# LUMII-Syslab/DiffusionSAT

Hardware: NVIDIA B200
Metric: diffusion samples/sec, 3-SAT n=100 (higher is better)
Workload: dtype f32

## Files before the change

diffusionsat_b200/csrc/dsat_api.cu:

```cuda
#include <cuda_runtime.h>
#include <math.h>
#include <stdint.h>
#include <stdio.h>
#include <stdlib.h>
#include <string.h>

#include <algorithm>
#include <string>
#include <type_traits>
#include <vector>

#include "../../include/dsat.h"
#include "../../include/dsat_debug.h"
#include "dsat_common.cuh"
#include "dsat_gemm_simt.cuh"
#include "dsat_message.cuh"
#include "dsat_spmm.cuh"
#include "dsat_graph_host.cuh"
#include "dsat_norm_head.cuh"
#include "dsat_hist.cuh"
#ifdef DSAT_WITH_TCGEN05
#include "dsat_gemm_tc.cuh"
#include "dsat_mlp_fused.cuh"
#include "dsat_mlp_x3.cuh"
#endif

using namespace dsat;

static cudaError_t dsat_memcpy_sync(void* dst, const void* src, size_t bytes, cudaMemcpyKind kind) {
    cudaError_t e = cudaMemcpy(dst, src, bytes, kind);
    if (e == cudaSuccess && kind == cudaMemcpyHostToDevice) e = cudaDeviceSynchronize();
    return e;
}

namespace {

template <typename T>
struct DevBuf {
    T* p = nullptr;
    size_t count = 0;
    size_t cap = 0;
    cudaError_t alloc(size_t n) {
        if (p && n <= cap) { count = n; return cudaSuccess; }
        release();
        if (n == 0) return cudaSuccess;
        cudaError_t e = cudaMalloc(reinterpret_cast<void**>(&p), n * sizeof(T));
        if (e == cudaSuccess) { count = n; cap = n; }
        else p = nullptr;
        return e;
    }
    void drop() { count = 0; }
    void release() {
        if (p) cudaFree(p);
        p = nullptr; count = 0; cap = 0;
    }
    cudaError_t upload(const T* host, size_t n, cudaStream_t s) {
        return cudaMemcpyAsync(p, host, n * sizeof(T), cudaMemcpyHostToDevice, s);
    }
};

struct PackedLayer {
    DevBuf<float> w, b;
#ifdef DSAT_WITH_TCGEN05
    DevBuf<__nv_bfloat16> w_bf16;
#endif
    int K = 0, N = 0;
};

enum OpId { OP_V1 = 0, OP_Q2, OP_L2, OP_L3, OP_C1, OP_C2, OP_U1, OP_U2, OP_U3, OP_O1, OP_O2, OP_COUNT };

}

constexpr int SPMM_DW_CLAUSE = 2;
struct dsat_ctx {
    int device = 0;
    int sm_count = 148;
    cudaStream_t own_stream = nullptr, stream = nullptr;
    cudaEvent_t ev0 = nullptr, ev1 = nullptr;
    std::string err;
    long long launches = 0;
#ifdef DSAT_WITH_TCGEN05
    int precision = DSAT_F32_TC;
#else
    int precision = DSAT_F32;
#endif
    struct ProfMark { cudaEvent_t ev; int cls; };
    std::vector<ProfMark> prof;
    size_t prof_used = 0;
    bool profiling = false;

    bool has_model = false;
    int F = 0, Q = 0, HQ = 0, HL = 0, HC = 0, HU = 0, HO = 0;
    PackedLayer ops[OP_COUNT];

    bool has_graph = false;
    int n = 0, m = 0, nnz = 0, n_graphs = 0, chains = 0, group_graphs = 0, n_groups = 0, total_graphs = 0;
    int words = 0;
    int max_graph_vars = 0, max_graph_clauses = 0;
    long long Nt = 0, Mt = 0;
    DevBuf<int> cl_rowptr, cl_lit, lit_rowptr, lit_clause, var_seg, clause_seg;
    DevBuf<float> deg_w, vdeg_w, rev_w;
    DevBuf<int> var_order;
    DevBuf<unsigned short> cl_idx16, lit_idx16;
    int cl_idx16_vecs = 0, lit_idx16_vecs = 0, cl_col_off = 0, lit_col_off = 0, lit_ord_off = 0;
    DevBuf<int> cl_desc, lit_desc, lit_desc4;
    bool use_spmm_order = true;
    std::vector<int32_t> h_cl_rowptr, h_cl_lit, h_lit_rowptr, h_lit_clause;
    std::vector<float> h_deg_w, h_rev_w;
    bool spmm_desc_ready = false;
    int spmm_minb = 0, spmm_pf = -1;
    int spmm_half = -1;
    int spmm_lit_dw = 0;
    bool use_idx16 = true;

    bool has_buffers = false;
    DevBuf<float> VROW, CROW, H1, H2, QS, LIT, CH, COUT, U1, U2, UOUT, SPRE, O1, LOGITS, OUT;
    DevBuf<float2> X;
    DevBuf<int> labels, done, steps_taken, rounds_run, graph_sat, graph_map, latch_step, sat_now;
    DevBuf<float> loss_sum, graph_loss;
    DevBuf<unsigned char> BITS, LAST, LATCH, FINAL, is_sat, sat_any;
    DevBuf<unsigned long long> packed;
    DevBuf<int> hist_idx, hist_run, hist_totals;
    DevBuf<unsigned long long> hist_keys, hist_counts;
    DevBuf<float> inj_normals, inj_uniforms, inj_noisy;
    DevBuf<int> inj_labels;
#ifdef DSAT_WITH_TCGEN05
    DevBuf<__nv_bfloat16> VROWb, CROWb, H1b, H2b, QSb, LITb, CHb, COUTb, U1b, U2b, UOUTb, SPREb, O1b;
    CUtensorMap map_a[OP_COUNT];
    CUtensorMap map_b[OP_COUNT];
    int a_box_rows[OP_COUNT] = {0}, b_box_rows[OP_COUNT] = {0};
    bool has_tc_buffers = false;
    fm::FusedMlp fused[5];
    bool fused_ready = false;
    bool use_fused = true;
    bool use_smem_gather = true;
    DevBuf<__nv_bfloat16> VROWp, CROWp, SPREp, H1p, H2p;
    DevBuf<__nv_bfloat16> CHp, U1p, U2p;
    x3::X3Mlp x3s[5];
    bool split_clause = false, split_update = false;
    DevBuf<__nv_bfloat16> wx[12];
    int wx_k64[12] = {0}, wx_n[12] = {0};
    x3::X3Mlp x3[7];
    bool has_x3_buffers = false;
    bool x3_ready = false;
#endif
    bool has_simt_buffers = false;
    float last_noise_scale = 0.f;
    int sampling = DSAT_SAMPLE_INVERSE_CDF;
    DevBuf<StepParams> step_tab;
    DevBuf<int> step_cur;
    std::vector<StepParams> step_tab_host;
    cudaGraphExec_t step_graph = nullptr;
    long long generation = 0, step_graph_generation = -1;
    int step_graph_rounds = -1, step_graph_precision = -1, step_launches = 0;
    bool use_graph = true;

    int ldv() const { return F + DSAT_AUX_PAD + 3 * Q; }
    int ldc() const { return F + 2 * Q; }
    int ldh1() const { return HQ + HL; }
};

#ifdef DSAT_ASSERT
static int* g_assert_host = nullptr;
static std::string assert_note() {
    return g_assert_host && g_assert_host[0] ? " [DSAT_ASSERT failed at line " + std::to_string(g_assert_host[0]) + " of a kernel header]" : "";
}
#else
static std::string assert_note() { return ""; }
#endif

#define CK_CUDA(ctx, expr)                                                              \
    do {                                                                                \
        cudaError_t e__ = (expr);                                                       \
        if (e__ != cudaSuccess) {                                                       \
            (ctx)->err = std::string(#expr) + ": " + cudaGetErrorString(e__) + assert_note(); \
            return DSAT_ERR_CUDA;                                                       \
        }                                                                               \
    } while (0)

#define CK_ARG(ctx, cond, msg)                                                          \
    do {                                                                                \
        if (!(cond)) { (ctx)->err = (msg); return DSAT_ERR_ARG; }                       \
    } while (0)

#define LAUNCHED(ctx)                                                                   \
    do {                                                                                \
        (ctx)->launches++;                                                              \
        CK_CUDA(ctx, cudaGetLastError());                                               \
    } while (0)

namespace {

cudaError_t configure_kernels_for_device() {
    static PerDeviceOnce configured;
    if (configured.done()) return cudaSuccess;
    cudaError_t e = cudaSuccess;
    auto opt_in = [&](auto kernel) {
        if (e == cudaSuccess) e = cudaFuncSetAttribute(kernel, cudaFuncAttributeMaxDynamicSharedMemorySize, 227 * 1024);
    };
#ifdef DSAT_WITH_TCGEN05
    opt_in(clause_gather_smem_kernel<128, true>); opt_in(clause_gather_smem_kernel<128, false>);
    opt_in(clause_gather_smem_kernel<64, true>); opt_in(clause_gather_smem_kernel<64, false>);
    opt_in(clause_gather_smem_kernel<32, true>); opt_in(clause_gather_smem_kernel<32, false>);
    opt_in(literal_gather_smem_kernel<128, true>); opt_in(literal_gather_smem_kernel<128, false>);
    opt_in(literal_gather_smem_kernel<64, true>); opt_in(literal_gather_smem_kernel<64, false>);
    opt_in(literal_gather_smem_kernel<32, true>); opt_in(literal_gather_smem_kernel<32, false>);
    opt_in(clause_gather_smem_f32_kernel<128, true>); opt_in(clause_gather_smem_f32_kernel<128, false>);
    opt_in(clause_gather_smem_f32_kernel<64, true>); opt_in(clause_gather_smem_f32_kernel<64, false>);
    opt_in(clause_gather_smem_f32_kernel<32, true>); opt_in(clause_gather_smem_f32_kernel<32, false>);
    opt_in(clause_gather_smem_f32x2_kernel<128, true>); opt_in(clause_gather_smem_f32x2_kernel<128, false>);
    opt_in(clause_gather_smem_f32x2_kernel<64, true>); opt_in(clause_gather_smem_f32x2_kernel<64, false>);
    opt_in(clause_gather_smem_f32x2_kernel<32, true>); opt_in(clause_gather_smem_f32x2_kernel<32, false>);
    opt_in(literal_gather_smem_f32_kernel<128, true>); opt_in(literal_gather_smem_f32_kernel<128, false>);
    opt_in(literal_gather_smem_f32_kernel<64, true>); opt_in(literal_gather_smem_f32_kernel<64, false>);
    opt_in(literal_gather_smem_f32_kernel<32, true>); opt_in(literal_gather_smem_f32_kernel<32, false>);
    opt_in(pairnorm_smem_kernel<2>); opt_in(pairnorm_smem_kernel<4>); opt_in(pairnorm_smem_kernel<8>);
    if (e == cudaSuccess) e = fm::configure_fused_device();
    if (e == cudaSuccess) e = x3::configure_x3_device(0);
    if (e == cudaSuccess) e = tc::configure_tc_device();
#endif
    if (e == cudaSuccess) configured.mark();
    return e;
}

UnitGraphDev graph_view(const dsat_ctx* c) {
    UnitGraphDev g;
    g.n = c->n; g.m = c->m; g.nnz = c->nnz; g.n_graphs = c->n_graphs;
    g.cl_rowptr = c->cl_rowptr.p; g.cl_lit = c->cl_lit.p;
    g.lit_rowptr = c->lit_rowptr.p; g.lit_clause = c->lit_clause.p;
    g.var_seg = c->var_seg.p; g.clause_seg = c->clause_seg.p;
    g.deg_w = c->deg_w.p; g.vdeg_w = c->vdeg_w.p; g.rev_w = c->rev_w.p;
    g.var_order = c->var_order.p;
    g.cl_idx16 = c->cl_idx16_vecs ? c->cl_idx16.p : nullptr;
    g.lit_idx16 = c->lit_idx16_vecs ? c->lit_idx16.p : nullptr;
    g.cl_idx16_vecs = c->cl_idx16_vecs; g.lit_idx16_vecs = c->lit_idx16_vecs;
    g.cl_col_off = c->cl_col_off; g.lit_col_off = c->lit_col_off; g.lit_ord_off = c->lit_ord_off;
    return g;
}

SkipInfo skip_info(const dsat_ctx* c) {
    static const bool off = getenv("DSAT_SKIP_DONE") && atoi(getenv("DSAT_SKIP_DONE")) == 0;
    if (off || c->n_graphs <= 0 || c->group_graphs % c->n_graphs != 0) return SkipInfo{nullptr, 1};
    return SkipInfo{c->done.p, c->group_graphs / c->n_graphs};
}

int ensure_common_buffers(dsat_ctx* c) {
    if (c->has_buffers) return DSAT_OK;
    if (!c->has_model || !c->has_graph) { c->err = "set the model and the graph first"; return DSAT_ERR_STATE; }
    const size_t Nt = (size_t)c->Nt, Mt = (size_t)c->Mt;
    CK_CUDA(c, c->QS.alloc(Nt * 3 * c->Q));
    CK_CUDA(c, c->LIT.alloc(Nt * 2 * c->Q));
    CK_CUDA(c, c->COUT.alloc(Mt * (c->Q + c->F)));
    CK_CUDA(c, c->UOUT.alloc(Nt * c->F));
    CK_CUDA(c, c->LOGITS.alloc(Nt * DSAT_LOGIT_PAD));
    CK_CUDA(c, c->OUT.alloc(Nt));
    CK_CUDA(c, c->X.alloc(Nt + 1));
    CK_CUDA(c, c->labels.alloc(Nt));
    CK_CUDA(c, c->BITS.alloc(Nt));
    CK_CUDA(c, c->LAST.alloc(Nt));
    CK_CUDA(c, c->LATCH.alloc(Nt));
    CK_CUDA(c, c->FINAL.alloc(Nt));
    const size_t G = (size_t)c->total_graphs, NG = (size_t)c->n_groups;
    CK_CUDA(c, c->done.alloc(NG));
    CK_CUDA(c, c->steps_taken.alloc(NG));
    CK_CUDA(c, c->rounds_run.alloc(NG));
    CK_CUDA(c, c->loss_sum.alloc(NG));
    CK_CUDA(c, c->graph_sat.alloc(G));
    CK_CUDA(c, c->graph_map.alloc(G));
    CK_CUDA(c, c->graph_loss.alloc(G));
    CK_CUDA(c, c->latch_step.alloc(G));
    CK_CUDA(c, c->sat_now.alloc(G));
    CK_CUDA(c, c->is_sat.alloc(G));
    CK_CUDA(c, c->sat_any.alloc(G));
    CK_CUDA(c, c->packed.alloc(G * c->words));
    CK_CUDA(c, cudaMemsetAsync(c->OUT.p, 0, c->OUT.count * sizeof(float), c->stream));
    c->has_buffers = true;
    return DSAT_OK;
}

int ensure_buffers(dsat_ctx* c) {
    int rc = ensure_common_buffers(c);
    if (rc) return rc;
    if (c->has_simt_buffers) return DSAT_OK;
    const size_t Nt = (size_t)c->Nt, Mt = (size_t)c->Mt;
    CK_CUDA(c, c->VROW.alloc(Nt * c->ldv()));
    CK_CUDA(c, c->CROW.alloc(Mt * c->ldc()));
    CK_CUDA(c, c->H1.alloc(Nt * c->ldh1()));
    CK_CUDA(c, c->H2.alloc(Nt * c->HL));
    CK_CUDA(c, c->CH.alloc(Mt * c->HC));
    CK_CUDA(c, c->U1.alloc(Nt * c->HU));
    CK_CUDA(c, c->U2.alloc(Nt * c->HU));
    CK_CUDA(c, c->SPRE.alloc(Nt * c->F));
    CK_CUDA(c, c->O1.alloc(Nt * c->HO));
    CK_CUDA(c, cudaMemsetAsync(c->VROW.p, 0, c->VROW.count * sizeof(float), c->stream));
    CK_CUDA(c, cudaMemsetAsync(c->CROW.p, 0, c->CROW.count * sizeof(float), c->stream));
    c->has_simt_buffers = true;
    return DSAT_OK;
}

#ifdef DSAT_WITH_TCGEN05
static int pick_slice_width(size_t table_rows, int Q, size_t* bytes_out, int budget_kb, int elt_bytes = 2);

__global__ void mirror_cols_kernel(const float* __restrict__ src, int ld_src, __nv_bfloat16* __restrict__ dst, int ld_dst,
                                   long long rows, int cols) {
    const long long i = (long long)blockIdx.x * blockDim.x + threadIdx.x;
    if (i >= rows * cols) return;
    const long long r = i / cols; const int cc = (int)(i % cols);
    dst[(size_t)r * ld_dst + cc] = __float2bfloat16_rn(src[(size_t)r * ld_src + cc]);
}

int ensure_tc_buffers(dsat_ctx* c) {
    if (c->has_tc_buffers) return DSAT_OK;
    int rc = ensure_buffers(c);
    if (rc) return rc;
    const size_t Nt = (size_t)c->Nt, Mt = (size_t)c->Mt;
    const int F = c->F, Q = c->Q;
    CK_CUDA(c, c->VROWb.alloc(Nt * c->ldv()));
    CK_CUDA(c, c->CROWb.alloc(Mt * c->ldc()));
    CK_CUDA(c, c->H1b.alloc(Nt * c->ldh1()));
    CK_CUDA(c, c->H2b.alloc(Nt * c->HL));
    CK_CUDA(c, c->QSb.alloc(Nt * 3 * Q));
    CK_CUDA(c, c->LITb.alloc(Nt * 2 * Q));
    CK_CUDA(c, c->CHb.alloc(Mt * c->HC));
    CK_CUDA(c, c->COUTb.alloc(Mt * (Q + F)));
    CK_CUDA(c, c->UOUTb.alloc(Nt * F));
    CK_CUDA(c, c->U1b.alloc(Nt * c->HU));
    CK_CUDA(c, c->U2b.alloc(Nt * c->HU));
    CK_CUDA(c, c->SPREb.alloc(Nt * F));
    CK_CUDA(c, c->O1b.alloc(Nt * c->HO));
    CK_CUDA(c, cudaMemsetAsync(c->VROWb.p, 0, c->VROWb.count * 2, c->stream));
    CK_CUDA(c, cudaMemsetAsync(c->CROWb.p, 0, c->CROWb.count * 2, c->stream));
    struct Src { const void* p; long long rows; int k; int ld; };
    const Src srcs[OP_COUNT] = {
        {c->VROWb.p, c->Nt, F + DSAT_AUX_PAD, c->ldv()},
        {c->H1b.p, c->Nt, c->HQ, c->ldh1()},
        {c->H1b.p + c->HQ, c->Nt, c->HL, c->ldh1()},
        {c->H2b.p, c->Nt, c->HL, c->HL},
        {c->CROWb.p, c->Mt, F + 2 * Q, c->ldc()},
        {c->CHb.p, c->Mt, c->HC, c->HC},
        {c->VROWb.p, c->Nt, F + DSAT_AUX_PAD + 3 * Q, c->ldv()},
        {c->U1b.p, c->Nt, c->HU, c->HU},
        {c->U2b.p, c->Nt, c->HU, c->HU},
        {c->SPREb.p, c->Nt, F, F},
        {c->O1b.p, c->Nt, c->HO, c->HO},
    };
    for (int op = 0; op < OP_COUNT; ++op) {
        if (srcs[op].k != c->ops[op].K) { c->err = "internal: A operand width mismatch"; return DSAT_ERR_STATE; }
        c->a_box_rows[op] = (int)(srcs[op].rows < tc::BLOCK_M ? srcs[op].rows : tc::BLOCK_M);
        if (!tc::make_bf16_map(&c->map_a[op], srcs[op].p, srcs[op].rows, srcs[op].k, srcs[op].ld, c->a_box_rows[op])) {
            c->err = "cuTensorMapEncodeTiled failed for an activation operand";
            return DSAT_ERR_CUDA;
        }
    }
    {
        enum { FQ = 0, FL, FC, FU, FO };
        const int k64_v1 = (c->ops[OP_V1].K + 63) / 64 * 64;
        struct L { int op; int n; const __nv_bfloat16* w; const float* b; int epi; };
        auto build = [&](int which, int a_op, std::initializer_list<L> layers, tc::TcOut out) -> bool {
            fm::FusedMlp& f = c->fused[which];
            f.map_a = c->map_a[a_op];
            f.p.n_layers = (int)layers.size();
            f.p.rows = (int)(a_op == OP_C1 ? c->Mt : c->Nt);
            f.p.a_box_rows = c->a_box_rows[a_op];
            f.p.qmaps = Q;
            f.p.prof = nullptr;
            f.p.dbg = getenv("DSAT_FM_DEBUG") ? atoi(getenv("DSAT_FM_DEBUG")) : 0;
            f.p.out = out;
            int i = 0;
            for (const L& l : layers) {
                const int K = c->ops[l.op].K, K64 = (K + 63) / 64 * 64;
                f.p.layer[i].K = K; f.p.layer[i].N = l.n; f.p.layer[i].epi = l.epi; f.p.layer[i].bias = l.b;
                f.p.layer[i].box_rows = l.n < 256 ? l.n : 256;
                if (!tc::make_bf16_map(&f.map_w[i], l.w, l.n, K64, K64, f.p.layer[i].box_rows)) return false;
                if (!tc::make_bf16_map(&f.map_wp[i], l.w, l.n, K64, K64, f.p.layer[i].box_rows / 2)) return false;
                ++i;
            }
            {
                static const int mask = getenv("DSAT_A_RING") ? atoi(getenv("DSAT_A_RING")) : 0x1d;
                f.stream_input = ((mask >> which) & 1) != 0;
                static const int pair_mask = getenv("DSAT_PAIR_MODE") ? atoi(getenv("DSAT_PAIR_MODE")) : 0xe;
                f.pair_mode = ((pair_mask >> which) & 1) != 0;
                static const bool pp_env = getenv("DSAT_PING_PONG") != nullptr;
                static const int pp_mask = pp_env ? atoi(getenv("DSAT_PING_PONG")) : 0x1b;
                f.ping_pong = ((pp_mask >> which) & 1) != 0 || (!pp_env && which == FC && f.pair_mode);
                static const int split_on = getenv("DSAT_SPLIT_MODE") ? atoi(getenv("DSAT_SPLIT_MODE")) : 1;
                f.split_step_bias = (split_on & 2) == 0;
                f.split_mode = split_on != 0;
            }
            if (!fm::plan_fused(f)) return false;
            if (getenv("DSAT_PLAN_LOG"))
                fprintf(stderr, "[dsat] fused mlp %d: smem %d B (pad %d), hidden blocks %d x%d, input ring %d, weight ring %d x %d B, "
                        "epilogue warps %d, ping-pong %d, staging in hidden %d, cta pair %d, split %d (%d steps)\n", which, f.smem_bytes, f.p.smem_pad, f.p.ah_blocks,
                        f.p.pp ? 2 : 1, f.p.a_slots, f.p.slots, f.p.slot_bytes, f.p.epi_warps, f.p.pp, f.p.stage_in_h, f.p.pair, f.p.split, f.p.n_steps);
            return true;
        };
        auto W = [&](int op) { return (const __nv_bfloat16*)c->ops[op].w_bf16.p; };
        auto B = [&](int op) { return (const float*)c->ops[op].b.p; };
        tc::TcOut o;
        bool ok = true;
        o = {c->QSb.p, 3 * Q, 1, nullptr, 0, 0, 0};
        ok = ok && build(FQ, OP_V1, {{OP_V1, c->HQ, W(OP_V1), B(OP_V1), tc::TC_LRELU},
                                     {OP_Q2, Q, W(OP_Q2), B(OP_Q2), tc::TC_QUERY}}, o);
        o = {c->LITb.p, 2 * Q, 1, nullptr, 0, 0, 0};
        ok = ok && build(FL, OP_V1, {{OP_V1, c->HL, W(OP_V1) + (size_t)c->HQ * k64_v1, B(OP_V1) + c->HQ, tc::TC_LRELU},
                                     {OP_L2, c->HL, W(OP_L2), B(OP_L2), tc::TC_LRELU},
                                     {OP_L3, 2 * Q, W(OP_L3), B(OP_L3), tc::TC_LINEAR}}, o);
        o = {c->COUTb.p, Q + F, 1, nullptr, 0, 0, 0};
        ok = ok && build(FC, OP_C1, {{OP_C1, c->HC, W(OP_C1), B(OP_C1), tc::TC_LRELU},
                                     {OP_C2, Q + F, W(OP_C2), B(OP_C2), tc::TC_LINEAR}}, o);
        o = {c->UOUTb.p, F, 1, nullptr, 0, 0, 0};
        ok = ok && build(FU, OP_U1, {{OP_U1, c->HU, W(OP_U1), B(OP_U1), tc::TC_LRELU},
                                     {OP_U2, c->HU, W(OP_U2), B(OP_U2), tc::TC_LRELU},
                                     {OP_U3, F, W(OP_U3), B(OP_U3), tc::TC_LINEAR}}, o);
        o = {c->LOGITS.p, DSAT_LOGIT_PAD, 0, nullptr, 0, 0, 0};
        ok = ok && build(FO, OP_O1, {{OP_O1, c->HO, W(OP_O1), B(OP_O1), tc::TC_LRELU},
                                     {OP_O2, DSAT_LOGIT_PAD, W(OP_O2), B(OP_O2), tc::TC_LINEAR}}, o);
        c->fused_ready = ok;
    }
    c->has_tc_buffers = true;
    return DSAT_OK;
}

int tc_pack_weights(dsat_ctx* c) {
    for (int op = 0; op < OP_COUNT; ++op) {
        const int K = c->ops[op].K, N = c->ops[op].N;
        const int K64 = (K + 63) / 64 * 64;
        std::vector<float> w((size_t)K * N);
        CK_CUDA(c, dsat_memcpy_sync(w.data(), c->ops[op].w.p, w.size() * sizeof(float), cudaMemcpyDeviceToHost));
        std::vector<__nv_bfloat16> wt((size_t)N * K64, __float2bfloat16(0.f));
        for (int k = 0; k < K; ++k)
            for (int n = 0; n < N; ++n) wt[(size_t)n * K64 + k] = __float2bfloat16(w[(size_t)k * N + n]);
        CK_CUDA(c, c->ops[op].w_bf16.alloc(wt.size()));
        CK_CUDA(c, dsat_memcpy_sync(c->ops[op].w_bf16.p, wt.data(), wt.size() * 2, cudaMemcpyHostToDevice));
        c->b_box_rows[op] = N < tc::BLOCK_N ? N : tc::BLOCK_N;
        if (!tc::make_bf16_map(&c->map_b[op], c->ops[op].w_bf16.p, N, K64, K64, c->b_box_rows[op])) {
            c->err = "cuTensorMapEncodeTiled failed for a weight operand (no CUDA driver?)";
            return DSAT_ERR_CUDA;
        }
    }
    return DSAT_OK;
}
#endif

void release_buffers(dsat_ctx* c) {
    c->generation++;
    c->VROW.drop(); c->CROW.drop(); c->H1.drop(); c->H2.drop(); c->QS.drop(); c->LIT.drop();
    c->CH.drop(); c->COUT.drop(); c->U1.drop(); c->U2.drop(); c->UOUT.drop(); c->SPRE.drop();
    c->O1.drop(); c->LOGITS.drop(); c->OUT.drop(); c->X.drop(); c->labels.drop();
    c->BITS.drop(); c->LAST.drop(); c->LATCH.drop(); c->FINAL.drop();
    c->done.drop(); c->steps_taken.drop(); c->rounds_run.drop(); c->loss_sum.drop();
    c->graph_sat.drop(); c->graph_map.drop(); c->graph_loss.drop(); c->latch_step.drop();
    c->sat_now.drop(); c->is_sat.drop(); c->sat_any.drop(); c->packed.drop();
    c->inj_normals.drop(); c->inj_uniforms.drop(); c->inj_noisy.drop(); c->inj_labels.drop();
    c->hist_idx.drop(); c->hist_run.drop(); c->hist_totals.drop(); c->hist_keys.drop(); c->hist_counts.drop();
#ifdef DSAT_WITH_TCGEN05
    c->VROWb.drop(); c->CROWb.drop(); c->H1b.drop(); c->H2b.drop(); c->QSb.drop(); c->LITb.drop();
    c->CHb.drop(); c->COUTb.drop(); c->UOUTb.drop(); c->U1b.drop(); c->U2b.drop(); c->SPREb.drop();
    c->O1b.drop();
    c->has_tc_buffers = false;
    c->VROWp.drop(); c->CROWp.drop(); c->SPREp.drop(); c->H1p.drop(); c->H2p.drop();
    c->CHp.drop(); c->U1p.drop(); c->U2p.drop();
    c->has_x3_buffers = false;
#endif
    c->has_buffers = false;
    c->has_simt_buffers = false;
}

void free_buffers(dsat_ctx* c) {
    c->VROW.release(); c->CROW.release(); c->H1.release(); c->H2.release(); c->QS.release(); c->LIT.release();
    c->CH.release(); c->COUT.release(); c->U1.release(); c->U2.release(); c->UOUT.release(); c->SPRE.release();
    c->O1.release(); c->LOGITS.release(); c->OUT.release(); c->X.release(); c->labels.release();
    c->BITS.release(); c->LAST.release(); c->LATCH.release(); c->FINAL.release();
    c->done.release(); c->steps_taken.release(); c->rounds_run.release(); c->loss_sum.release();
    c->graph_sat.release(); c->graph_map.release(); c->graph_loss.release(); c->latch_step.release();
    c->sat_now.release(); c->is_sat.release(); c->sat_any.release(); c->packed.release();
    c->inj_normals.release(); c->inj_uniforms.release(); c->inj_noisy.release(); c->inj_labels.release();
    c->hist_idx.release(); c->hist_run.release(); c->hist_totals.release(); c->hist_keys.release(); c->hist_counts.release();
#ifdef DSAT_WITH_TCGEN05
    c->VROWb.release(); c->CROWb.release(); c->H1b.release(); c->H2b.release(); c->QSb.release(); c->LITb.release();
    c->CHb.release(); c->COUTb.release(); c->UOUTb.release(); c->U1b.release(); c->U2b.release(); c->SPREb.release();
    c->O1b.release();
    c->has_tc_buffers = false;
    c->VROWp.release(); c->CROWp.release(); c->SPREp.release(); c->H1p.release(); c->H2p.release();
    c->CHp.release(); c->U1p.release(); c->U2p.release();
    c->has_x3_buffers = false;
#endif
    c->has_buffers = false;
    c->has_simt_buffers = false;
}

enum ProfClass { PROF_CLAUSE_GATHER = OP_COUNT, PROF_LITERAL_GATHER, PROF_NORM_CLAUSE, PROF_NORM_VAR, PROF_HEAD,
                 PROF_NOISE, PROF_END, PROF_CLASSES = PROF_END };

void prof_mark(dsat_ctx* c, int cls) {
    if (!c->profiling) return;
    if (c->prof_used == c->prof.size()) {
        cudaEvent_t e;
        cudaEventCreate(&e);
        c->prof.push_back({e, cls});
    }
    c->prof[c->prof_used].cls = cls;
    cudaEventRecord(c->prof[c->prof_used].ev, c->stream);
    c->prof_used++;
}

#ifdef DSAT_WITH_TCGEN05
int x3_pack_weights(dsat_ctx* c) {
    struct Cut { int op, col0, n; };
    const Cut cuts[12] = {
        {OP_V1, 0, c->HQ}, {OP_Q2, 0, c->Q}, {OP_V1, c->HQ, c->HL}, {OP_L2, 0, c->HL}, {OP_L3, 0, 2 * c->Q},
        {OP_C1, 0, c->HC}, {OP_C2, 0, c->Q + c->F}, {OP_U1, 0, c->HU}, {OP_U2, 0, c->HU}, {OP_U3, 0, c->F},
        {OP_O1, 0, c->HO}, {OP_O2, 0, DSAT_LOGIT_PAD}};
    for (int i = 0; i < 12; ++i) {
        const int op = cuts[i].op, K = c->ops[op].K, Nop = c->ops[op].N, n = cuts[i].n;
        const int K64 = (K + 63) / 64 * 64;
        std::vector<float> w((size_t)K * Nop);
        CK_CUDA(c, dsat_memcpy_sync(w.data(), c->ops[op].w.p, w.size() * sizeof(float), cudaMemcpyDeviceToHost));
        std::vector<__nv_bfloat16> wt((size_t)2 * n * K64, __float2bfloat16(0.f));
        for (int k = 0; k < K; ++k)
            for (int j = 0; j < n; ++j) {
                const float v = w[(size_t)k * Nop + cuts[i].col0 + j];
                const __nv_bfloat16 hi = __float2bfloat16(v);
                wt[(size_t)j * K64 + k] = hi;
                wt[(size_t)(n + j) * K64 + k] = __float2bfloat16(v - __bfloat162float(hi));
            }
        CK_CUDA(c, c->wx[i].alloc(wt.size()));
        CK_CUDA(c, dsat_memcpy_sync(c->wx[i].p, wt.data(), wt.size() * 2, cudaMemcpyHostToDevice));
        c->wx_k64[i] = K64; c->wx_n[i] = n;
    }
    return DSAT_OK;
}

int ensure_x3_buffers(dsat_ctx* c) {
    if (c->has_x3_buffers) return DSAT_OK;
    int rc = ensure_common_buffers(c);
    if (rc) return rc;
    const size_t Nt = (size_t)c->Nt, Mt = (size_t)c->Mt;
    const int F = c->F, Q = c->Q;
    CK_CUDA(c, c->VROWp.alloc(2 * Nt * c->ldv()));
    CK_CUDA(c, c->CROWp.alloc(2 * Mt * c->ldc()));
    CK_CUDA(c, c->SPREp.alloc(2 * Nt * F));
    CK_CUDA(c, c->H1p.alloc(2 * Nt * c->HL));
    CK_CUDA(c, c->H2p.alloc(2 * Nt * c->HL));
    CK_CUDA(c, cudaMemsetAsync(c->VROWp.p, 0, c->VROWp.count * 2, c->stream));
    CK_CUDA(c, cudaMemsetAsync(c->CROWp.p, 0, c->CROWp.count * 2, c->stream));
    enum { XQ = 0, XL1, XL2, XL3, XC, XU, XO };
    struct L { int wi; int op; int bias_off; int epi; };
    static const int pair_mask = getenv("DSAT_X3_PAIR") ? atoi(getenv("DSAT_X3_PAIR")) : 0x3e;
    auto build = [&](int which, const __nv_bfloat16* a_hi, size_t a_plane, long long rows, int k, int lda,
                     std::initializer_list<L> layers, int n_groups, int out_mode, void* out0, void* out1, int ld_out) -> bool {
        x3::X3Mlp& f = c->x3[which];
        f.ready = false;
        x3::X3Params& p = f.p;
        p.n_layers = (int)layers.size();
        p.rows = (int)rows;
        p.n_groups = n_groups;
        p.a_box_rows = (int)(rows < x3::BLOCK_M ? rows : x3::BLOCK_M);
        p.qmaps = Q;
        p.prof = nullptr;
        p.out_mode = out_mode; p.out0 = out0; p.out1 = out1; p.ld_out = ld_out;
        {
            const SkipInfo sk = skip_info(c);
            p.done = sk.done; p.chains_per_group = sk.chains_per_group;
            p.rows_per_chain = rows == c->Mt ? c->m : c->n;
        }
        f.pair_mode = ((pair_mask >> which) & 1) != 0;
        static const int epi4_mask = getenv("DSAT_X3_EPI4") ? atoi(getenv("DSAT_X3_EPI4")) : 0;
        f.four_epilogue_warps = ((epi4_mask >> which) & 1) != 0;
        if (!tc::make_bf16_map(&f.map_a_hi, a_hi, rows, k, lda, p.a_box_rows)) return false;
        if (!tc::make_bf16_map(&f.map_a_lo, a_hi + a_plane, rows, k, lda, p.a_box_rows)) return false;
        int i = 0;
        for (const L& l : layers) {
            x3::X3Layer& ly = p.layer[i];
            const int n_total = c->wx_n[l.wi];
            ly.K = c->ops[l.op].K; ly.N = n_groups > 1 ? 256 : n_total; ly.n_total = n_total;
            ly.epi = l.epi; ly.w_lo_row = n_total; ly.bias = c->ops[l.op].b.p + l.bias_off;
            if (n_groups > 1 && n_total != 256 * n_groups) return false;
            ++i;
        }
        if (!x3::plan_x3(f)) return false;
        i = 0;
        for (const L& l : layers) {
            const int box = f.p.pair ? p.layer[i].N / 2 : p.layer[i].N;
            if (!tc::make_bf16_map(&f.map_w[i], c->wx[l.wi].p, 2 * c->wx_n[l.wi], c->wx_k64[l.wi], c->wx_k64[l.wi], box)) return false;
            ++i;
        }
        for (; i < x3::MAX_LAYERS; ++i) f.map_w[i] = f.map_w[0];
        if (getenv("DSAT_PLAN_LOG"))
            fprintf(stderr, "[dsat] x3 mlp %d: smem %d B, hidden blocks 2 x %d, input ring %d, weight ring %d x %d B, epilogue warps %d, "
                    "staging in hidden %d, cta pair %d, groups %d\n", which, f.smem_bytes, p.h_blocks, p.a_slots, p.w_slots, p.w_slot_bytes,
                    p.epi_warps, p.stage_in_h, p.pair, p.n_groups);
        return true;
    };
    const size_t vplane = Nt * c->ldv(), cplane = Mt * c->ldc(), splane = Nt * F, hplane = Nt * c->HL;
    bool ok = true;
    ok = ok && build(XQ, c->VROWp.p, vplane, c->Nt, F + DSAT_AUX_PAD, c->ldv(),
                     {{0, OP_V1, 0, tc::TC_LRELU}, {1, OP_Q2, 0, tc::TC_QUERY}}, 1, x3::OUT_F32, c->QS.p, nullptr, 3 * Q);
    const int lgroups = c->HL > 256 ? c->HL / 256 : 1;
    ok = ok && (c->HL <= 256 || c->HL % 256 == 0);
    ok = ok && build(XL1, c->VROWp.p, vplane, c->Nt, F + DSAT_AUX_PAD, c->ldv(),
                     {{2, OP_V1, c->HQ, tc::TC_LRELU}}, lgroups, x3::OUT_SPLIT, c->H1p.p, c->H1p.p + hplane, c->HL);
    ok = ok && build(XL2, c->H1p.p, hplane, c->Nt, c->HL, c->HL,
                     {{3, OP_L2, 0, tc::TC_LRELU}}, lgroups, x3::OUT_SPLIT, c->H2p.p, c->H2p.p + hplane, c->HL);
    const int l3groups = 2 * Q > 256 ? 2 * Q / 256 : 1;
    ok = ok && build(XL3, c->H2p.p, hplane, c->Nt, c->HL, c->HL,
                     {{4, OP_L3, 0, tc::TC_LINEAR}}, l3groups, x3::OUT_F32, c->LIT.p, nullptr, 2 * Q);
    if (Q + F <= 256 && c->HC <= 256)
        ok = ok && build(XC, c->CROWp.p, cplane, c->Mt, F + 2 * Q, c->ldc(),
                         {{5, OP_C1, 0, tc::TC_LRELU}, {6, OP_C2, 0, tc::TC_LINEAR}}, 1, x3::OUT_F32, c->COUT.p, nullptr, Q + F);
    else ok = false;
    if (c->HU <= 256)
        ok = ok && build(XU, c->VROWp.p, vplane, c->Nt, F + DSAT_AUX_PAD + 3 * Q, c->ldv(),
                         {{7, OP_U1, 0, tc::TC_LRELU}, {8, OP_U2, 0, tc::TC_LRELU}, {9, OP_U3, 0, tc::TC_LINEAR}}, 1, x3::OUT_F32,
                         c->UOUT.p, nullptr, F);
    else ok = false;
    ok = ok && build(XO, c->SPREp.p, splane, c->Nt, F, F,
                     {{10, OP_O1, 0, tc::TC_LRELU}, {11, OP_O2, 0, tc::TC_LINEAR}}, 1, x3::OUT_F32, c->LOGITS.p, nullptr, DSAT_LOGIT_PAD);
    {
        static const int split_mask = getenv("DSAT_X3_SPLIT") ? atoi(getenv("DSAT_X3_SPLIT")) : 1;
        c->split_clause = c->split_update = false;
        if (ok && (split_mask & 1)) {
            const size_t chplane = Mt * c->HC;
            CK_CUDA(c, c->CHp.alloc(2 * chplane));
            x3::X3Mlp keep_c = c->x3[XC];
            bool k = build(XC, c->CROWp.p, cplane, c->Mt, F + 2 * Q, c->ldc(), {{5, OP_C1, 0, tc::TC_LRELU}}, 1, x3::OUT_SPLIT,
                           c->CHp.p, c->CHp.p + chplane, c->HC);
            c->x3s[0] = c->x3[XC];
            k = k && build(XC, c->CHp.p, chplane, c->Mt, c->HC, c->HC, {{6, OP_C2, 0, tc::TC_LINEAR}}, 1, x3::OUT_F32,
                           c->COUT.p, nullptr, Q + F);
            c->x3s[1] = c->x3[XC];
            c->x3[XC] = keep_c;
            c->split_clause = k;
        }
        if (ok && (split_mask & 2)) {
            const size_t uplane = Nt * c->HU;
            CK_CUDA(c, c->U1p.alloc(2 * uplane));
            CK_CUDA(c, c->U2p.alloc(2 * uplane));
            x3::X3Mlp keep_u = c->x3[XU];
            bool k = build(XU, c->VROWp.p, vplane, c->Nt, F + DSAT_AUX_PAD + 3 * Q, c->ldv(), {{7, OP_U1, 0, tc::TC_LRELU}}, 1,
                           x3::OUT_SPLIT, c->U1p.p, c->U1p.p + uplane, c->HU);
            c->x3s[2] = c->x3[XU];
            k = k && build(XU, c->U1p.p, uplane, c->Nt, c->HU, c->HU, {{8, OP_U2, 0, tc::TC_LRELU}}, 1, x3::OUT_SPLIT,
                           c->U2p.p, c->U2p.p + uplane, c->HU);
            c->x3s[3] = c->x3[XU];
            k = k && build(XU, c->U2p.p, uplane, c->Nt, c->HU, c->HU, {{9, OP_U3, 0, tc::TC_LINEAR}}, 1, x3::OUT_F32,
                           c->UOUT.p, nullptr, F);
            c->x3s[4] = c->x3[XU];
            c->x3[XU] = keep_u;
            c->split_update = k;
        }
    }
    c->x3_ready = ok;
    if (!ok) { c->err = "the fp32-accurate tensor-core path supports feature_maps = query_maps <= 128 (hidden widths <= 256 or 512)"; return DSAT_ERR_UNSUPPORTED; }
    c->has_x3_buffers = true;
    return DSAT_OK;
}

int run_x3(dsat_ctx* c, int which, int prof_class) {
    prof_mark(c, prof_class);
    CK_CUDA(c, x3::launch_x3(c->x3[which], c->device, c->sm_count, c->stream));
    c->launches++;
    return DSAT_OK;
}
#endif

int run_linear(dsat_ctx* c, int op, const float* A, int lda, float* Y, int ldy, long long rows, int epi) {
    prof_mark(c, op);
    LinearOp l;
    l.A = A; l.lda = lda; l.W = c->ops[op].w.p; l.ldw = c->ops[op].N; l.bias = c->ops[op].b.p;
    l.Y = Y; l.ldy = ldy; l.rows = (int)rows; l.K = c->ops[op].K; l.N = c->ops[op].N; l.epi = epi; l.qmaps = c->Q;
    CK_CUDA(c, launch_sgemm(l, c->stream));
    c->launches++;
    return DSAT_OK;
}

template <typename KernelLauncher>
int dispatch_width(dsat_ctx* c, int width, KernelLauncher&& fn) {
    switch (width) {
        case 64: fn(std::integral_constant<int, 2>()); break;
        case 128: fn(std::integral_constant<int, 4>()); break;
        case 256: fn(std::integral_constant<int, 8>()); break;
        default: c->err = "feature width must be 64, 128 or 256"; return DSAT_ERR_UNSUPPORTED;
    }
    return DSAT_OK;
}

struct LossScalars { float t, ts, norm_plus; };


float kl_host(float pa, float pb) {
    float qa = 1.0f - pa;
    float t1 = pa == 0.f ? 0.f : pa * (logf(pa) - logf(pb));
    float t2 = qa == 0.f ? 0.f : qa * (log1pf(-pa) - log1pf(-pb));
    return t1 + t2;
}
LossScalars loss_scalars(float noise_scale) {
    LossScalars s;
    s.t = powf(noise_scale, 0.5f);
    s.ts = fminf(s.t + 0.01f, 1.0f);
    float pa = 0.0f * (1.0f - s.ts) + s.ts / 2.0f;
    float pb = 0.0f * (1.0f - 1.0f) + 1.0f / 2.0f;
    s.norm_plus = kl_host(pa, pb) + 1e-4f;
    return s;
}

#ifdef DSAT_WITH_TCGEN05
static inline bool use_tc(const dsat_ctx* c) { return c->precision == DSAT_BF16 || c->precision == DSAT_BF16_UNFUSED; }
static inline bool use_x3(const dsat_ctx* c) { return c->precision == DSAT_F32_TC; }
static inline __nv_bfloat16* vrow_b(dsat_ctx* c) { return use_tc(c) ? c->VROWb.p : use_x3(c) ? c->VROWp.p : nullptr; }
static inline __nv_bfloat16* crow_b(dsat_ctx* c) { return use_tc(c) ? c->CROWb.p : use_x3(c) ? c->CROWp.p : nullptr; }
#else
static inline bool use_tc(const dsat_ctx*) { return false; }
static inline bool use_x3(const dsat_ctx*) { return false; }
static inline __nv_bfloat16* vrow_b(dsat_ctx*) { return nullptr; }
static inline __nv_bfloat16* crow_b(dsat_ctx*) { return nullptr; }
#endif

int ensure_active_buffers(dsat_ctx* c) {
#ifdef DSAT_WITH_TCGEN05
    if (use_tc(c)) return ensure_tc_buffers(c);
    if (use_x3(c)) return ensure_x3_buffers(c);
#endif
    return ensure_buffers(c);
}

int begin_call(dsat_ctx* c, float noise_scale, const float* noisy_dev, const float* uniforms_dev,
               const int* labels_dev, bool use_x, NoiseSource ns, const StepParams* sp_tab = nullptr, const int* sp_cur = nullptr) {
    const long long Nt = c->Nt;
    const int threads = 256;
    const bool x3p = use_x3(c);
    const size_t vplane = x3p ? (size_t)Nt * c->ldv() : 0, cplane = x3p ? (size_t)c->Mt * c->ldc() : 0;
    c->last_noise_scale = noise_scale;
    step_begin_kernel<<<(unsigned)((Nt + threads - 1) / threads), threads, 0, c->stream>>>(
        Nt, noise_scale, use_x ? c->X.p : nullptr, noisy_dev, uniforms_dev, labels_dev, c->labels.p,
        x3p ? nullptr : c->VROW.p, c->ldv(), c->F, vrow_b(c), ns, vplane, sp_tab, sp_cur, c->sampling == DSAT_SAMPLE_GUMBEL ? 1 : 0);
    LAUNCHED(c);
    {
        long long tot;
        if (!x3p) {
            tot = Nt * (c->F / 4);
            fill_cols_kernel<<<(unsigned)((tot + threads - 1) / threads), threads, 0, c->stream>>>(
                c->VROW.p, c->ldv(), Nt, c->F / 4, 1.0f);
            LAUNCHED(c);
            tot = c->Mt * (c->F / 4);
            fill_cols_kernel<<<(unsigned)((tot + threads - 1) / threads), threads, 0, c->stream>>>(
                c->CROW.p, c->ldc(), c->Mt, c->F / 4, 1.0f);
            LAUNCHED(c);
        }
        if (use_tc(c) || x3p) {
            tot = Nt * (c->F / 8);
            fill_cols_bf16_kernel<<<(unsigned)((tot + threads - 1) / threads), threads, 0, c->stream>>>(
                vrow_b(c), c->ldv(), Nt, c->F / 8, 1.0f);
            LAUNCHED(c);
            if (x3p) {
                fill_cols_bf16_kernel<<<(unsigned)((tot + threads - 1) / threads), threads, 0, c->stream>>>(
                    vrow_b(c) + vplane, c->ldv(), Nt, c->F / 8, 0.0f);
                LAUNCHED(c);
            }
            tot = c->Mt * (c->F / 8);
            fill_cols_bf16_kernel<<<(unsigned)((tot + threads - 1) / threads), threads, 0, c->stream>>>(
                crow_b(c), c->ldc(), c->Mt, c->F / 8, 1.0f);
            LAUNCHED(c);
            if (x3p) {
                fill_cols_bf16_kernel<<<(unsigned)((tot + threads - 1) / threads), threads, 0, c->stream>>>(
                    crow_b(c) + cplane, c->ldc(), c->Mt, c->F / 8, 0.0f);
                LAUNCHED(c);
            }
        }
    }
    CK_CUDA(c, cudaMemsetAsync(c->done.p, 0, c->done.count * sizeof(int), c->stream));
    CK_CUDA(c, cudaMemsetAsync(c->steps_taken.p, 0xff, c->steps_taken.count * sizeof(int), c->stream));
    CK_CUDA(c, cudaMemsetAsync(c->rounds_run.p, 0, c->rounds_run.count * sizeof(int), c->stream));
    CK_CUDA(c, cudaMemsetAsync(c->loss_sum.p, 0, c->loss_sum.count * sizeof(float), c->stream));
    return DSAT_OK;
}

#ifdef DSAT_WITH_TCGEN05
int run_linear_tc(dsat_ctx* c, int op, long long rows, int epi, void* p0, int ld0, bool bf0,
                  void* p1 = nullptr, int ld1 = 0, bool bf1 = false, int split = 0) {
    prof_mark(c, op);
    tc::TcLinear l;
    l.map_a = c->map_a[op]; l.map_b = c->map_b[op]; l.bias = c->ops[op].b.p;
    l.out.ptr0 = p0; l.out.ld0 = ld0; l.out.bf16_0 = bf0 ? 1 : 0;
    l.out.ptr1 = p1; l.out.ld1 = ld1; l.out.bf16_1 = bf1 ? 1 : 0; l.out.split = split;
    l.rows = (int)rows; l.K = c->ops[op].K; l.N = c->ops[op].N; l.epi = epi; l.qmaps = c->Q;
    l.a_box_rows = c->a_box_rows[op]; l.b_box_rows = c->b_box_rows[op];
    CK_CUDA(c, tc::launch_tc_linear(l, c->stream));
    c->launches++;
    return DSAT_OK;
}
#endif

#ifdef DSAT_WITH_TCGEN05
int run_fused(dsat_ctx* c, int which, int prof_class) {
    prof_mark(c, prof_class);
    CK_CUDA(c, fm::launch_fused(c->fused[which], c->sm_count, c->stream));
    c->launches++;
    return DSAT_OK;
}
#endif

#ifdef DSAT_WITH_TCGEN05
static int pick_slice_width(size_t table_rows, int Q, size_t* bytes_out, int budget_kb, int elt_bytes) {
    static const int env_kb = getenv("DSAT_GATHER_KB") ? atoi(getenv("DSAT_GATHER_KB")) : 0;
    if (env_kb > 0) budget_kb = env_kb;
    const int widths[3] = {128, 64, 32};
    for (int pass = 0; pass < 2; ++pass)
        for (int w : widths) {
            if (w > Q || Q % w) continue;
            const size_t bytes = 2 * table_rows * (size_t)w * (size_t)elt_bytes;
            if (bytes <= (size_t)(pass == 0 ? budget_kb : 220) * 1024u) { *bytes_out = bytes; return w; }
        }
    return 0;
}

static bool idx_fits(size_t table_bytes, int idx_vecs) {
    if (idx_vecs <= 0) return false;
    const size_t sm_bytes = 227 * 1024, reserved = 1024, with_idx = table_bytes + (size_t)idx_vecs * 16;
    if (with_idx + reserved > sm_bytes) return false;
    return sm_bytes / (with_idx + reserved) == sm_bytes / (table_bytes + reserved);
}


bool launch_clause_gather_smem(dsat_ctx* c, const UnitGraphDev& g) {
    if (c->n_graphs != 1 || !c->use_smem_gather) return false;
    size_t bytes = 0;
    const int w = pick_slice_width((size_t)2 * c->n, c->Q, &bytes, 56);
    if (!w) return false;
    dim3 grid((unsigned)c->chains, (unsigned)(c->Q / w));
    const int Q = c->Q;
    const bool si = c->use_idx16 && idx_fits(bytes, g.cl_idx16_vecs);
    const size_t smem = bytes + (si ? (size_t)g.cl_idx16_vecs * 16 : 0);
    auto launch = [&](auto kernel) -> bool {
        kernel<<<grid, 512, smem, c->stream>>>(g, Q, c->LITb.p, 2 * Q, c->QSb.p, 3 * Q, Q, c->CROWb.p, c->ldc(), c->F, skip_info(c));
        return true;
    };
    if (w == 128) return si ? launch(clause_gather_smem_kernel<128, true>) : launch(clause_gather_smem_kernel<128, false>);
    if (w == 64) return si ? launch(clause_gather_smem_kernel<64, true>) : launch(clause_gather_smem_kernel<64, false>);
    return si ? launch(clause_gather_smem_kernel<32, true>) : launch(clause_gather_smem_kernel<32, false>);
}

bool launch_literal_gather_smem(dsat_ctx* c, const UnitGraphDev& g) {
    if (c->n_graphs != 1 || !c->use_smem_gather) return false;
    size_t bytes = 0;
    const int w = pick_slice_width((size_t)c->m, c->Q, &bytes, 112);
    if (!w) return false;
    dim3 grid((unsigned)c->chains, (unsigned)(c->Q / w));
    const int Q = c->Q, F = c->F;
    const bool si = c->use_idx16 && idx_fits(bytes, g.lit_idx16_vecs);
    const size_t smem = bytes + (si ? (size_t)g.lit_idx16_vecs * 16 : 0);
    auto launch = [&](auto kernel) -> bool {
        kernel<<<grid, 512, smem, c->stream>>>(g, Q, c->CROWb.p, c->ldc(), F + Q, c->COUTb.p, Q + F, c->QSb.p, 3 * Q, c->VROWb.p,
                                               c->ldv(), F + DSAT_AUX_PAD, skip_info(c));
        return true;
    };
    if (w == 128) return si ? launch(literal_gather_smem_kernel<128, true>) : launch(literal_gather_smem_kernel<128, false>);
    if (w == 64) return si ? launch(literal_gather_smem_kernel<64, true>) : launch(literal_gather_smem_kernel<64, false>);
    return si ? launch(literal_gather_smem_kernel<32, true>) : launch(literal_gather_smem_kernel<32, false>);
}
#endif

#ifdef DSAT_WITH_TCGEN05
bool launch_clause_gather_smem_f32(dsat_ctx* c, const UnitGraphDev& g) {
    if (c->n_graphs != 1 || !c->use_smem_gather) return false;
    static const bool one_table = getenv("DSAT_GATHER_F32_CL1") && atoi(getenv("DSAT_GATHER_F32_CL1")) != 0;
    size_t bytes = 0;
    static const int budget = getenv("DSAT_GATHER_F32_KB_CL") ? atoi(getenv("DSAT_GATHER_F32_KB_CL")) : 110;
    const int w = pick_slice_width((size_t)2 * c->n, c->Q, &bytes, budget, one_table ? 2 : 4);
    if (!w || bytes > 112 * 1024) return false;
    dim3 grid((unsigned)c->chains, (unsigned)((one_table ? 2 : 1) * (c->Q / w)));
    const int Q = c->Q;
    const bool si = c->use_idx16 && idx_fits(bytes, g.cl_idx16_vecs);
    const size_t smem = bytes + (si ? (size_t)g.cl_idx16_vecs * 16 : 0);
    const size_t cplane = (size_t)c->Mt * c->ldc();
    auto launch = [&](auto kernel) -> bool {
        kernel<<<grid, 512, smem, c->stream>>>(g, Q, c->LIT.p, 2 * Q, c->QS.p, 3 * Q, Q, c->CROWp.p, cplane, c->ldc(), c->F, skip_info(c));
        return true;
    };
    if (one_table) {
        if (w == 128) return si ? launch(clause_gather_smem_f32_kernel<128, true>) : launch(clause_gather_smem_f32_kernel<128, false>);
        if (w == 64) return si ? launch(clause_gather_smem_f32_kernel<64, true>) : launch(clause_gather_smem_f32_kernel<64, false>);
        return si ? launch(clause_gather_smem_f32_kernel<32, true>) : launch(clause_gather_smem_f32_kernel<32, false>);
    }
    if (w == 128) return si ? launch(clause_gather_smem_f32x2_kernel<128, true>) : launch(clause_gather_smem_f32x2_kernel<128, false>);
    if (w == 64) return si ? launch(clause_gather_smem_f32x2_kernel<64, true>) : launch(clause_gather_smem_f32x2_kernel<64, false>);
    return si ? launch(clause_gather_smem_f32x2_kernel<32, true>) : launch(clause_gather_smem_f32x2_kernel<32, false>);
}

bool launch_literal_gather_smem_f32(dsat_ctx* c, const UnitGraphDev& g) {
    if (c->n_graphs != 1 || !c->use_smem_gather) return false;
    size_t bytes = 0;
    static const int budget = getenv("DSAT_GATHER_F32_KB_LIT") ? atoi(getenv("DSAT_GATHER_F32_KB_LIT")) : 112;
    const int w = pick_slice_width((size_t)c->m, c->Q, &bytes, budget, 2);
    if (!w || bytes > 112 * 1024) return false;
    dim3 grid((unsigned)c->chains, (unsigned)(2 * (c->Q / w)));
    const int Q = c->Q, F = c->F;
    const bool si = c->use_idx16 && idx_fits(bytes, g.lit_idx16_vecs);
    const size_t smem = bytes + (si ? (size_t)g.lit_idx16_vecs * 16 : 0);
    const size_t cplane = (size_t)c->Mt * c->ldc(), vplane = (size_t)c->Nt * c->ldv();
    static const int planes_tables = getenv("DSAT_GATHER_F32_PLANES") ? atoi(getenv("DSAT_GATHER_F32_PLANES")) : 1;
    auto launch = [&](auto kernel) -> bool {
        kernel<<<grid, 512, smem, c->stream>>>(g, Q, c->CROWp.p, cplane, c->ldc(), F + Q, c->COUT.p, Q + F, c->QS.p, 3 * Q,
                                                c->VROWp.p, vplane, c->ldv(), F + DSAT_AUX_PAD, skip_info(c), planes_tables);
        return true;
    };
    if (w == 128) return si ? launch(literal_gather_smem_f32_kernel<128, true>) : launch(literal_gather_smem_f32_kernel<128, false>);
    if (w == 64) return si ? launch(literal_gather_smem_f32_kernel<64, true>) : launch(literal_gather_smem_f32_kernel<64, false>);
    return si ? launch(literal_gather_smem_f32_kernel<32, true>) : launch(literal_gather_smem_f32_kernel<32, false>);
}
#endif

#ifdef DSAT_WITH_TCGEN05
template <int V>
bool launch_pairnorm_smem(dsat_ctx* c, const int* seg, int rows_per_chain, int max_graph_rows, const float* src, int ld_src, int src_off,
                          __nv_bfloat16* state_hi, size_t state_plane, int ld_state, __nv_bfloat16* pre_hi, size_t pre_plane, int ld_pre) {
    static const bool off = getenv("DSAT_PN_SMEM") && atoi(getenv("DSAT_PN_SMEM")) == 0;
    if (off) return false;
    constexpr int F = 32 * V;
    const size_t row_bytes = (size_t)max_graph_rows * F * 4;
    const int threads = row_bytes > 100 * 1024 ? 1024 : row_bytes > 48 * 1024 ? 512 : 256;
    const int groups = threads / F > 0 ? threads / F : 1;
    const size_t smem = (size_t)(F + groups * F) * 4 + row_bytes;
    if (smem > 227 * 1024) return false;
    int per_sm = (int)((228 * 1024) / (smem + 1024));
    const int by_threads = 2048 / threads;
    if (per_sm > by_threads) per_sm = by_threads;
    if (per_sm < 1) per_sm = 1;
    int grid = c->sm_count * per_sm;
    if (grid > c->total_graphs) grid = c->total_graphs;
    pairnorm_smem_kernel<V><<<grid, threads, smem, c->stream>>>(seg, c->n_graphs, rows_per_chain, c->total_graphs, src, ld_src, src_off,
                                                                state_hi, state_plane, ld_state, pre_hi, pre_plane, ld_pre, skip_info(c));
    return true;
}
#endif

int run_round(dsat_ctx* c, int round, const float* normals_dev, NoiseSource ns, LossScalars ls,
              const StepParams* sp_tab = nullptr, const int* sp_cur = nullptr) {
    const long long Nt = c->Nt, Mt = c->Mt;
    const int F = c->F, Q = c->Q, ldv = c->ldv(), ldc = c->ldc(), ldh1 = c->ldh1();
    const UnitGraphDev g = graph_view(c);
    const bool tcp = use_tc(c);
    const bool x3p = use_x3(c);
    const size_t vplane = x3p ? (size_t)Nt * ldv : 0, cplane = x3p ? (size_t)Mt * ldc : 0;
    const SkipInfo skip = skip_info(c);
#ifdef DSAT_WITH_TCGEN05
    const bool fusedp = tcp && c->precision == DSAT_BF16 && c->fused_ready && c->use_fused;
    enum { XQ = 0, XL1, XL2, XL3, XC, XU, XO };
#endif
    int rc;
    {
        const int threads = 256;
        prof_mark(c, PROF_NOISE);
        round_noise_kernel<<<(unsigned)((Nt + threads - 1) / threads), threads, 0, c->stream>>>(
            Nt, normals_dev, x3p ? nullptr : c->VROW.p, ldv, F, vrow_b(c), ns, (unsigned)round, vplane, sp_tab, sp_cur, skip, c->n);
        LAUNCHED(c);
    }
    if (x3p) {
#ifdef DSAT_WITH_TCGEN05
        if ((rc = run_x3(c, XQ, OP_Q2))) return rc;
        if ((rc = run_x3(c, XL1, OP_V1))) return rc;
        if ((rc = run_x3(c, XL2, OP_L2))) return rc;
        if ((rc = run_x3(c, XL3, OP_L3))) return rc;
#endif
    } else if (!tcp) {
        if ((rc = run_linear(c, OP_V1, c->VROW.p, ldv, c->H1.p, ldh1, Nt, EPI_LRELU))) return rc;
        if ((rc = run_linear(c, OP_Q2, c->H1.p, ldh1, c->QS.p, 3 * Q, Nt, EPI_QUERY))) return rc;
        if ((rc = run_linear(c, OP_L2, c->H1.p + c->HQ, ldh1, c->H2.p, c->HL, Nt, EPI_LRELU))) return rc;
        if ((rc = run_linear(c, OP_L3, c->H2.p, c->HL, c->LIT.p, 2 * Q, Nt, EPI_LINEAR))) return rc;
    }
#ifdef DSAT_WITH_TCGEN05
    else {
        if (fusedp) {
            if ((rc = run_fused(c, 0, OP_Q2))) return rc;
            if ((rc = run_fused(c, 1, OP_L3))) return rc;
        } else {
        if ((rc = run_linear_tc(c, OP_V1, Nt, tc::TC_LRELU, c->H1b.p, ldh1, true))) return rc;
        if ((rc = run_linear_tc(c, OP_Q2, Nt, tc::TC_QUERY, c->QSb.p, 3 * Q, true))) return rc;
        if ((rc = run_linear_tc(c, OP_L2, Nt, tc::TC_LRELU, c->H2b.p, c->HL, true))) return rc;
        if ((rc = run_linear_tc(c, OP_L3, Nt, tc::TC_LINEAR, c->LITb.p, 2 * Q, true))) return rc;
        }
    }
#endif
    prof_mark(c, PROF_CLAUSE_GATHER);
    rc = dispatch_width(c, Q, [&](auto v) {
        constexpr int V = decltype(v)::value;
        const int grid = tcp ? gather_grid(clause_gather_kernel<V, __nv_bfloat16>, Mt, GATHER_WARPS, c->sm_count)
                             : gather_grid(clause_gather_kernel<V, float>, Mt, GATHER_WARPS, c->sm_count);
        if (x3p) {
#ifdef DSAT_WITH_TCGEN05
            if (!launch_clause_gather_smem_f32(c, g))
#endif
            clause_gather_kernel<V, float><<<grid, GATHER_WARPS * 32, 0, c->stream>>>(
                g, c->chains, c->LIT.p, 2 * Q, c->QS.p, 3 * Q, Q, nullptr, ldc, F, crow_b(c), cplane, skip);
        } else if (!tcp)
            clause_gather_kernel<V, float><<<grid, GATHER_WARPS * 32, 0, c->stream>>>(
                g, c->chains, c->LIT.p, 2 * Q, c->QS.p, 3 * Q, Q, c->CROW.p, ldc, F, nullptr, 0, skip);
#ifdef DSAT_WITH_TCGEN05
        else if (!launch_clause_gather_smem(c, g))
            clause_gather_kernel<V, __nv_bfloat16><<<grid, GATHER_WARPS * 32, 0, c->stream>>>(
                g, c->chains, c->LITb.p, 2 * Q, c->QSb.p, 3 * Q, Q, c->CROWb.p, ldc, F, nullptr, 0, skip);
#endif
    });
    if (rc) return rc;
    LAUNCHED(c);
    if (x3p) {
#ifdef DSAT_WITH_TCGEN05
        if (c->split_clause) {
            for (int k = 0; k < 2; ++k) {
                prof_mark(c, k == 0 ? OP_C1 : OP_C2);
                CK_CUDA(c, x3::launch_x3(c->x3s[k], c->device, c->sm_count, c->stream));
                c->launches++;
            }
        } else if ((rc = run_x3(c, XC, OP_C2))) return rc;
#endif
    } else if (!tcp) {
        if ((rc = run_linear(c, OP_C1, c->CROW.p, ldc, c->CH.p, c->HC, Mt, EPI_LRELU))) return rc;
        if ((rc = run_linear(c, OP_C2, c->CH.p, c->HC, c->COUT.p, Q + F, Mt, EPI_LINEAR))) return rc;
    }
#ifdef DSAT_WITH_TCGEN05
    else {
        if (fusedp) {
            if ((rc = run_fused(c, 2, OP_C2))) return rc;
        } else {
        if ((rc = run_linear_tc(c, OP_C1, Mt, tc::TC_LRELU, c->CHb.p, c->HC, true))) return rc;
        if ((rc = run_linear_tc(c, OP_C2, Mt, tc::TC_LINEAR, c->COUTb.p, Q + F, true))) return rc;
        }
    }
#endif
    prof_mark(c, PROF_LITERAL_GATHER);
    rc = dispatch_width(c, Q, [&](auto v) {
        constexpr int V = decltype(v)::value;
        const int grid = tcp ? gather_grid(literal_gather_kernel<V, __nv_bfloat16>, Nt, GATHER_WARPS, c->sm_count)
                             : gather_grid(literal_gather_kernel<V, float>, Nt, GATHER_WARPS, c->sm_count);
        if (x3p) {
#ifdef DSAT_WITH_TCGEN05
            if (!launch_literal_gather_smem_f32(c, g))
#endif
            literal_gather_kernel<V, float><<<grid, GATHER_WARPS * 32, 0, c->stream>>>(
                g, c->chains, nullptr, ldc, F + Q, c->COUT.p, Q + F, c->QS.p, 3 * Q, nullptr, ldv, F + DSAT_AUX_PAD,
                vrow_b(c), vplane, crow_b(c), cplane, skip);
        } else if (!tcp)
            literal_gather_kernel<V, float><<<grid, GATHER_WARPS * 32, 0, c->stream>>>(
                g, c->chains, c->CROW.p, ldc, F + Q, c->COUT.p, Q + F, c->QS.p, 3 * Q, c->VROW.p, ldv, F + DSAT_AUX_PAD,
                nullptr, 0, nullptr, 0, skip);
#ifdef DSAT_WITH_TCGEN05
        else if (!launch_literal_gather_smem(c, g))
            literal_gather_kernel<V, __nv_bfloat16><<<grid, GATHER_WARPS * 32, 0, c->stream>>>(
                g, c->chains, c->CROWb.p, ldc, F + Q, c->COUTb.p, Q + F, c->QSb.p, 3 * Q, c->VROWb.p, ldv, F + DSAT_AUX_PAD,
                nullptr, 0, nullptr, 0, skip);
#endif
    });
    if (rc) return rc;
    LAUNCHED(c);
    prof_mark(c, PROF_NORM_CLAUSE);
    rc = dispatch_width(c, F, [&](auto v) {
        constexpr int V = decltype(v)::value;
        int grid = c->total_graphs < c->sm_count * 8 ? c->total_graphs : c->sm_count * 8;
        {
            static const int l2_mb = getenv("DSAT_PN_L2_MB") ? atoi(getenv("DSAT_PN_L2_MB")) : 0;
            if (l2_mb > 0) {
                const double per_graph = (double)c->m / c->n_graphs * F * (tcp ? 2 : 4);
                int cap = (int)(l2_mb * 1048576.0 / (per_graph > 1 ? per_graph : 1));
                cap = cap < c->sm_count ? c->sm_count : cap;
                if (grid > cap) grid = cap;
            }
        }
        if (x3p) {
#ifdef DSAT_WITH_TCGEN05
            if (!launch_pairnorm_smem<V>(c, c->clause_seg.p, c->m, c->max_graph_clauses, c->COUT.p, Q + F, Q, crow_b(c), cplane, ldc,
                                         nullptr, 0, 0))
#endif
            pairnorm_kernel<V, float, float><<<grid, PN_WARPS * 32, 0, c->stream>>>(
                c->clause_seg.p, c->n_graphs, c->m, c->total_graphs, c->COUT.p, Q + F, Q, nullptr, ldc, nullptr, 0,
                crow_b(c), cplane, nullptr, 0, skip);
        } else if (!tcp)
            pairnorm_kernel<V, float, float><<<grid, PN_WARPS * 32, 0, c->stream>>>(
                c->clause_seg.p, c->n_graphs, c->m, c->total_graphs, c->COUT.p, Q + F, Q, c->CROW.p, ldc, nullptr, 0,
                nullptr, 0, nullptr, 0, skip);
#ifdef DSAT_WITH_TCGEN05
        else
            pairnorm_bf16_kernel<32 * V><<<grid, PN_WARPS * 32, 0, c->stream>>>(
                c->clause_seg.p, c->n_graphs, c->m, c->total_graphs, c->COUTb.p, Q + F, Q, c->CROWb.p, ldc, nullptr, 0, skip);
#endif
    });
    if (rc) return rc;
    LAUNCHED(c);
    if (x3p) {
#ifdef DSAT_WITH_TCGEN05
        if (c->split_update) {
            for (int k = 0; k < 3; ++k) {
                prof_mark(c, k == 0 ? OP_U1 : k == 1 ? OP_U2 : OP_U3);
                CK_CUDA(c, x3::launch_x3(c->x3s[2 + k], c->device, c->sm_count, c->stream));
                c->launches++;
            }
        } else if ((rc = run_x3(c, XU, OP_U3))) return rc;
#endif
    } else if (!tcp) {
        if ((rc = run_linear(c, OP_U1, c->VROW.p, ldv, c->U1.p, c->HU, Nt, EPI_LRELU))) return rc;
        if ((rc = run_linear(c, OP_U2, c->U1.p, c->HU, c->U2.p, c->HU, Nt, EPI_LRELU))) return rc;
        if ((rc = run_linear(c, OP_U3, c->U2.p, c->HU, c->UOUT.p, F, Nt, EPI_LINEAR))) return rc;
    }
#ifdef DSAT_WITH_TCGEN05
    else {
        if (fusedp) {
            if ((rc = run_fused(c, 3, OP_U3))) return rc;
        } else {
        if ((rc = run_linear_tc(c, OP_U1, Nt, tc::TC_LRELU, c->U1b.p, c->HU, true))) return rc;
        if ((rc = run_linear_tc(c, OP_U2, Nt, tc::TC_LRELU, c->U2b.p, c->HU, true))) return rc;
        if ((rc = run_linear_tc(c, OP_U3, Nt, tc::TC_LINEAR, c->UOUTb.p, F, true))) return rc;
        }
    }
#endif
    prof_mark(c, PROF_NORM_VAR);
    rc = dispatch_width(c, F, [&](auto v) {
        constexpr int V = decltype(v)::value;
        int grid = c->total_graphs < c->sm_count * 8 ? c->total_graphs : c->sm_count * 8;
        if (x3p) {
#ifdef DSAT_WITH_TCGEN05
            if (!launch_pairnorm_smem<V>(c, c->var_seg.p, c->n, c->max_graph_vars, c->UOUT.p, F, 0, vrow_b(c), vplane, ldv,
                                         c->SPREp.p, (size_t)Nt * F, F))
            pairnorm_kernel<V, float, float><<<grid, PN_WARPS * 32, 0, c->stream>>>(
                c->var_seg.p, c->n_graphs, c->n, c->total_graphs, c->UOUT.p, F, 0, nullptr, ldv, nullptr, F,
                vrow_b(c), vplane, c->SPREp.p, (size_t)Nt * F, skip);
#endif
        } else if (!tcp)
            pairnorm_kernel<V, float, float><<<grid, PN_WARPS * 32, 0, c->stream>>>(
                c->var_seg.p, c->n_graphs, c->n, c->total_graphs, c->UOUT.p, F, 0, c->VROW.p, ldv, c->SPRE.p, F,
                nullptr, 0, nullptr, 0, skip);
#ifdef DSAT_WITH_TCGEN05
        else
            pairnorm_bf16_kernel<32 * V><<<grid, PN_WARPS * 32, 0, c->stream>>>(
                c->var_seg.p, c->n_graphs, c->n, c->total_graphs, c->UOUTb.p, F, 0, c->VROWb.p, ldv, c->SPREb.p, F, skip);
#endif
    });
    if (rc) return rc;
    LAUNCHED(c);
    if (x3p) {
#ifdef DSAT_WITH_TCGEN05
        if ((rc = run_x3(c, XO, OP_O2))) return rc;
#endif
    } else if (!tcp) {
        if ((rc = run_linear(c, OP_O1, c->SPRE.p, F, c->O1.p, c->HO, Nt, EPI_LRELU))) return rc;
        if ((rc = run_linear(c, OP_O2, c->O1.p, c->HO, c->LOGITS.p, DSAT_LOGIT_PAD, Nt, EPI_LINEAR))) return rc;
    }
#ifdef DSAT_WITH_TCGEN05
    else {
        if (fusedp) {
            if ((rc = run_fused(c, 4, OP_O2))) return rc;
        } else {
        if ((rc = run_linear_tc(c, OP_O1, Nt, tc::TC_LRELU, c->O1b.p, c->HO, true))) return rc;
        if ((rc = run_linear_tc(c, OP_O2, Nt, tc::TC_LINEAR, c->LOGITS.p, DSAT_LOGIT_PAD, false))) return rc;
        }
    }
#endif
    prof_mark(c, PROF_HEAD);
    head_kernel<<<c->total_graphs, 128, 0, c->stream>>>(g, c->total_graphs, c->group_graphs, c->LOGITS.p,
                                                         DSAT_LOGIT_PAD, c->labels.p, ls.t, ls.ts, ls.norm_plus,
                                                         c->done.p, c->OUT.p, c->BITS.p, c->graph_sat.p,
                                                         c->graph_loss.p, c->graph_map.p, sp_tab, sp_cur);
    LAUNCHED(c);
    group_finalize_kernel<<<(c->n_groups + 127) / 128, 128, 0, c->stream>>>(
        c->n_groups, c->group_graphs, c->total_graphs, round, c->graph_sat.p, c->graph_loss.p, c->done.p,
        c->steps_taken.p, c->loss_sum.p, c->rounds_run.p);
    LAUNCHED(c);
    prof_mark(c, PROF_END);
    return DSAT_OK;
}

int pack_weights(dsat_ctx* c, const float* const* kernels, const float* const* biases, const int* in_dims,
                 const int* out_dims) {
    const int F = c->F, Q = c->Q, A = DSAT_AUX_PAD;
    const int hq = out_dims[0], hl = out_dims[2], hc = out_dims[5], hu = out_dims[7], ho = out_dims[10];
    c->HQ = pad16(hq); c->HL = pad16(hl); c->HC = pad16(hc); c->HU = pad16(hu); c->HO = pad16(ho);

    auto upload = [&](int op, int K, int N, const std::vector<float>& w, const std::vector<float>& b) -> int {
        c->ops[op].K = K; c->ops[op].N = N;
        CK_CUDA(c, c->ops[op].w.alloc((size_t)K * N));
        CK_CUDA(c, c->ops[op].b.alloc((size_t)N));
        CK_CUDA(c, dsat_memcpy_sync(c->ops[op].w.p, w.data(), w.size() * sizeof(float), cudaMemcpyHostToDevice));
        CK_CUDA(c, dsat_memcpy_sync(c->ops[op].b.p, b.data(), b.size() * sizeof(float), cudaMemcpyHostToDevice));
        return DSAT_OK;
    };
    auto blit = [](std::vector<float>& dst, int dst_ld, int dst_r, int dst_c, const float* src, int src_ld,
                   int src_r, int rows, int cols) {
        for (int r = 0; r < rows; ++r)
            memcpy(&dst[(size_t)(dst_r + r) * dst_ld + dst_c], src + (size_t)(src_r + r) * src_ld, cols * sizeof(float));
    };
    auto plain = [&](int op, int layer, int Kp, int Np) -> int {
        std::vector<float> w((size_t)Kp * Np, 0.f), b(Np, 0.f);
        blit(w, Np, 0, 0, kernels[layer], out_dims[layer], 0, in_dims[layer], out_dims[layer]);
        memcpy(b.data(), biases[layer], out_dims[layer] * sizeof(float));
        return upload(op, Kp, Np, w, b);
    };
    int rc;
    {
        const int K = F + A, N = c->HQ + c->HL;
        std::vector<float> w((size_t)K * N, 0.f), b(N, 0.f);
        blit(w, N, 0, 0, kernels[0], hq, 0, F + 9, hq);
        blit(w, N, 0, c->HQ, kernels[2], hl, 0, F + 9, hl);
        memcpy(b.data(), biases[0], hq * sizeof(float));
        memcpy(b.data() + c->HQ, biases[2], hl * sizeof(float));
        if ((rc = upload(OP_V1, K, N, w, b))) return rc;
    }
    if ((rc = plain(OP_Q2, 1, c->HQ, Q))) return rc;
    if ((rc = plain(OP_L2, 3, c->HL, c->HL))) return rc;
    if ((rc = plain(OP_L3, 4, c->HL, 2 * Q))) return rc;
    if ((rc = plain(OP_C1, 5, F + 2 * Q, c->HC))) return rc;
    if ((rc = plain(OP_C2, 6, c->HC, Q + F))) return rc;
    {
        const int K = F + A + 3 * Q, N = c->HU;
        std::vector<float> w((size_t)K * N, 0.f), b(N, 0.f);
        blit(w, N, 0, 0, kernels[7], hu, Q, F + 9, hu);
        blit(w, N, F + A, 0, kernels[7], hu, 0, Q, hu);
        blit(w, N, F + A + Q, 0, kernels[7], hu, Q + F + 9, 2 * Q, hu);
        memcpy(b.data(), biases[7], hu * sizeof(float));
        if ((rc = upload(OP_U1, K, N, w, b))) return rc;
    }
    if ((rc = plain(OP_U2, 8, c->HU, c->HU))) return rc;
    if ((rc = plain(OP_U3, 9, c->HU, F))) return rc;
    if ((rc = plain(OP_O1, 10, F, c->HO))) return rc;
    if ((rc = plain(OP_O2, 11, c->HO, DSAT_LOGIT_PAD))) return rc;
    return DSAT_OK;
}

}

static void drop_step_graph(dsat_ctx* c) {
    if (c->step_graph) cudaGraphExecDestroy(c->step_graph);
    c->step_graph = nullptr;
    c->step_graph_generation = -1;
}

extern "C" {

int dsat_version(void) { return 2; }

int dsat_build_info(void) {
    int flags = 0;
#ifdef DSAT_WITH_TCGEN05
    flags |= 1;
#endif
#ifdef DSAT_ASSERT
    flags |= 2;
#endif
    return flags;
}

int dsat_create(int device, dsat_ctx** out) {
    if (!out) return DSAT_ERR_ARG;
    *out = nullptr;
    int count = 0;
    if (cudaGetDeviceCount(&count) != cudaSuccess || device < 0 || device >= count) return DSAT_ERR_CUDA;
    dsat_ctx* c = new dsat_ctx();
    c->device = device;
    if (cudaSetDevice(device) != cudaSuccess) { delete c; return DSAT_ERR_CUDA; }
    cudaDeviceGetAttribute(&c->sm_count, cudaDevAttrMultiProcessorCount, device);
    if (configure_kernels_for_device() != cudaSuccess) { delete c; return DSAT_ERR_CUDA; }
#ifdef DSAT_ASSERT
    if (!g_assert_host && cudaHostAlloc(reinterpret_cast<void**>(&g_assert_host), 2 * sizeof(int), cudaHostAllocMapped) == cudaSuccess) {
        g_assert_host[0] = g_assert_host[1] = 0;
        int* dev_view = nullptr;
        if (cudaHostGetDevicePointer(reinterpret_cast<void**>(&dev_view), g_assert_host, 0) == cudaSuccess)
            cudaMemcpyToSymbol(g_dsat_assert_slot, &dev_view, sizeof(dev_view));
    }
#endif
    if (cudaStreamCreateWithFlags(&c->own_stream, cudaStreamNonBlocking) != cudaSuccess) { delete c; return DSAT_ERR_CUDA; }
    c->stream = c->own_stream;
    cudaEventCreate(&c->ev0);
    cudaEventCreate(&c->ev1);
#ifdef DSAT_WITH_TCGEN05
    {
        const char* e = getenv("DSAT_FUSED_MLP");
        if (e && e[0] == '0') c->use_fused = false;
        e = getenv("DSAT_SPMM_ORDER");
        if (e) c->use_spmm_order = e[0] != '0';
        e = getenv("DSAT_SPMM_MINB");
        if (e) c->spmm_minb = atoi(e);
        e = getenv("DSAT_SPMM_PF");
        if (e) c->spmm_pf = atoi(e);
        e = getenv("DSAT_SPMM_LIT_DW");
        if (e) c->spmm_lit_dw = atoi(e);
        e = getenv("DSAT_SPMM_HALF");
        if (e) c->spmm_half = atoi(e);
        e = getenv("DSAT_IDX16");
        if (e) c->use_idx16 = e[0] != '0';
        e = getenv("DSAT_SMEM_GATHER");
        if (e && e[0] == '0') c->use_smem_gather = false;
        e = getenv("DSAT_GRAPH");
        if (e && e[0] == '0') c->use_graph = false;
    }
#endif
    *out = c;
    return DSAT_OK;
}

void dsat_destroy(dsat_ctx* c) {
    if (!c) return;
    cudaSetDevice(c->device);
    cudaStreamSynchronize(c->stream);
    drop_step_graph(c);
    c->step_tab.release(); c->step_cur.release();
    free_buffers(c);
    for (auto& op : c->ops) {
        op.w.release(); op.b.release();
#ifdef DSAT_WITH_TCGEN05
        op.w_bf16.release();
#endif
    }
#ifdef DSAT_WITH_TCGEN05
    for (auto& w : c->wx) w.release();
#endif
    c->cl_rowptr.release(); c->cl_lit.release(); c->lit_rowptr.release(); c->lit_clause.release();
    c->var_seg.release(); c->clause_seg.release(); c->deg_w.release(); c->vdeg_w.release(); c->rev_w.release(); c->var_order.release();
    c->cl_idx16.release(); c->lit_idx16.release(); c->cl_idx16_vecs = c->lit_idx16_vecs = 0;
    c->cl_desc.release(); c->lit_desc.release(); c->lit_desc4.release();
    for (auto& pm : c->prof) cudaEventDestroy(pm.ev);
    if (c->ev0) cudaEventDestroy(c->ev0);
    if (c->ev1) cudaEventDestroy(c->ev1);
    if (c->own_stream) cudaStreamDestroy(c->own_stream);
    delete c;
}

const char* dsat_last_error(const dsat_ctx* c) { return c ? c->err.c_str() : "null context"; }

int dsat_set_stream(dsat_ctx* c, void* s) {
    if (!c) return DSAT_ERR_ARG;
    c->generation++;
    c->stream = s ? reinterpret_cast<cudaStream_t>(s) : c->own_stream;
    return DSAT_OK;
}

int dsat_synchronize(dsat_ctx* c) {
    if (!c) return DSAT_ERR_ARG;
    CK_CUDA(c, cudaSetDevice(c->device));
    CK_CUDA(c, cudaStreamSynchronize(c->stream));
    return DSAT_OK;
}

int dsat_timer_begin(dsat_ctx* c) {
    if (!c) return DSAT_ERR_ARG;
    CK_CUDA(c, cudaSetDevice(c->device));
    CK_CUDA(c, cudaEventRecord(c->ev0, c->stream));
    return DSAT_OK;
}

int dsat_timer_end(dsat_ctx* c, float* ms) {
    if (!c || !ms) return DSAT_ERR_ARG;
    CK_CUDA(c, cudaEventRecord(c->ev1, c->stream));
    CK_CUDA(c, cudaEventSynchronize(c->ev1));
    CK_CUDA(c, cudaEventElapsedTime(ms, c->ev0, c->ev1));
    return DSAT_OK;
}

long long dsat_launch_count(const dsat_ctx* c) { return c ? c->launches : 0; }

#ifdef DSAT_WITH_TCGEN05
static bool x3_supported(const dsat_ctx* c) {
    auto wide_ok = [](int n) { return n <= 256 || n % 256 == 0; };
    return c->HQ <= 256 && c->HC <= 256 && c->HU <= 256 && c->HO <= 256 && c->Q + c->F <= 256 && wide_ok(c->HL) && wide_ok(2 * c->Q);
}
#endif

int dsat_get_precision(const dsat_ctx* c) { return c ? c->precision : DSAT_ERR_ARG; }

int dsat_set_precision(dsat_ctx* c, int dtype) {
    if (!c) return DSAT_ERR_ARG;
    if (dtype == DSAT_F32) { c->precision = dtype; return DSAT_OK; }
#ifdef DSAT_WITH_TCGEN05
    if (dtype == DSAT_BF16 || dtype == DSAT_BF16_UNFUSED) { c->precision = dtype; return DSAT_OK; }
    if (dtype == DSAT_F32_TC) {
        if (c->has_model && !x3_supported(c)) {
            c->err = "DSAT_F32_TC needs layer widths of at most 256 (feature_maps, query_maps <= 128); use DSAT_F32";
            return DSAT_ERR_UNSUPPORTED;
        }
        c->precision = dtype;
        return DSAT_OK;
    }
#endif
    c->err = "precision not available in this build";
    return DSAT_ERR_UNSUPPORTED;
}

int dsat_set_sampling(dsat_ctx* c, int mode) {
    if (!c) return DSAT_ERR_ARG;
    CK_ARG(c, mode == DSAT_SAMPLE_INVERSE_CDF || mode == DSAT_SAMPLE_GUMBEL, "dsat_set_sampling: unknown mode");
    if (mode != c->sampling) c->generation++;
    c->sampling = mode;
    return DSAT_OK;
}

int dsat_set_model(dsat_ctx* c, int n_layers, const float* const* kernels, const float* const* biases,
                   const int* in_dims, const int* out_dims) {
    if (!c) return DSAT_ERR_ARG;
    CK_ARG(c, n_layers == 12 && kernels && biases && in_dims && out_dims, "dsat_set_model: expected 12 layers");
    CK_CUDA(c, cudaSetDevice(c->device));
    const int F = in_dims[10], Q = out_dims[1];
    CK_ARG(c, (F == 64 || F == 128 || F == 256) && (Q == 64 || Q == 128 || Q == 256),
           "feature_maps and query_maps must be 64, 128 or 256");
// ... 559 lines not shown
        cudaError_t e = x3::launch_x3(f, c->device, c->sm_count, c->stream);
        c->launches++;
        if (e == cudaSuccess) e = cudaStreamSynchronize(c->stream);
        if (e == cudaSuccess) e = dsat_memcpy_sync(counters16, d.p, 16 * sizeof(long long), cudaMemcpyDeviceToHost);
        d.release();
        CK_CUDA(c, e);
        return DSAT_OK;
    }
    if (which > 4) return DSAT_ERR_ARG;
    int rc = ensure_tc_buffers(c);
    if (rc) return rc;
    CK_ARG(c, c->fused_ready, "fused kernels unavailable");
    DevBuf<long long> d;
    CK_CUDA(c, d.alloc(16));
    CK_CUDA(c, cudaMemsetAsync(d.p, 0, 16 * sizeof(long long), c->stream));
    fm::FusedMlp f = c->fused[which];
    f.p.prof = d.p;
    cudaError_t e = fm::launch_fused(f, c->sm_count, c->stream);
    c->launches++;
    if (e == cudaSuccess) e = cudaStreamSynchronize(c->stream);
    if (e == cudaSuccess) e = dsat_memcpy_sync(counters16, d.p, 16 * sizeof(long long), cudaMemcpyDeviceToHost);
    d.release();
    CK_CUDA(c, e);
    return DSAT_OK;
#endif
}

int dsat_profile_classes(void) { return PROF_CLASSES; }

int dsat_profile_rounds(dsat_ctx* c, int rounds, uint64_t seed, float* class_ms, int32_t* class_launches) {
    if (!c || !class_ms) return DSAT_ERR_ARG;
    CK_ARG(c, rounds > 0, "dsat_profile_rounds: rounds must be positive");
    CK_CUDA(c, cudaSetDevice(c->device));
    int rc = ensure_active_buffers(c);
    if (rc) return rc;
    {
        const long long rows4 = (2 * c->Nt + 3) / 4;
        fill_cols_kernel<<<(unsigned)((rows4 + 255) / 256), 256, 0, c->stream>>>(reinterpret_cast<float*>(c->X.p), 4, rows4, 1, 0.5f);
        LAUNCHED(c);
    }
    NoiseSource ns{seed, 0ull, 0u};
    if ((rc = begin_call(c, 0.5f, nullptr, nullptr, nullptr, true, ns))) return rc;
    const LossScalars ls = loss_scalars(0.5f);
    c->prof_used = 0;
    c->profiling = true;
    for (int r = 0; r < rounds && rc == 0; ++r) rc = run_round(c, r, nullptr, ns, ls);
    c->profiling = false;
    if (rc) return rc;
    CK_CUDA(c, cudaStreamSynchronize(c->stream));
    for (int k = 0; k < PROF_CLASSES; ++k) { class_ms[k] = 0.f; if (class_launches) class_launches[k] = 0; }
    for (size_t i = 0; i + 1 < c->prof_used; ++i) {
        const int cls = c->prof[i].cls;
        if (cls < 0 || cls >= PROF_CLASSES) continue;
        float ms = 0.f;
        CK_CUDA(c, cudaEventElapsedTime(&ms, c->prof[i].ev, c->prof[i + 1].ev));
        class_ms[cls] += ms;
        if (class_launches) class_launches[cls] += 1;
    }
    return DSAT_OK;
}

static int debug_buffer(dsat_ctx* c, int id, float** p, long long* rows, int* ld) {
    const long long Nt = c->Nt, Mt = c->Mt;
    switch (id) {
        case DSAT_BUF_VROW: *p = c->VROW.p; *rows = Nt; *ld = c->ldv(); break;
        case DSAT_BUF_CROW: *p = c->CROW.p; *rows = Mt; *ld = c->ldc(); break;
        case DSAT_BUF_H1: *p = c->H1.p; *rows = Nt; *ld = c->ldh1(); break;
        case DSAT_BUF_H2: *p = c->H2.p; *rows = Nt; *ld = c->HL; break;
        case DSAT_BUF_QS: *p = c->QS.p; *rows = Nt; *ld = 3 * c->Q; break;
        case DSAT_BUF_LIT: *p = c->LIT.p; *rows = Nt; *ld = 2 * c->Q; break;
        case DSAT_BUF_CH: *p = c->CH.p; *rows = Mt; *ld = c->HC; break;
        case DSAT_BUF_COUT: *p = c->COUT.p; *rows = Mt; *ld = c->Q + c->F; break;
        case DSAT_BUF_U1: *p = c->U1.p; *rows = Nt; *ld = c->HU; break;
        case DSAT_BUF_U2: *p = c->U2.p; *rows = Nt; *ld = c->HU; break;
        case DSAT_BUF_UOUT: *p = c->UOUT.p; *rows = Nt; *ld = c->F; break;
        case DSAT_BUF_SPRE: *p = c->SPRE.p; *rows = Nt; *ld = c->F; break;
        case DSAT_BUF_O1: *p = c->O1.p; *rows = Nt; *ld = c->HO; break;
        case DSAT_BUF_LOGITS: *p = c->LOGITS.p; *rows = Nt; *ld = DSAT_LOGIT_PAD; break;
        case DSAT_BUF_OUT: *p = c->OUT.p; *rows = Nt; *ld = 1; break;
        case DSAT_BUF_X: *p = reinterpret_cast<float*>(c->X.p); *rows = Nt; *ld = 2; break;
        default: c->err = "unknown buffer id"; return DSAT_ERR_ARG;
    }
    return DSAT_OK;
}

int dsat_debug_dims(const dsat_ctx* cc, int buffer, long long* rows, int* ld) {
    dsat_ctx* c = const_cast<dsat_ctx*>(cc);
    if (!c || !rows || !ld) return DSAT_ERR_ARG;
    CK_ARG(c, c->has_model && c->has_graph, "set the model and the graph first");
    float* p;
    return debug_buffer(c, buffer, &p, rows, ld);
}

int dsat_debug_read(dsat_ctx* c, int buffer, float* host_out, long long count) {
    if (!c || !host_out) return DSAT_ERR_ARG;
    CK_CUDA(c, cudaSetDevice(c->device));
    int rc = ensure_active_buffers(c);
    if (rc) return rc;
    float* p; long long rows; int ld;
    if ((rc = debug_buffer(c, buffer, &p, &rows, &ld))) return rc;
    CK_ARG(c, count == rows * ld, "dsat_debug_read: count must be rows*ld");
    CK_CUDA(c, cudaStreamSynchronize(c->stream));
#ifdef DSAT_WITH_TCGEN05
    if (use_x3(c)) {
        const __nv_bfloat16* src = nullptr;
        switch (buffer) {
            case DSAT_BUF_VROW: src = c->VROWp.p; break;
            case DSAT_BUF_CROW: src = c->CROWp.p; break;
            case DSAT_BUF_SPRE: src = c->SPREp.p; break;
            case DSAT_BUF_H2: src = c->H2p.p; break;
            case DSAT_BUF_H1: case DSAT_BUF_CH: case DSAT_BUF_U1: case DSAT_BUF_U2: case DSAT_BUF_O1:
                c->err = "this buffer stays on-chip on the fp32-accurate tensor-core path";
                return DSAT_ERR_UNSUPPORTED;
            default: break;
        }
        if (src) {
            std::vector<__nv_bfloat16> tmp((size_t)count * 2);
            CK_CUDA(c, dsat_memcpy_sync(tmp.data(), src, (size_t)count * 4, cudaMemcpyDeviceToHost));
            for (long long i = 0; i < count; ++i) host_out[i] = __bfloat162float(tmp[i]) + __bfloat162float(tmp[count + i]);
            return DSAT_OK;
        }
    }
    if (use_tc(c)) {
        const __nv_bfloat16* src = nullptr;
        switch (buffer) {
            case DSAT_BUF_VROW: src = c->VROWb.p; break;
            case DSAT_BUF_CROW: src = c->CROWb.p; break;
            case DSAT_BUF_SPRE: src = c->SPREb.p; break;
            case DSAT_BUF_QS: src = c->QSb.p; break;
            case DSAT_BUF_LIT: src = c->LITb.p; break;
            case DSAT_BUF_COUT: src = c->COUTb.p; break;
            case DSAT_BUF_UOUT: src = c->UOUTb.p; break;
            default: break;
        }
        if (src) {
            std::vector<__nv_bfloat16> tmp((size_t)count);
            CK_CUDA(c, dsat_memcpy_sync(tmp.data(), src, (size_t)count * 2, cudaMemcpyDeviceToHost));
            for (long long i = 0; i < count; ++i) host_out[i] = __bfloat162float(tmp[i]);
            return DSAT_OK;
        }
    }
#endif
    CK_CUDA(c, dsat_memcpy_sync(host_out, p, (size_t)count * sizeof(float), cudaMemcpyDeviceToHost));
    return DSAT_OK;
}

int dsat_debug_write(dsat_ctx* c, int buffer, const float* host_in, long long count) {
    if (!c || !host_in) return DSAT_ERR_ARG;
    CK_CUDA(c, cudaSetDevice(c->device));
    int rc = ensure_active_buffers(c);
    if (rc) return rc;
    float* p; long long rows; int ld;
    if ((rc = debug_buffer(c, buffer, &p, &rows, &ld))) return rc;
    CK_ARG(c, count == rows * ld, "dsat_debug_write: count must be rows*ld");
    CK_CUDA(c, cudaStreamSynchronize(c->stream));
#ifdef DSAT_WITH_TCGEN05
    if (use_x3(c)) {
        __nv_bfloat16* dst = buffer == DSAT_BUF_VROW ? c->VROWp.p : buffer == DSAT_BUF_CROW ? c->CROWp.p
                           : buffer == DSAT_BUF_SPRE ? c->SPREp.p : nullptr;
        if (dst) {
            std::vector<__nv_bfloat16> tmp((size_t)count * 2);
            for (long long i = 0; i < count; ++i) {
                const __nv_bfloat16 hi = __float2bfloat16(host_in[i]);
                tmp[i] = hi;
                tmp[count + i] = __float2bfloat16(host_in[i] - __bfloat162float(hi));
            }
            CK_CUDA(c, dsat_memcpy_sync(dst, tmp.data(), (size_t)count * 4, cudaMemcpyHostToDevice));
            return DSAT_OK;
        }
        if (p == nullptr) { c->err = "this buffer stays on-chip on the fp32-accurate tensor-core path"; return DSAT_ERR_UNSUPPORTED; }
    }
#endif
    CK_CUDA(c, dsat_memcpy_sync(p, host_in, (size_t)count * sizeof(float), cudaMemcpyHostToDevice));
#ifdef DSAT_WITH_TCGEN05
    if (use_tc(c) && (buffer == DSAT_BUF_VROW || buffer == DSAT_BUF_CROW || buffer == DSAT_BUF_SPRE)) {
        __nv_bfloat16* dst = buffer == DSAT_BUF_VROW ? c->VROWb.p : buffer == DSAT_BUF_CROW ? c->CROWb.p : c->SPREb.p;
        const long long tot = rows * ld;
        mirror_cols_kernel<<<(unsigned)((tot + 255) / 256), 256, 0, c->stream>>>(p, ld, dst, ld, rows, ld);
        LAUNCHED(c);
        CK_CUDA(c, cudaStreamSynchronize(c->stream));
    }
#endif
    return DSAT_OK;
}

int dsat_tc_linear_test(dsat_ctx* c, int rows, int K, int N, const float* a_host, const float* w_host,
                        const float* bias_host, int epi, int out_bf16, float* out_host) {
    if (!c || !a_host || !w_host || !bias_host || !out_host) return DSAT_ERR_ARG;
#ifndef DSAT_WITH_TCGEN05
    c->err = "built without the tcgen05 path";
    return DSAT_ERR_UNSUPPORTED;
#else
    CK_ARG(c, rows > 0 && K > 0 && N > 0 && K % 16 == 0 && N % 16 == 0, "dsat_tc_linear_test: K and N must be multiples of 16");
    CK_ARG(c, epi != tc::TC_QUERY || N % 32 == 0, "query epilogue needs N % 32 == 0");
    CK_CUDA(c, cudaSetDevice(c->device));
    const int K64 = (K + 63) / 64 * 64;
    const int out_cols = epi == tc::TC_QUERY ? 3 * N : N;
    std::vector<__nv_bfloat16> a((size_t)rows * K), wt((size_t)N * K64, __float2bfloat16(0.f));
    for (size_t i = 0; i < a.size(); ++i) a[i] = __float2bfloat16(a_host[i]);
    for (int k = 0; k < K; ++k)
        for (int n = 0; n < N; ++n) wt[(size_t)n * K64 + k] = __float2bfloat16(w_host[(size_t)k * N + n]);
    DevBuf<__nv_bfloat16> da, dw, dout_b;
    DevBuf<float> db, dout_f;
    CK_CUDA(c, da.alloc(a.size()));
    CK_CUDA(c, dw.alloc(wt.size()));
    CK_CUDA(c, db.alloc(N));
    CK_CUDA(c, dout_b.alloc((size_t)rows * out_cols));
    CK_CUDA(c, dout_f.alloc((size_t)rows * out_cols));
    CK_CUDA(c, dsat_memcpy_sync(da.p, a.data(), a.size() * 2, cudaMemcpyHostToDevice));
    CK_CUDA(c, dsat_memcpy_sync(dw.p, wt.data(), wt.size() * 2, cudaMemcpyHostToDevice));
    CK_CUDA(c, dsat_memcpy_sync(db.p, bias_host, N * sizeof(float), cudaMemcpyHostToDevice));
    tc::TcLinear l;
    l.a_box_rows = rows < tc::BLOCK_M ? rows : tc::BLOCK_M;
    l.b_box_rows = N < tc::BLOCK_N ? N : tc::BLOCK_N;
    if (!tc::make_bf16_map(&l.map_a, da.p, rows, K, K, l.a_box_rows) || !tc::make_bf16_map(&l.map_b, dw.p, N, K64, K64, l.b_box_rows)) {
        c->err = "cuTensorMapEncodeTiled failed";
        da.release(); dw.release(); db.release(); dout_b.release(); dout_f.release();
        return DSAT_ERR_CUDA;
    }
    l.bias = db.p;
    l.out.ptr0 = out_bf16 ? (void*)dout_b.p : (void*)dout_f.p; l.out.ld0 = out_cols; l.out.bf16_0 = out_bf16 ? 1 : 0;
    l.out.ptr1 = nullptr; l.out.ld1 = 0; l.out.bf16_1 = 0; l.out.split = 0;
    l.rows = rows; l.K = K; l.N = N; l.epi = epi; l.qmaps = N;
    cudaError_t e = tc::launch_tc_linear(l, c->stream);
    c->launches++;
    if (e == cudaSuccess) e = cudaStreamSynchronize(c->stream);
    if (e == cudaSuccess) {
        if (out_bf16) {
            std::vector<__nv_bfloat16> ob((size_t)rows * out_cols);
            e = dsat_memcpy_sync(ob.data(), dout_b.p, ob.size() * 2, cudaMemcpyDeviceToHost);
            for (size_t i = 0; i < ob.size(); ++i) out_host[i] = __bfloat162float(ob[i]);
        } else {
            e = dsat_memcpy_sync(out_host, dout_f.p, (size_t)rows * out_cols * sizeof(float), cudaMemcpyDeviceToHost);
        }
    }
    da.release(); dw.release(); db.release(); dout_b.release(); dout_f.release();
    CK_CUDA(c, e);
    return DSAT_OK;
#endif
}

int dsat_debug_rounding(dsat_ctx* c, uint64_t seed, int step) {
    if (!c) return DSAT_ERR_ARG;
    CK_CUDA(c, cudaSetDevice(c->device));
    int rc = ensure_active_buffers(c);
    if (rc) return rc;
    NoiseSource ns{seed, 0ull, (unsigned)step};
    if ((rc = begin_call(c, 0.5f, nullptr, nullptr, nullptr, true, ns))) return rc;
    CK_CUDA(c, cudaStreamSynchronize(c->stream));
    return DSAT_OK;
}

int dsat_debug_begin(dsat_ctx* c, float noise_scale, const float* noisy_num, const int32_t* labels) {
    if (!c || !noisy_num) return DSAT_ERR_ARG;
    CK_CUDA(c, cudaSetDevice(c->device));
    int rc = ensure_active_buffers(c);
    if (rc) return rc;
    const size_t Nt = (size_t)c->Nt;
    CK_CUDA(c, c->inj_noisy.alloc(Nt * 2));
    CK_CUDA(c, c->inj_noisy.upload(noisy_num, Nt * 2, c->stream));
    if (labels) {
        CK_CUDA(c, c->inj_labels.alloc(Nt));
        CK_CUDA(c, c->inj_labels.upload(labels, Nt, c->stream));
    }
    NoiseSource ns{0ull, 0ull, 0u};
    if ((rc = begin_call(c, noise_scale, c->inj_noisy.p, nullptr, labels ? c->inj_labels.p : nullptr, false, ns))) return rc;
    CK_CUDA(c, cudaStreamSynchronize(c->stream));
    return DSAT_OK;
}

int dsat_debug_round(dsat_ctx* c, int round, const float* normals) {
    if (!c) return DSAT_ERR_ARG;
    CK_CUDA(c, cudaSetDevice(c->device));
    int rc = ensure_active_buffers(c);
    if (rc) return rc;
    const size_t Nt = (size_t)c->Nt;
    if (normals) {
        CK_CUDA(c, c->inj_normals.alloc(Nt * 4));
        CK_CUDA(c, c->inj_normals.upload(normals, Nt * 4, c->stream));
    }
    CK_CUDA(c, cudaStreamSynchronize(c->stream));
    const float noise_scale = c->last_noise_scale;
    NoiseSource ns{0ull, 0ull, 0u};
    rc = run_round(c, round, normals ? c->inj_normals.p : nullptr, ns, loss_scalars(noise_scale));
    if (rc) return rc;
    CK_CUDA(c, cudaStreamSynchronize(c->stream));
    return DSAT_OK;
}

int dsat_debug_mlp(dsat_ctx* c, int which) {
    if (!c || which < 0 || which > 4) return DSAT_ERR_ARG;
    CK_CUDA(c, cudaSetDevice(c->device));
    int rc = ensure_active_buffers(c);
    if (rc) return rc;
    const long long Nt = c->Nt, Mt = c->Mt;
    const int F = c->F, Q = c->Q, ldv = c->ldv(), ldc = c->ldc(), ldh1 = c->ldh1();
    (void)Mt; (void)ldc;
#ifdef DSAT_WITH_TCGEN05
    if (use_x3(c)) {
        enum { XQ = 0, XL1, XL2, XL3, XC, XU, XO };
        switch (which) {
            case 0: rc = run_x3(c, XQ, OP_Q2); break;
            case 1: rc = run_x3(c, XL1, OP_V1); if (!rc) rc = run_x3(c, XL2, OP_L2); if (!rc) rc = run_x3(c, XL3, OP_L3); break;
            case 2:
                if (c->split_clause) {
                    for (int k = 0; k < 2 && !rc; ++k) {
                        CK_CUDA(c, x3::launch_x3(c->x3s[k], c->device, c->sm_count, c->stream));
                        c->launches++;
                    }
                } else rc = run_x3(c, XC, OP_C2);
                break;
            case 3:
                if (c->split_update) {
                    for (int k = 0; k < 3 && !rc; ++k) {
                        CK_CUDA(c, x3::launch_x3(c->x3s[2 + k], c->device, c->sm_count, c->stream));
                        c->launches++;
                    }
                } else rc = run_x3(c, XU, OP_U3);
                break;
            default: rc = run_x3(c, XO, OP_O2); break;
        }
    } else if (use_tc(c) && c->precision == DSAT_BF16 && c->fused_ready && c->use_fused) {
        static const int cls[5] = {OP_Q2, OP_L3, OP_C2, OP_U3, OP_O2};
        rc = run_fused(c, which, cls[which]);
    } else if (use_tc(c)) {
        switch (which) {
            case 0: rc = run_linear_tc(c, OP_V1, Nt, tc::TC_LRELU, c->H1b.p, ldh1, true);
                    if (!rc) rc = run_linear_tc(c, OP_Q2, Nt, tc::TC_QUERY, c->QSb.p, 3 * Q, true); break;
            case 1: rc = run_linear_tc(c, OP_V1, Nt, tc::TC_LRELU, c->H1b.p, ldh1, true);
                    if (!rc) rc = run_linear_tc(c, OP_L2, Nt, tc::TC_LRELU, c->H2b.p, c->HL, true);
                    if (!rc) rc = run_linear_tc(c, OP_L3, Nt, tc::TC_LINEAR, c->LITb.p, 2 * Q, true); break;
            case 2: rc = run_linear_tc(c, OP_C1, Mt, tc::TC_LRELU, c->CHb.p, c->HC, true);
                    if (!rc) rc = run_linear_tc(c, OP_C2, Mt, tc::TC_LINEAR, c->COUTb.p, Q + F, true); break;
            case 3: rc = run_linear_tc(c, OP_U1, Nt, tc::TC_LRELU, c->U1b.p, c->HU, true);
                    if (!rc) rc = run_linear_tc(c, OP_U2, Nt, tc::TC_LRELU, c->U2b.p, c->HU, true);
                    if (!rc) rc = run_linear_tc(c, OP_U3, Nt, tc::TC_LINEAR, c->UOUTb.p, F, true); break;
            default: rc = run_linear_tc(c, OP_O1, Nt, tc::TC_LRELU, c->O1b.p, c->HO, true);
                     if (!rc) rc = run_linear_tc(c, OP_O2, Nt, tc::TC_LINEAR, c->LOGITS.p, DSAT_LOGIT_PAD, false); break;
        }
    } else
#endif
    {
        switch (which) {
            case 0: rc = run_linear(c, OP_V1, c->VROW.p, ldv, c->H1.p, ldh1, Nt, EPI_LRELU);
                    if (!rc) rc = run_linear(c, OP_Q2, c->H1.p, ldh1, c->QS.p, 3 * Q, Nt, EPI_QUERY); break;
            case 1: rc = run_linear(c, OP_V1, c->VROW.p, ldv, c->H1.p, ldh1, Nt, EPI_LRELU);
                    if (!rc) rc = run_linear(c, OP_L2, c->H1.p + c->HQ, ldh1, c->H2.p, c->HL, Nt, EPI_LRELU);
                    if (!rc) rc = run_linear(c, OP_L3, c->H2.p, c->HL, c->LIT.p, 2 * Q, Nt, EPI_LINEAR); break;
            case 2: rc = run_linear(c, OP_C1, c->CROW.p, ldc, c->CH.p, c->HC, Mt, EPI_LRELU);
                    if (!rc) rc = run_linear(c, OP_C2, c->CH.p, c->HC, c->COUT.p, Q + F, Mt, EPI_LINEAR); break;
            case 3: rc = run_linear(c, OP_U1, c->VROW.p, ldv, c->U1.p, c->HU, Nt, EPI_LRELU);
                    if (!rc) rc = run_linear(c, OP_U2, c->U1.p, c->HU, c->U2.p, c->HU, Nt, EPI_LRELU);
                    if (!rc) rc = run_linear(c, OP_U3, c->U2.p, c->HU, c->UOUT.p, F, Nt, EPI_LINEAR); break;
            default: rc = run_linear(c, OP_O1, c->SPRE.p, F, c->O1.p, c->HO, Nt, EPI_LRELU);
                     if (!rc) rc = run_linear(c, OP_O2, c->O1.p, c->HO, c->LOGITS.p, DSAT_LOGIT_PAD, Nt, EPI_LINEAR); break;
        }
    }
    if (rc) return rc;
    CK_CUDA(c, cudaStreamSynchronize(c->stream));
    return DSAT_OK;
}

int dsat_debug_groups(dsat_ctx* c, int32_t* done, int32_t* steps_taken, float* loss_sum, int32_t* graph_sat,
                      int32_t* graph_map) {
    if (!c) return DSAT_ERR_ARG;
    CK_ARG(c, c->has_buffers, "no buffers yet");
    CK_CUDA(c, cudaSetDevice(c->device));
    CK_CUDA(c, cudaStreamSynchronize(c->stream));
    if (done) CK_CUDA(c, dsat_memcpy_sync(done, c->done.p, c->n_groups * sizeof(int), cudaMemcpyDeviceToHost));
    if (steps_taken) CK_CUDA(c, dsat_memcpy_sync(steps_taken, c->steps_taken.p, c->n_groups * sizeof(int), cudaMemcpyDeviceToHost));
    if (loss_sum) CK_CUDA(c, dsat_memcpy_sync(loss_sum, c->loss_sum.p, c->n_groups * sizeof(float), cudaMemcpyDeviceToHost));
    if (graph_sat) CK_CUDA(c, dsat_memcpy_sync(graph_sat, c->graph_sat.p, c->total_graphs * sizeof(int), cudaMemcpyDeviceToHost));
    if (graph_map) CK_CUDA(c, dsat_memcpy_sync(graph_map, c->graph_map.p, c->total_graphs * sizeof(int), cudaMemcpyDeviceToHost));
    return DSAT_OK;
}

}
```

diffusionsat_b200/csrc/dsat_gemm_tc.cuh:

```cuda
#pragma once
#include <cuda.h>
#include "dsat_common.cuh"

namespace dsat {
namespace tc {

constexpr int BLOCK_M = 128;
constexpr int BLOCK_N = 256;
constexpr int BLOCK_K = 64;
constexpr int STAGES = 2;
constexpr int THREADS = 192;
constexpr int A_BYTES = BLOCK_M * BLOCK_K * 2;
constexpr int B_BYTES = BLOCK_N * BLOCK_K * 2;
constexpr int SMEM_BYTES = STAGES * (A_BYTES + B_BYTES) + 1024  + 256 ;

enum TcEpilogue : int { TC_LINEAR = 0, TC_LRELU = 1, TC_QUERY = 2 };

struct TcOut {
    void* ptr0; int ld0; int bf16_0;
    void* ptr1; int ld1; int bf16_1;
    int split;
};

__device__ __forceinline__ uint32_t smem_u32(const void* p) { return (uint32_t)__cvta_generic_to_shared(p); }

__device__ __forceinline__ void mbar_init(uint64_t* bar, uint32_t count) {
    asm volatile("mbarrier.init.shared::cta.b64 [%0], %1;" ::"r"(smem_u32(bar)), "r"(count));
}
__device__ __forceinline__ void mbar_expect_tx(uint64_t* bar, uint32_t bytes) {
    asm volatile("mbarrier.arrive.expect_tx.shared::cta.b64 _, [%0], %1;" ::"r"(smem_u32(bar)), "r"(bytes) : "memory");
}
__device__ __forceinline__ void mbar_wait(uint64_t* bar, uint32_t parity) {
    asm volatile(
        "{\n"
        ".reg .pred p;\n"
        "WAIT_LOOP:\n"
        "mbarrier.try_wait.parity.shared::cta.b64 p, [%0], %1;\n"
        "@p bra WAIT_DONE;\n"
        "bra WAIT_LOOP;\n"
        "WAIT_DONE:\n"
        "}\n" ::"r"(smem_u32(bar)), "r"(parity) : "memory");
}
__device__ __forceinline__ void tma_load_2d(void* smem_dst, const CUtensorMap* map, uint64_t* bar, int c0, int c1) {
    asm volatile(
        "cp.async.bulk.tensor.2d.shared::cluster.global.mbarrier::complete_tx::bytes [%0], [%1, {%3, %4}], [%2];"
        ::"r"(smem_u32(smem_dst)), "l"(map), "r"(smem_u32(bar)), "r"(c0), "r"(c1) : "memory");
}
__device__ __forceinline__ void tcgen05_commit(uint64_t* bar) {
    asm volatile("tcgen05.commit.cta_group::1.mbarrier::arrive::one.shared::cluster.b64 [%0];" ::"r"(smem_u32(bar)) : "memory");
}
__device__ __forceinline__ void tcgen05_fence_before() { asm volatile("tcgen05.fence::before_thread_sync;" ::: "memory"); }
__device__ __forceinline__ void tcgen05_fence_after() { asm volatile("tcgen05.fence::after_thread_sync;" ::: "memory"); }

__device__ __forceinline__ void umma_bf16(uint32_t tmem_d, uint64_t desc_a, uint64_t desc_b, uint32_t idesc, uint32_t accumulate) {
    asm volatile(
        "{\n"
        ".reg .pred p;\n"
        "setp.ne.b32 p, %4, 0;\n"
        "tcgen05.mma.cta_group::1.kind::f16 [%0], %1, %2, %3, p;\n"
        "}\n" ::"r"(tmem_d), "l"(desc_a), "l"(desc_b), "r"(idesc), "r"(accumulate) : "memory");
}

__device__ __forceinline__ void umma_bf16_elect(uint32_t tmem_d, uint64_t desc_a, uint64_t desc_b, uint32_t idesc, uint32_t accumulate) {
    asm volatile(
        "{\n"
        ".reg .pred p, q;\n"
        "setp.ne.b32 p, %4, 0;\n"
        "elect.sync _|q, 0xffffffff;\n"
        "@q tcgen05.mma.cta_group::1.kind::f16 [%0], %1, %2, %3, p;\n"
        "}\n" ::"r"(tmem_d), "l"(desc_a), "l"(desc_b), "r"(idesc), "r"(accumulate) : "memory");
}
__device__ __forceinline__ void umma_bf16_kblock_commit_elect(uint32_t tmem_d, uint64_t desc_a, uint64_t desc_b, uint32_t idesc,
                                                              uint32_t accumulate_first, uint64_t* slot_free_bar) {
    asm volatile(
        "{\n"
        ".reg .pred p, q, t;\n"
        ".reg .b64 a1, a2, a3, b1, b2, b3;\n"
        "setp.ne.b32 p, %4, 0;\n"
        "setp.eq.b32 t, 0, 0;\n"
        "add.s64 a1, %1, 2;\n add.s64 a2, %1, 4;\n add.s64 a3, %1, 6;\n"
        "add.s64 b1, %2, 2;\n add.s64 b2, %2, 4;\n add.s64 b3, %2, 6;\n"
        "elect.sync _|q, 0xffffffff;\n"
        "@q tcgen05.mma.cta_group::1.kind::f16 [%0], %1, %2, %3, p;\n"
        "@q tcgen05.mma.cta_group::1.kind::f16 [%0], a1, b1, %3, t;\n"
        "@q tcgen05.mma.cta_group::1.kind::f16 [%0], a2, b2, %3, t;\n"
        "@q tcgen05.mma.cta_group::1.kind::f16 [%0], a3, b3, %3, t;\n"
        "@q tcgen05.commit.cta_group::1.mbarrier::arrive::one.shared::cluster.b64 [%5];\n"
        "}\n" ::"r"(tmem_d), "l"(desc_a), "l"(desc_b), "r"(idesc), "r"(accumulate_first), "r"(smem_u32(slot_free_bar)) : "memory");
}
__device__ __forceinline__ uint32_t cluster_rank() {
    uint32_t r;
    asm volatile("mov.u32 %0, %%cluster_ctarank;" : "=r"(r));
    return r;
}
__device__ __forceinline__ void cluster_sync_all() {
    asm volatile("barrier.cluster.arrive.release.aligned;" ::: "memory");
    asm volatile("barrier.cluster.wait.acquire.aligned;" ::: "memory");
}
__device__ __forceinline__ uint32_t mapa_rank(uint32_t local_smem_addr, uint32_t rank) {
    uint32_t r;
    asm volatile("mapa.shared::cluster.u32 %0, %1, %2;" : "=r"(r) : "r"(local_smem_addr), "r"(rank));
    return r;
}
__device__ __forceinline__ void mbar_expect_tx_at(uint32_t cluster_addr, uint32_t bytes) {
    asm volatile("mbarrier.arrive.expect_tx.shared::cluster.b64 _, [%0], %1;" ::"r"(cluster_addr), "r"(bytes) : "memory");
}
__device__ __forceinline__ void mbar_arrive_at(uint32_t cluster_addr) {
    asm volatile("mbarrier.arrive.shared::cluster.b64 _, [%0];" ::"r"(cluster_addr) : "memory");
}
__device__ __forceinline__ void mbar_wait_cluster_scope(uint64_t* bar, uint32_t parity) {
    asm volatile(
        "{\n"
        ".reg .pred p;\n"
        "WAIT_LOOP_CS:\n"
        "mbarrier.try_wait.parity.acquire.cluster.shared::cta.b64 p, [%0], %1;\n"
        "@p bra WAIT_DONE_CS;\n"
        "bra WAIT_LOOP_CS;\n"
        "WAIT_DONE_CS:\n"
        "}\n" ::"r"(smem_u32(bar)), "r"(parity) : "memory");
}
__device__ __forceinline__ void tma_load_2d_cg2(void* smem_dst, const CUtensorMap* map, uint32_t bar_cluster_addr, int c0, int c1) {
    asm volatile(
        "cp.async.bulk.tensor.2d.cta_group::2.shared::cluster.global.mbarrier::complete_tx::bytes [%0], [%1, {%3, %4}], [%2];"
        ::"r"(smem_u32(smem_dst)), "l"(map), "r"(bar_cluster_addr), "r"(c0), "r"(c1) : "memory");
}
__device__ __forceinline__ void umma_bf16_elect_cg2(uint32_t tmem_d, uint64_t desc_a, uint64_t desc_b, uint32_t idesc, uint32_t accumulate) {
    asm volatile(
        "{\n"
        ".reg .pred p, q;\n"
        "setp.ne.b32 p, %4, 0;\n"
        "elect.sync _|q, 0xffffffff;\n"
        "@q tcgen05.mma.cta_group::2.kind::f16 [%0], %1, %2, %3, p;\n"
        "}\n" ::"r"(tmem_d), "l"(desc_a), "l"(desc_b), "r"(idesc), "r"(accumulate) : "memory");
}
__device__ __forceinline__ void tcgen05_commit_elect_cg2(uint64_t* bar) {
    asm volatile(
        "{\n"
        ".reg .pred q;\n"
        ".reg .b16 m;\n"
        "mov.b16 m, 3;\n"
        "elect.sync _|q, 0xffffffff;\n"
        "@q tcgen05.commit.cta_group::2.mbarrier::arrive::one.shared::cluster.multicast::cluster.b64 [%0], m;\n"
        "}\n" ::"r"(smem_u32(bar)) : "memory");
}
__device__ __forceinline__ void umma_bf16_kblock_commit_elect_cg2(uint32_t tmem_d, uint64_t desc_a, uint64_t desc_b, uint32_t idesc,
                                                                  uint32_t accumulate_first, uint64_t* slot_free_bar) {
    asm volatile(
        "{\n"
        ".reg .pred p, q, t;\n"
        ".reg .b64 a1, a2, a3, b1, b2, b3;\n"
        ".reg .b16 m;\n"
        "mov.b16 m, 3;\n"
        "setp.ne.b32 p, %4, 0;\n"
        "setp.eq.b32 t, 0, 0;\n"
        "add.s64 a1, %1, 2;\n add.s64 a2, %1, 4;\n add.s64 a3, %1, 6;\n"
        "add.s64 b1, %2, 2;\n add.s64 b2, %2, 4;\n add.s64 b3, %2, 6;\n"
        "elect.sync _|q, 0xffffffff;\n"
        "@q tcgen05.mma.cta_group::2.kind::f16 [%0], %1, %2, %3, p;\n"
        "@q tcgen05.mma.cta_group::2.kind::f16 [%0], a1, b1, %3, t;\n"
        "@q tcgen05.mma.cta_group::2.kind::f16 [%0], a2, b2, %3, t;\n"
        "@q tcgen05.mma.cta_group::2.kind::f16 [%0], a3, b3, %3, t;\n"
        "@q tcgen05.commit.cta_group::2.mbarrier::arrive::one.shared::cluster.multicast::cluster.b64 [%5], m;\n"
        "}\n" ::"r"(tmem_d), "l"(desc_a), "l"(desc_b), "r"(idesc), "r"(accumulate_first), "r"(smem_u32(slot_free_bar)) : "memory");
}
__device__ __forceinline__ void umma_bf16_kblock_elect(uint32_t tmem_d, uint64_t desc_a, uint64_t desc_b, uint32_t idesc,
                                                       uint32_t accumulate_first) {
    asm volatile(
        "{\n"
        ".reg .pred p, q, t;\n"
        ".reg .b64 a1, a2, a3, b1, b2, b3;\n"
        "setp.ne.b32 p, %4, 0;\n"
        "setp.eq.b32 t, 0, 0;\n"
        "add.s64 a1, %1, 2;\n add.s64 a2, %1, 4;\n add.s64 a3, %1, 6;\n"
        "add.s64 b1, %2, 2;\n add.s64 b2, %2, 4;\n add.s64 b3, %2, 6;\n"
        "elect.sync _|q, 0xffffffff;\n"
        "@q tcgen05.mma.cta_group::1.kind::f16 [%0], %1, %2, %3, p;\n"
        "@q tcgen05.mma.cta_group::1.kind::f16 [%0], a1, b1, %3, t;\n"
        "@q tcgen05.mma.cta_group::1.kind::f16 [%0], a2, b2, %3, t;\n"
        "@q tcgen05.mma.cta_group::1.kind::f16 [%0], a3, b3, %3, t;\n"
        "}\n" ::"r"(tmem_d), "l"(desc_a), "l"(desc_b), "r"(idesc), "r"(accumulate_first) : "memory");
}
__device__ __forceinline__ void umma_bf16_kblock_elect_cg2(uint32_t tmem_d, uint64_t desc_a, uint64_t desc_b, uint32_t idesc,
                                                           uint32_t accumulate_first) {
    asm volatile(
        "{\n"
        ".reg .pred p, q, t;\n"
        ".reg .b64 a1, a2, a3, b1, b2, b3;\n"
        "setp.ne.b32 p, %4, 0;\n"
        "setp.eq.b32 t, 0, 0;\n"
        "add.s64 a1, %1, 2;\n add.s64 a2, %1, 4;\n add.s64 a3, %1, 6;\n"
        "add.s64 b1, %2, 2;\n add.s64 b2, %2, 4;\n add.s64 b3, %2, 6;\n"
        "elect.sync _|q, 0xffffffff;\n"
        "@q tcgen05.mma.cta_group::2.kind::f16 [%0], %1, %2, %3, p;\n"
        "@q tcgen05.mma.cta_group::2.kind::f16 [%0], a1, b1, %3, t;\n"
        "@q tcgen05.mma.cta_group::2.kind::f16 [%0], a2, b2, %3, t;\n"
        "@q tcgen05.mma.cta_group::2.kind::f16 [%0], a3, b3, %3, t;\n"
        "}\n" ::"r"(tmem_d), "l"(desc_a), "l"(desc_b), "r"(idesc), "r"(accumulate_first) : "memory");
}
__device__ __forceinline__ void tcgen05_commit_elect(uint64_t* bar) {
    asm volatile(
        "{\n"
        ".reg .pred q;\n"
        "elect.sync _|q, 0xffffffff;\n"
        "@q tcgen05.commit.cta_group::1.mbarrier::arrive::one.shared::cluster.b64 [%0];\n"
        "}\n" ::"r"(smem_u32(bar)) : "memory");
}

__device__ __forceinline__ uint64_t make_smem_desc_sw128(uint32_t smem_addr) {
    uint64_t d = 0;
    d |= (uint64_t)((smem_addr & 0x3FFFF) >> 4);
    d |= (uint64_t)(1024 >> 4) << 32;
    d |= (uint64_t)1 << 46;
    d |= (uint64_t)2 << 61;
    return d;
}

__device__ __forceinline__ uint32_t make_idesc_bf16(int m, int n) {
    uint32_t d = 0;
    d |= 1u << 4;
    d |= 1u << 7;
    d |= 1u << 10;
    d |= (uint32_t)(n >> 3) << 17;
    d |= (uint32_t)(m >> 4) << 24;
    return d;
}

__device__ __forceinline__ void tmem_ld_32cols(uint32_t taddr, uint32_t (&r)[32]) {
    asm volatile(
        "tcgen05.ld.sync.aligned.32x32b.x32.b32 "
        "{%0, %1, %2, %3, %4, %5, %6, %7, %8, %9, %10, %11, %12, %13, %14, %15, "
        "%16, %17, %18, %19, %20, %21, %22, %23, %24, %25, %26, %27, %28, %29, %30, %31}, [%32];"
        : "=r"(r[0]), "=r"(r[1]), "=r"(r[2]), "=r"(r[3]), "=r"(r[4]), "=r"(r[5]), "=r"(r[6]), "=r"(r[7]),
          "=r"(r[8]), "=r"(r[9]), "=r"(r[10]), "=r"(r[11]), "=r"(r[12]), "=r"(r[13]), "=r"(r[14]), "=r"(r[15]),
          "=r"(r[16]), "=r"(r[17]), "=r"(r[18]), "=r"(r[19]), "=r"(r[20]), "=r"(r[21]), "=r"(r[22]), "=r"(r[23]),
          "=r"(r[24]), "=r"(r[25]), "=r"(r[26]), "=r"(r[27]), "=r"(r[28]), "=r"(r[29]), "=r"(r[30]), "=r"(r[31])
        : "r"(taddr));
    asm volatile("tcgen05.wait::ld.sync.aligned;" ::: "memory");
}

__device__ __forceinline__ void store_chunk(const TcOut& out, size_t row, int col, const float (&v)[32]) {
    const bool second = out.ptr1 != nullptr && col >= out.split;
    void* base = second ? out.ptr1 : out.ptr0;
    const int ld = second ? out.ld1 : out.ld0;
    const int c = second ? col - out.split : col;
    const int is_bf16 = second ? out.bf16_1 : out.bf16_0;
    if (is_bf16) {
        __nv_bfloat16* dst = reinterpret_cast<__nv_bfloat16*>(base) + row * ld + c;
#pragma unroll
        for (int j = 0; j < 4; ++j) {
            uint4 pack;
            __nv_bfloat162 p0 = __floats2bfloat162_rn(v[8 * j + 0], v[8 * j + 1]);
            __nv_bfloat162 p1 = __floats2bfloat162_rn(v[8 * j + 2], v[8 * j + 3]);
            __nv_bfloat162 p2 = __floats2bfloat162_rn(v[8 * j + 4], v[8 * j + 5]);
            __nv_bfloat162 p3 = __floats2bfloat162_rn(v[8 * j + 6], v[8 * j + 7]);
            pack.x = *reinterpret_cast<uint32_t*>(&p0); pack.y = *reinterpret_cast<uint32_t*>(&p1);
            pack.z = *reinterpret_cast<uint32_t*>(&p2); pack.w = *reinterpret_cast<uint32_t*>(&p3);
            reinterpret_cast<uint4*>(dst)[j] = pack;
        }
    } else {
        float* dst = reinterpret_cast<float*>(base) + row * ld + c;
#pragma unroll
        for (int j = 0; j < 8; ++j)
            reinterpret_cast<float4*>(dst)[j] = make_float4(v[4 * j], v[4 * j + 1], v[4 * j + 2], v[4 * j + 3]);
    }
}

__global__ void __launch_bounds__(THREADS, 2)
tc_linear_kernel(const __grid_constant__ CUtensorMap map_a, const __grid_constant__ CUtensorMap map_b,
                 const float* __restrict__ bias, TcOut out, int rows, int K, int N, int n_tiles, int epi, int qmaps,
                 int a_box_rows, int b_box_rows) {
    extern __shared__ uint8_t smem_raw[];
    uint8_t* smem = reinterpret_cast<uint8_t*>((reinterpret_cast<uintptr_t>(smem_raw) + 1023) & ~(uintptr_t)1023);
    uint8_t* smem_a = smem;
    uint8_t* smem_b = smem + STAGES * A_BYTES;
    uint64_t* full_bar = reinterpret_cast<uint64_t*>(smem + STAGES * (A_BYTES + B_BYTES));
    uint64_t* empty_bar = full_bar + STAGES;
    uint64_t* tmem_full_bar = empty_bar + STAGES;
    uint32_t* tmem_slot = reinterpret_cast<uint32_t*>(tmem_full_bar + 1);

    const int warp = threadIdx.x >> 5, lane = threadIdx.x & 31;
    const int row0 = (blockIdx.x / n_tiles) * BLOCK_M;
    const int n0 = (blockIdx.x % n_tiles) * BLOCK_N;
    const int bn = min(BLOCK_N, N - n0);
    const int k_blocks = (K + BLOCK_K - 1) / BLOCK_K;

    if (threadIdx.x == 0) {
#pragma unroll
        for (int s = 0; s < STAGES; ++s) { mbar_init(&full_bar[s], 1); mbar_init(&empty_bar[s], 1); }
        mbar_init(tmem_full_bar, 1);
        asm volatile("fence.mbarrier_init.release.cluster;" ::: "memory");
        asm volatile("prefetch.tensormap [%0];" ::"l"(&map_a) : "memory");
        asm volatile("prefetch.tensormap [%0];" ::"l"(&map_b) : "memory");
    }
    if (warp == 1) {
        asm volatile("tcgen05.alloc.cta_group::1.sync.aligned.shared::cta.b32 [%0], %1;" ::"r"(smem_u32(tmem_slot)), "n"(BLOCK_N));
        asm volatile("tcgen05.relinquish_alloc_permit.cta_group::1.sync.aligned;");
    }
    tcgen05_fence_before();
    __syncthreads();
    tcgen05_fence_after();
    const uint32_t tmem_base = *tmem_slot;

    if (warp == 0) {
        if (lane == 0) {
            for (int kb = 0; kb < k_blocks; ++kb) {
                const int s = kb % STAGES;
                const uint32_t phase = (kb / STAGES) & 1;
                mbar_wait(&empty_bar[s], phase ^ 1);
                mbar_expect_tx(&full_bar[s], (uint32_t)(a_box_rows + b_box_rows) * (BLOCK_K * 2));
                tma_load_2d(smem_a + s * A_BYTES, &map_a, &full_bar[s], kb * BLOCK_K, row0);
                tma_load_2d(smem_b + s * B_BYTES, &map_b, &full_bar[s], kb * BLOCK_K, n0);
            }
        }
    } else if (warp == 1) {
        if (lane == 0) {
            const uint32_t idesc = make_idesc_bf16(BLOCK_M, bn);
            for (int kb = 0; kb < k_blocks; ++kb) {
                const int s = kb % STAGES;
                const uint32_t phase = (kb / STAGES) & 1;
                mbar_wait(&full_bar[s], phase);
                tcgen05_fence_after();
                const uint64_t da = make_smem_desc_sw128(smem_u32(smem_a + s * A_BYTES));
                const uint64_t db = make_smem_desc_sw128(smem_u32(smem_b + s * B_BYTES));
                const int ksteps = min(BLOCK_K / 16, (K - kb * BLOCK_K + 15) / 16);
                for (int k = 0; k < ksteps; ++k) {
                    umma_bf16(tmem_base, da + (uint64_t)(2 * k), db + (uint64_t)(2 * k), idesc, (kb | k) != 0);
                }
                tcgen05_commit(&empty_bar[s]);
            }
            tcgen05_commit(tmem_full_bar);
        }
    } else {
        const int quad = warp & 3;
        const size_t row = (size_t)row0 + quad * 32 + lane;
        mbar_wait(tmem_full_bar, 0);
        tcgen05_fence_after();
        for (int c = 0; c < bn; c += 32) {
            uint32_t raw[32];
            tmem_ld_32cols(tmem_base + ((uint32_t)(quad * 32) << 16) + (uint32_t)c, raw);
            if (row < (size_t)rows) {
                float v[32];
                const int col = n0 + c;
#pragma unroll
                for (int j = 0; j < 32; ++j) {
                    float x = __uint_as_float(raw[j]) + ((col + j < N) ? __ldg(bias + col + j) : 0.f);
                    if (epi == TC_LRELU) x = x > 0.f ? x : 0.2f * x;
                    v[j] = x;
                }
                const int valid = min(32, bn - c);
                if (valid == 32) {
                    store_chunk(out, row, col, v);
                    if (epi == TC_QUERY) {
                        float sp[32], sn[32];
#pragma unroll
                        for (int j = 0; j < 32; ++j) {
                            const float tail = __logf(1.0f + __expf(-fabsf(v[j])));
                            sp[j] = fmaxf(v[j], 0.f) + tail;
                            sn[j] = fmaxf(-v[j], 0.f) + tail;
                        }
                        store_chunk(out, row, col + qmaps, sp);
                        store_chunk(out, row, col + 2 * qmaps, sn);
                    }
                } else {
                    const bool second = out.ptr1 != nullptr && col >= out.split;
                    void* base = second ? out.ptr1 : out.ptr0;
                    const int ld = second ? out.ld1 : out.ld0;
                    const int cc = second ? col - out.split : col;
                    const int is_bf16 = second ? out.bf16_1 : out.bf16_0;
                    for (int j = 0; j < valid; ++j) {
                        if (is_bf16) reinterpret_cast<__nv_bfloat16*>(base)[row * ld + cc + j] = __float2bfloat16_rn(v[j]);
                        else reinterpret_cast<float*>(base)[row * ld + cc + j] = v[j];
                    }
                }
            }
        }
        tcgen05_fence_before();
    }
    __syncthreads();
    if (warp == 1) {
        tcgen05_fence_after();
        asm volatile("tcgen05.dealloc.cta_group::1.sync.aligned.b32 %0, %1;" ::"r"(tmem_base), "n"(BLOCK_N));
    }
}

typedef CUresult (*EncodeTiledFn)(CUtensorMap*, CUtensorMapDataType, cuuint32_t, void*, const cuuint64_t*,
                                  const cuuint64_t*, const cuuint32_t*, const cuuint32_t*, CUtensorMapInterleave,
                                  CUtensorMapSwizzle, CUtensorMapL2promotion, CUtensorMapFloatOOBfill);

inline EncodeTiledFn encode_tiled_fn() {
    static EncodeTiledFn fn = nullptr;
    if (!fn) {
        void* p = nullptr;
        cudaDriverEntryPointQueryResult q;
        if (cudaGetDriverEntryPoint("cuTensorMapEncodeTiled", &p, cudaEnableDefault, &q) == cudaSuccess &&
            q == cudaDriverEntryPointSuccess)
            fn = reinterpret_cast<EncodeTiledFn>(p);
    }
    return fn;
}

inline bool make_bf16_map(CUtensorMap* map, const void* base, long long rows, int cols, int ld, int box_rows) {
    EncodeTiledFn fn = encode_tiled_fn();
    if (!fn) return false;
    cuuint64_t dims[2] = {(cuuint64_t)cols, (cuuint64_t)rows};
    cuuint64_t strides[1] = {(cuuint64_t)ld * 2};
    cuuint32_t box[2] = {(cuuint32_t)BLOCK_K, (cuuint32_t)box_rows};
    cuuint32_t estr[2] = {1, 1};
    CUresult r = fn(map, CU_TENSOR_MAP_DATA_TYPE_BFLOAT16, 2, const_cast<void*>(base), dims, strides, box, estr,
                    CU_TENSOR_MAP_INTERLEAVE_NONE, CU_TENSOR_MAP_SWIZZLE_128B, CU_TENSOR_MAP_L2_PROMOTION_L2_256B,
                    CU_TENSOR_MAP_FLOAT_OOB_FILL_NONE);
    return r == CUDA_SUCCESS;
}

struct TcLinear {
    CUtensorMap map_a, map_b;
    const float* bias;
    TcOut out;
    int rows, K, N, epi, qmaps;
    int a_box_rows, b_box_rows;
};

inline cudaError_t configure_tc_device() {
    static PerDeviceOnce configured;
    if (configured.done()) return cudaSuccess;
    cudaError_t e = cudaFuncSetAttribute(tc_linear_kernel, cudaFuncAttributeMaxDynamicSharedMemorySize, SMEM_BYTES);
    if (e == cudaSuccess) configured.mark();
    return e;
}

inline cudaError_t launch_tc_linear(const TcLinear& op, cudaStream_t stream) {
    if (op.rows <= 0) return cudaSuccess;
    {
        cudaError_t e = configure_tc_device();
        if (e != cudaSuccess) return e;
    }
    const int n_tiles = ceil_div(op.N, BLOCK_N);
    const unsigned grid = (unsigned)(n_tiles * ceil_div(op.rows, BLOCK_M));
    tc_linear_kernel<<<grid, THREADS, SMEM_BYTES, stream>>>(op.map_a, op.map_b, op.bias, op.out, op.rows, op.K, op.N,
                                                             n_tiles, op.epi, op.qmaps, op.a_box_rows, op.b_box_rows);
    return cudaGetLastError();
}

}
}
```

diffusionsat_b200/csrc/dsat_mlp_fused.cuh:

```cuda
#pragma once
#include "dsat_gemm_tc.cuh"

namespace dsat {
namespace fm {

using tc::TcOut;

constexpr int BLOCK_M = 128;
constexpr int BLOCK_K = 64;
constexpr int MAX_THREADS = 320;
constexpr int MAX_LAYERS = 3;
constexpr int MAX_SLOTS = 8;
constexpr int AH_BLOCK_BYTES = BLOCK_M * BLOCK_K * 2;
constexpr int TMEM_COLS = 512;
constexpr int STAGE_ROW = 128 + 16;
constexpr int BAR_BYTES = 512;
constexpr int MAX_A_SLOTS = 8;
constexpr int SMEM_LIMIT = 227 * 1024;
#ifndef DSAT_EPI_SERIAL_HIDDEN
#define DSAT_EPI_SERIAL_HIDDEN 0
#endif

struct FmLayer {
    int K, N;
    int epi;
    int box_rows;
    int bias_off;
    const float* bias;
};

struct FmStep {
    short layer, n0, N;
    char hidden;
    char wait_next;
};
constexpr int MAX_STEPS = 6;

struct FmParams {
    int n_layers;
    FmLayer layer[MAX_LAYERS];
    int rows, n_tiles, a_box_rows, ah_blocks, slots, slot_bytes, two_bufs, qmaps;
    int dbg;
    int pair;
    int pp;
    int stage_in_h;
    int stage_off;
    int a_slots;
    int stage_row;
    int bias_total;
    int smem_pad;
    int epi_warps;
    int step_bias;
    int split;
    int n_steps;
    FmStep step[MAX_STEPS];
    TcOut out;
    long long* prof;
};

#define DSAT_TIMED_WAIT(acc, call)                 \
    do {                                           \
        if (timing) {                              \
            const long long t0__ = clock64();      \
            call;                                  \
            acc += clock64() - t0__;               \
        } else {                                   \
            call;                                  \
        }                                          \
    } while (0)

__device__ __forceinline__ void sts128(uint32_t addr, const uint4& v) {
    asm volatile("st.shared.v4.b32 [%0], {%1, %2, %3, %4};" ::"r"(addr), "r"(v.x), "r"(v.y), "r"(v.z), "r"(v.w));
}
__device__ __forceinline__ uint4 lds128(uint32_t addr) {
    uint4 v;
    asm volatile("ld.shared.v4.b32 {%0, %1, %2, %3}, [%4];" : "=r"(v.x), "=r"(v.y), "=r"(v.z), "=r"(v.w) : "r"(addr));
    return v;
}
__device__ __forceinline__ float4 lds128f(uint32_t addr) {
    float4 v;
    asm volatile("ld.shared.v4.f32 {%0, %1, %2, %3}, [%4];" : "=f"(v.x), "=f"(v.y), "=f"(v.z), "=f"(v.w) : "r"(addr));
    return v;
}
__device__ __forceinline__ void tmem_ld_32cols_async(uint32_t taddr, uint32_t (&r)[32]) {
    asm volatile(
        "tcgen05.ld.sync.aligned.32x32b.x32.b32 "
        "{%0, %1, %2, %3, %4, %5, %6, %7, %8, %9, %10, %11, %12, %13, %14, %15, "
        "%16, %17, %18, %19, %20, %21, %22, %23, %24, %25, %26, %27, %28, %29, %30, %31}, [%32];"
        : "=r"(r[0]), "=r"(r[1]), "=r"(r[2]), "=r"(r[3]), "=r"(r[4]), "=r"(r[5]), "=r"(r[6]), "=r"(r[7]),
          "=r"(r[8]), "=r"(r[9]), "=r"(r[10]), "=r"(r[11]), "=r"(r[12]), "=r"(r[13]), "=r"(r[14]), "=r"(r[15]),
          "=r"(r[16]), "=r"(r[17]), "=r"(r[18]), "=r"(r[19]), "=r"(r[20]), "=r"(r[21]), "=r"(r[22]), "=r"(r[23]),
          "=r"(r[24]), "=r"(r[25]), "=r"(r[26]), "=r"(r[27]), "=r"(r[28]), "=r"(r[29]), "=r"(r[30]), "=r"(r[31])
        : "r"(taddr));
}
__device__ __forceinline__ void tmem_ld_wait(uint32_t (&r)[32]) {
    asm volatile("tcgen05.wait::ld.sync.aligned;"
                 : "+r"(r[0]), "+r"(r[1]), "+r"(r[2]), "+r"(r[3]), "+r"(r[4]), "+r"(r[5]), "+r"(r[6]), "+r"(r[7]),
                   "+r"(r[8]), "+r"(r[9]), "+r"(r[10]), "+r"(r[11]), "+r"(r[12]), "+r"(r[13]), "+r"(r[14]), "+r"(r[15]),
                   "+r"(r[16]), "+r"(r[17]), "+r"(r[18]), "+r"(r[19]), "+r"(r[20]), "+r"(r[21]), "+r"(r[22]), "+r"(r[23]),
                   "+r"(r[24]), "+r"(r[25]), "+r"(r[26]), "+r"(r[27]), "+r"(r[28]), "+r"(r[29]), "+r"(r[30]), "+r"(r[31]));
}

__device__ __forceinline__ uint4 pack8_bf16(const float* v) {
    __nv_bfloat162 p0 = __floats2bfloat162_rn(v[0], v[1]), p1 = __floats2bfloat162_rn(v[2], v[3]);
    __nv_bfloat162 p2 = __floats2bfloat162_rn(v[4], v[5]), p3 = __floats2bfloat162_rn(v[6], v[7]);
    uint4 pack;
    pack.x = *reinterpret_cast<uint32_t*>(&p0); pack.y = *reinterpret_cast<uint32_t*>(&p1);
    pack.z = *reinterpret_cast<uint32_t*>(&p2); pack.w = *reinterpret_cast<uint32_t*>(&p3);
    return pack;
}

__device__ __forceinline__ void bias_act_chunk(const uint32_t (&raw)[32], uint32_t bias_addr, bool lrelu, float (&v)[32]) {
#pragma unroll
    for (int q = 0; q < 8; ++q) {
        const float4 b = lds128f(bias_addr + 16 * q);
        const float x0 = __uint_as_float(raw[4 * q]) + b.x, x1 = __uint_as_float(raw[4 * q + 1]) + b.y;
        const float x2 = __uint_as_float(raw[4 * q + 2]) + b.z, x3 = __uint_as_float(raw[4 * q + 3]) + b.w;
        v[4 * q] = lrelu ? fmaxf(x0, 0.2f * x0) : x0;
        v[4 * q + 1] = lrelu ? fmaxf(x1, 0.2f * x1) : x1;
        v[4 * q + 2] = lrelu ? fmaxf(x2, 0.2f * x2) : x2;
        v[4 * q + 3] = lrelu ? fmaxf(x3, 0.2f * x3) : x3;
    }
}

__device__ __forceinline__ void bias_act_chunk_bf16(const uint32_t (&raw)[32], uint32_t bias_f_addr, bool lrelu, uint4 (&out)[4]) {
    const __nv_bfloat162 slope = __floats2bfloat162_rn(0.2f, 0.2f);
#pragma unroll
    for (int q = 0; q < 4; ++q) {
        const float4 b0 = lds128f(bias_f_addr + 32 * q), b1 = lds128f(bias_f_addr + 32 * q + 16);
        const float bb[8] = {b0.x, b0.y, b0.z, b0.w, b1.x, b1.y, b1.z, b1.w};
        uint32_t ow[4];
#pragma unroll
        for (int i = 0; i < 4; ++i) {
            __nv_bfloat162 x = __floats2bfloat162_rn(__uint_as_float(raw[8 * q + 2 * i]) + bb[2 * i],
                                                     __uint_as_float(raw[8 * q + 2 * i + 1]) + bb[2 * i + 1]);
            if (lrelu) x = __hmax2(x, __hmul2(x, slope));
            ow[i] = *reinterpret_cast<uint32_t*>(&x);
        }
        out[q] = make_uint4(ow[0], ow[1], ow[2], ow[3]);
    }
}

__device__ __forceinline__ void store_chunk_packed(uint32_t stage_addr, int stage_row, int lane, const uint4 (&w)[4], int valid,
                                                   uint8_t* gbase, size_t row_pitch_bytes, size_t row_first,
                                                   int rows_left, int col) {
    const uint32_t mine = stage_addr + lane * stage_row;
#pragma unroll
    for (int q = 0; q < 4; ++q) sts128(mine + 16 * q, w[q]);
    __syncwarp();
    const int valid_pieces = valid / 8;
    uint4 t[4];
#pragma unroll
    for (int k = 0; k < 4; ++k) {
        const int pidx = lane + 32 * k;
        t[k] = lds128(stage_addr + (pidx >> 2) * stage_row + 16 * (pidx & 3));
    }
    uint8_t* g0 = gbase + row_first * row_pitch_bytes + (size_t)col * 2;
#pragma unroll
    for (int k = 0; k < 4; ++k) {
        const int pidx = lane + 32 * k;
        const int rr = pidx >> 2, piece = pidx & 3;
        if (rr < rows_left && piece < valid_pieces)
            *reinterpret_cast<uint4*>(g0 + (size_t)rr * row_pitch_bytes + 16 * piece) = t[k];
    }
    __syncwarp();
}

template <bool BF16>
__device__ __forceinline__ void store_chunk_fast(uint32_t stage_addr, int stage_row, int lane, const float (&v)[32], int valid,
                                                 uint8_t* gbase, size_t row_pitch_bytes, size_t row_first,
                                                 int rows_left, int col) {
    const uint32_t mine = stage_addr + lane * stage_row;
    if (BF16) {
#pragma unroll
        for (int q = 0; q < 4; ++q) sts128(mine + 16 * q, pack8_bf16(&v[8 * q]));
    } else {
#pragma unroll
        for (int q = 0; q < 8; ++q) {
            uint4 w;
            w.x = __float_as_uint(v[4 * q]); w.y = __float_as_uint(v[4 * q + 1]);
            w.z = __float_as_uint(v[4 * q + 2]); w.w = __float_as_uint(v[4 * q + 3]);
            sts128(mine + 16 * q, w);
        }
    }
    __syncwarp();
    constexpr int ES = BF16 ? 2 : 4;
    constexpr int PIECES = BF16 ? 4 : 8;
    const int valid_pieces = valid * ES / 16;
    uint4 t[PIECES];
#pragma unroll
    for (int k = 0; k < PIECES; ++k) {
        const int pidx = lane + 32 * k;
        t[k] = lds128(stage_addr + (pidx / PIECES) * stage_row + 16 * (pidx % PIECES));
    }
    uint8_t* g0 = gbase + row_first * row_pitch_bytes + (size_t)col * ES;
#pragma unroll
    for (int k = 0; k < PIECES; ++k) {
        const int pidx = lane + 32 * k;
        const int rr = pidx / PIECES, piece = pidx % PIECES;
        if (rr < rows_left && piece < valid_pieces)
            *reinterpret_cast<uint4*>(g0 + (size_t)rr * row_pitch_bytes + 16 * piece) = t[k];
    }
    __syncwarp();
}

struct EpiCtx {
    uint32_t lane_addr, ah_addr, bl_addr, stage_addr;
    int N, epi, cpar, cstep, r, lane, qmaps, stage_row;
    size_t row_first; int rows_left;
    void* ptr0; void* ptr1; int ld0, ld1, bf0, bf1, split;
    bool skip;
};

template <bool HIDDEN>
__device__ __forceinline__ void epi_process(const EpiCtx& e, const uint32_t (&raw)[32], int c) {
    const bool lrelu = e.epi == tc::TC_LRELU;
    if (HIDDEN) {
        uint4 w[4];
        bias_act_chunk_bf16(raw, e.bl_addr + 4u * (uint32_t)c, lrelu, w);
        const uint32_t blk = e.ah_addr + (uint32_t)(c >> 6) * AH_BLOCK_BYTES + (uint32_t)e.r * 128;
        const int j0 = (c & 63) >> 3;
#pragma unroll
        for (int q = 0; q < 4; ++q)
            if (c + 8 * q < e.N) sts128(blk + (uint32_t)(((j0 + q) ^ (e.r & 7)) << 4), w[q]);
        return;
    }
    const bool second = e.ptr1 != nullptr && c >= e.split;
    uint8_t* gbase = reinterpret_cast<uint8_t*>(second ? e.ptr1 : e.ptr0);
    const int is_bf16 = second ? e.bf1 : e.bf0;
    const size_t pitch = (size_t)(second ? e.ld1 : e.ld0) * (is_bf16 ? 2 : 4);
    const int cc = second ? c - e.split : c;
    const int valid = min(32, e.N - c);
    if (is_bf16 && e.epi != tc::TC_QUERY) {
        uint4 w[4];
        bias_act_chunk_bf16(raw, e.bl_addr + 4u * (uint32_t)c, lrelu, w);
        store_chunk_packed(e.stage_addr, e.stage_row, e.lane, w, valid, gbase, pitch, e.row_first, e.rows_left, cc);
        return;
    }
    float v[32];
    bias_act_chunk(raw, e.bl_addr + 4u * (uint32_t)c, lrelu, v);
    if (is_bf16) store_chunk_fast<true>(e.stage_addr, e.stage_row, e.lane, v, valid, gbase, pitch, e.row_first, e.rows_left, cc);
    else store_chunk_fast<false>(e.stage_addr, e.stage_row, e.lane, v, valid, gbase, pitch, e.row_first, e.rows_left, cc);
    if (e.epi == tc::TC_QUERY) {
        float sp[32], sn[32];
#pragma unroll
        for (int i = 0; i < 32; ++i) {
            const float t = __logf(1.0f + __expf(-fabsf(v[i])));
            sp[i] = fmaxf(v[i], 0.f) + t;
            sn[i] = fmaxf(-v[i], 0.f) + t;
        }
        if (is_bf16) {
            store_chunk_fast<true>(e.stage_addr, e.stage_row, e.lane, sp, valid, gbase, pitch, e.row_first, e.rows_left, cc + e.qmaps);
            store_chunk_fast<true>(e.stage_addr, e.stage_row, e.lane, sn, valid, gbase, pitch, e.row_first, e.rows_left, cc + 2 * e.qmaps);
        } else {
            store_chunk_fast<false>(e.stage_addr, e.stage_row, e.lane, sp, valid, gbase, pitch, e.row_first, e.rows_left, cc + e.qmaps);
            store_chunk_fast<false>(e.stage_addr, e.stage_row, e.lane, sn, valid, gbase, pitch, e.row_first, e.rows_left, cc + 2 * e.qmaps);
        }
    }
}

template <bool PAIR>
__device__ __forceinline__ void arrive_addr(uint32_t addr) {
    if constexpr (PAIR) tc::mbar_arrive_at(addr);
    else asm volatile("mbarrier.arrive.shared::cta.b64 _, [%0];" ::"r"(addr) : "memory");
}

template <bool PAIR>
__device__ __forceinline__ void warp_arrive(uint32_t addr, int lane) {
    __syncwarp();
    if (lane == 0) arrive_addr<PAIR>(addr);
}

template <bool HIDDEN, bool PAIR>
__device__ __forceinline__ void epi_drain(const EpiCtx& e, uint32_t tmem_empty_addr) {
    bool released = false;
    if (e.skip) {
        if (!HIDDEN) { tc::tcgen05_fence_before(); warp_arrive<PAIR>(tmem_empty_addr, e.lane); }
        return;
    }
    if constexpr (!HIDDEN || DSAT_EPI_SERIAL_HIDDEN) {
#pragma unroll 1
        for (int c = 32 * e.cpar; c < e.N; c += e.cstep) {
            uint32_t ra[32];
            tmem_ld_32cols_async(e.lane_addr + (uint32_t)c, ra);
            tmem_ld_wait(ra);
            if (!HIDDEN && c + e.cstep >= e.N) {
                tc::tcgen05_fence_before();
                warp_arrive<PAIR>(tmem_empty_addr, e.lane);
                released = true;
            }
            epi_process<HIDDEN>(e, ra, c);
        }
    } else {
        int c = 32 * e.cpar;
        if (c < e.N) {
            uint32_t ra[32], rb[32];
            tmem_ld_32cols_async(e.lane_addr + (uint32_t)c, ra);
#pragma unroll 1
            while (true) {
                tmem_ld_wait(ra);
                const int c1 = c + e.cstep;
                if (c1 < e.N) tmem_ld_32cols_async(e.lane_addr + (uint32_t)c1, rb);
                epi_process<HIDDEN>(e, ra, c);
                if (c1 >= e.N) break;
                tmem_ld_wait(rb);
                c = c1 + e.cstep;
                if (c < e.N) tmem_ld_32cols_async(e.lane_addr + (uint32_t)c, ra);
                epi_process<HIDDEN>(e, rb, c1);
                if (c >= e.N) break;
            }
        }
    }
    if (!HIDDEN && !released) { tc::tcgen05_fence_before(); warp_arrive<PAIR>(tmem_empty_addr, e.lane); }
}

template <bool TIMING, bool PAIR>
__global__ void __launch_bounds__(MAX_THREADS, 1)
fused_mlp_kernel(const __grid_constant__ CUtensorMap map_a, const __grid_constant__ CUtensorMap map_w0, const __grid_constant__ CUtensorMap map_w1,
                 const __grid_constant__ CUtensorMap map_w2, FmParams p) {
    using namespace tc;
    extern __shared__ __align__(1024) uint8_t smem_raw[];
    uint8_t* smem = reinterpret_cast<uint8_t*>((reinterpret_cast<uintptr_t>(smem_raw) + 1023) & ~(uintptr_t)1023);
    if ((int)(smem - smem_raw) > p.smem_pad) __trap();
    uint8_t* ah = smem;
    const size_t h_bytes = (size_t)p.ah_blocks * AH_BLOCK_BYTES;
    uint8_t* a_ring = smem + (p.pp ? 2 : 1) * h_bytes;
    uint8_t* ring = a_ring + (size_t)p.a_slots * AH_BLOCK_BYTES;
    uint8_t* stage_all = ring + (size_t)p.slots * p.slot_bytes;
    uint8_t* tail = stage_all + (p.stage_in_h ? 0 : (size_t)p.epi_warps * 32 * p.stage_row);
    uint64_t* a_full = reinterpret_cast<uint64_t*>(tail);
    uint64_t* ah_free = a_full + 1;
    uint64_t* h_full = a_full + 2;
    uint64_t* tmem_full = a_full + 4;
    uint64_t* tmem_empty = a_full + 6;
    uint64_t* ring_full = a_full + 8;
    uint64_t* ring_empty = a_full + 8 + MAX_SLOTS;
    uint64_t* a_ring_full = a_full + 8 + 2 * MAX_SLOTS;
    uint64_t* a_ring_empty = a_ring_full + MAX_A_SLOTS;
    uint32_t* tmem_slot = reinterpret_cast<uint32_t*>(a_ring_empty + MAX_A_SLOTS);
    float* bias_s = reinterpret_cast<float*>(tail + BAR_BYTES);

    const int warp = threadIdx.x >> 5, lane = threadIdx.x & 31;
    const int epi_threads = 32 * p.epi_warps;
    const CUtensorMap* map_w[MAX_LAYERS] = {&map_w0, &map_w1, &map_w2};
    const bool timing = TIMING && p.prof != nullptr && blockIdx.x == 0;
    const long long t_kernel0 = timing ? clock64() : 0;
    long long w0 = 0, w1 = 0, w2 = 0, w3 = 0, w4 = 0, w5 = 0, w6 = 0, w7 = 0;

    const uint32_t rank = PAIR ? cluster_rank() : 0u;
    const bool leader = rank == 0;
    const bool pair_wait_cta_scope = (p.dbg & 2) == 0;
    constexpr int NC = PAIR ? 2 : 1;
    if (threadIdx.x == 0) {
        mbar_init(a_full, NC);
        mbar_init(ah_free, 1);
        for (int b = 0; b < 2; ++b) {
            mbar_init(&h_full[b], NC * p.epi_warps);
            mbar_init(&tmem_full[b], 1);
            mbar_init(&tmem_empty[b], NC * p.epi_warps);
        }
        for (int s = 0; s < MAX_SLOTS; ++s) { mbar_init(&ring_full[s], NC); mbar_init(&ring_empty[s], 1); }
        for (int s = 0; s < MAX_A_SLOTS; ++s) { mbar_init(&a_ring_full[s], NC); mbar_init(&a_ring_empty[s], 1); }
        asm volatile("fence.mbarrier_init.release.cluster;" ::: "memory");
        asm volatile("prefetch.tensormap [%0];" ::"l"(&map_a) : "memory");
        asm volatile("prefetch.tensormap [%0];" ::"l"(&map_w0) : "memory");
        asm volatile("prefetch.tensormap [%0];" ::"l"(&map_w1) : "memory");
        asm volatile("prefetch.tensormap [%0];" ::"l"(&map_w2) : "memory");
    }
    if (warp == 1) {
        if constexpr (PAIR) {
            asm volatile("tcgen05.alloc.cta_group::2.sync.aligned.shared::cta.b32 [%0], %1;" ::"r"(smem_u32(tmem_slot)), "n"(TMEM_COLS));
            asm volatile("tcgen05.relinquish_alloc_permit.cta_group::2.sync.aligned;");
        } else {
            asm volatile("tcgen05.alloc.cta_group::1.sync.aligned.shared::cta.b32 [%0], %1;" ::"r"(smem_u32(tmem_slot)), "n"(TMEM_COLS));
            asm volatile("tcgen05.relinquish_alloc_permit.cta_group::1.sync.aligned;");
        }
    }
    if (warp >= 2) {
        for (int l = 0; l < p.n_layers; ++l)
            for (int i = threadIdx.x - 64; i < p.layer[l].N; i += epi_threads) {
                bias_s[p.layer[l].bias_off + i] = __ldg(p.layer[l].bias + i);
            }
    }
    tcgen05_fence_before();
    __syncthreads();
    if constexpr (PAIR) cluster_sync_all();
    tcgen05_fence_after();
    const uint32_t tmem_base = *tmem_slot;
    const int n_layers = p.n_layers;
    auto wait = [&](uint64_t* bar, uint32_t parity) {
        if constexpr (PAIR) { if (pair_wait_cta_scope) mbar_wait(bar, parity); else mbar_wait_cluster_scope(bar, parity); }
        else mbar_wait(bar, parity);
    };
    auto wait_async = [&](uint64_t* bar, uint32_t parity) {
        if constexpr (PAIR) { if (pair_wait_cta_scope) mbar_wait(bar, parity); else mbar_wait_cluster_scope(bar, parity); }
        else mbar_wait(bar, parity);
    };
    auto at_leader = [&](uint64_t* bar) -> uint32_t { return PAIR ? mapa_rank(smem_u32(bar), 0) : smem_u32(bar); };
    const int unit0 = PAIR ? (int)(blockIdx.x >> 1) : (int)blockIdx.x;
    const int unit_stride = PAIR ? (int)(gridDim.x >> 1) : (int)gridDim.x;
    const int n_units = PAIR ? (p.n_tiles + 1) / 2 : p.n_tiles;
    const int nt = unit0 < n_units ? (n_units - unit0 + unit_stride - 1) / unit_stride : 0;
    auto tile_of = [&](int j) { const int u = unit0 + j * unit_stride; return PAIR ? 2 * u + (int)rank : u; };
    const int group = p.pp ? 2 : 1;
// ... 627 lines not shown
```

diffusionsat_b200/csrc/dsat_mlp_x3.cuh:

```cuda
#pragma once
#include "dsat_mlp_fused.cuh"

namespace dsat {
namespace x3 {

constexpr int BLOCK_M = 128;
constexpr int BLOCK_K = 64;
constexpr int BLK_BYTES = BLOCK_M * BLOCK_K * 2;
constexpr int MAX_LAYERS = 3;
constexpr int MAX_RING = 8;
constexpr int TMEM_COLS = 512;
constexpr int STAGE_ROW = 128 + 16;
constexpr int BAR_BYTES = 512;
constexpr int SMEM_LIMIT = 227 * 1024;

enum OutMode : int { OUT_F32 = 0, OUT_SPLIT = 1 };

struct X3Layer {
    int K, N;
    int epi;
    int w_lo_row;
    int bias_off;
    int n_total;
    const float* bias;
};

struct X3Params {
    int n_layers;
    X3Layer layer[MAX_LAYERS];
    int rows, n_tiles, n_groups, a_box_rows;
    int h_blocks;
    int a_slots, w_slots, w_slot_bytes;
    int epi_warps, stage_in_h, smem_pad, bias_total, qmaps, pair;
    int out_mode;
    void* out0; void* out1; int ld_out;
    long long* prof;
    const int* done; int rows_per_chain, chains_per_group;
};

__device__ __forceinline__ void split2(float v0, float v1, uint32_t& hi, uint32_t& lo) { split_bf16x2(v0, v1, hi, lo); }

struct Epi {
    uint32_t lane_addr, h_addr, bl_addr, stage_addr;
    int N, epi, cpar, cstep, r, lane, qmaps, col0, h_plane_bytes;
    size_t row_first; int rows_left;
    void* out0; void* out1; int ld_out, out_mode;
};

__device__ __forceinline__ void epi_hidden(const Epi& e, const uint32_t (&raw)[32], int c) {
    float v[32];
    fm::bias_act_chunk(raw, e.bl_addr + 4u * (uint32_t)c, e.epi == tc::TC_LRELU, v);
    const uint32_t blk = e.h_addr + (uint32_t)(c >> 6) * BLK_BYTES + (uint32_t)e.r * 128;
    const int j0 = (c & 63) >> 3;
#pragma unroll
    for (int q = 0; q < 4; ++q) {
        uint4 hi, lo;
        split2(v[8 * q], v[8 * q + 1], hi.x, lo.x);
        split2(v[8 * q + 2], v[8 * q + 3], hi.y, lo.y);
        split2(v[8 * q + 4], v[8 * q + 5], hi.z, lo.z);
        split2(v[8 * q + 6], v[8 * q + 7], hi.w, lo.w);
        if (c + 8 * q < e.N) {
            const uint32_t at = blk + (uint32_t)(((j0 + q) ^ (e.r & 7)) << 4);
            fm::sts128(at, hi);
            fm::sts128(at + (uint32_t)e.h_plane_bytes, lo);
        }
    }
}

__device__ __forceinline__ void epi_final(const Epi& e, const uint32_t (&raw)[32], int c) {
    float v[32];
    fm::bias_act_chunk(raw, e.bl_addr + 4u * (uint32_t)c, e.epi == tc::TC_LRELU, v);
    const int valid = min(32, e.N - c);
    const int col = e.col0 + c;
    if (e.out_mode == OUT_SPLIT) {
        uint4 hi[4], lo[4];
#pragma unroll
        for (int q = 0; q < 4; ++q) {
            split2(v[8 * q], v[8 * q + 1], hi[q].x, lo[q].x);
            split2(v[8 * q + 2], v[8 * q + 3], hi[q].y, lo[q].y);
            split2(v[8 * q + 4], v[8 * q + 5], hi[q].z, lo[q].z);
            split2(v[8 * q + 6], v[8 * q + 7], hi[q].w, lo[q].w);
        }
        const size_t pitch = (size_t)e.ld_out * 2;
        fm::store_chunk_packed(e.stage_addr, STAGE_ROW, e.lane, hi, valid, reinterpret_cast<uint8_t*>(e.out0), pitch, e.row_first, e.rows_left, col);
        fm::store_chunk_packed(e.stage_addr, STAGE_ROW, e.lane, lo, valid, reinterpret_cast<uint8_t*>(e.out1), pitch, e.row_first, e.rows_left, col);
        return;
    }
    uint8_t* gbase = reinterpret_cast<uint8_t*>(e.out0);
    const size_t pitch = (size_t)e.ld_out * 4;
    fm::store_chunk_fast<false>(e.stage_addr, STAGE_ROW, e.lane, v, valid, gbase, pitch, e.row_first, e.rows_left, col);
    if (e.epi == tc::TC_QUERY) {
        float sp[32], sn[32];
#pragma unroll
        for (int i = 0; i < 32; ++i) {
            const float t = __logf(1.0f + __expf(-fabsf(v[i])));
            sp[i] = fmaxf(v[i], 0.f) + t;
            sn[i] = fmaxf(-v[i], 0.f) + t;
        }
        fm::store_chunk_fast<false>(e.stage_addr, STAGE_ROW, e.lane, sp, valid, gbase, pitch, e.row_first, e.rows_left, col + e.qmaps);
        fm::store_chunk_fast<false>(e.stage_addr, STAGE_ROW, e.lane, sn, valid, gbase, pitch, e.row_first, e.rows_left, col + 2 * e.qmaps);
    }
}

template <bool PAIR>
__global__ void __launch_bounds__(64 + 32 * 8, 1)
x3_mlp_kernel(const __grid_constant__ CUtensorMap map_a_hi, const __grid_constant__ CUtensorMap map_a_lo,
              const __grid_constant__ CUtensorMap map_w0, const __grid_constant__ CUtensorMap map_w1,
              const __grid_constant__ CUtensorMap map_w2, X3Params p) {
    using namespace tc;
    extern __shared__ __align__(1024) uint8_t smem_raw[];
    uint8_t* smem = reinterpret_cast<uint8_t*>((reinterpret_cast<uintptr_t>(smem_raw) + 1023) & ~(uintptr_t)1023);
    if ((int)(smem - smem_raw) > p.smem_pad) __trap();
    const int h_plane_bytes = p.h_blocks * BLK_BYTES;
    uint8_t* hid = smem;
    uint8_t* a_ring = smem + 2 * (size_t)h_plane_bytes;
    uint8_t* w_ring = a_ring + (size_t)p.a_slots * BLK_BYTES;
    uint8_t* stage_all = w_ring + (size_t)p.w_slots * p.w_slot_bytes;
    uint8_t* tail = stage_all + (p.stage_in_h ? 0 : (size_t)p.epi_warps * 32 * STAGE_ROW);
    uint64_t* a_full = reinterpret_cast<uint64_t*>(tail);
    uint64_t* a_empty = a_full + MAX_RING;
    uint64_t* w_full = a_empty + MAX_RING;
    uint64_t* w_empty = w_full + MAX_RING;
    uint64_t* tmem_full = w_empty + MAX_RING;
    uint64_t* tmem_empty = tmem_full + 2;
    uint64_t* h_full = tmem_empty + 2;
    uint32_t* tmem_slot = reinterpret_cast<uint32_t*>(h_full + 1);
    float* bias_s = reinterpret_cast<float*>(tail + BAR_BYTES);

    const int warp = threadIdx.x >> 5, lane = threadIdx.x & 31;
    const int epi_threads = 32 * p.epi_warps;
    const CUtensorMap* map_w[MAX_LAYERS] = {&map_w0, &map_w1, &map_w2};
    const CUtensorMap* map_a[2] = {&map_a_hi, &map_a_lo};
    const uint32_t rank = PAIR ? cluster_rank() : 0u;
    const bool leader = rank == 0;
    constexpr int NC = PAIR ? 2 : 1;
    const bool timing = p.prof != nullptr && blockIdx.x == 0;

    if (threadIdx.x == 0) {
        for (int s = 0; s < MAX_RING; ++s) {
            mbar_init(&a_full[s], NC); mbar_init(&a_empty[s], 1);
            mbar_init(&w_full[s], NC); mbar_init(&w_empty[s], 1);
        }
        for (int b = 0; b < 2; ++b) { mbar_init(&tmem_full[b], 1); mbar_init(&tmem_empty[b], NC * p.epi_warps); }
        mbar_init(h_full, NC * p.epi_warps);
        asm volatile("fence.mbarrier_init.release.cluster;" ::: "memory");
        asm volatile("prefetch.tensormap [%0];" ::"l"(&map_a_hi) : "memory");
        asm volatile("prefetch.tensormap [%0];" ::"l"(&map_a_lo) : "memory");
        asm volatile("prefetch.tensormap [%0];" ::"l"(&map_w0) : "memory");
        asm volatile("prefetch.tensormap [%0];" ::"l"(&map_w1) : "memory");
        asm volatile("prefetch.tensormap [%0];" ::"l"(&map_w2) : "memory");
    }
    if (warp == 1) {
        if constexpr (PAIR) {
            asm volatile("tcgen05.alloc.cta_group::2.sync.aligned.shared::cta.b32 [%0], %1;" ::"r"(smem_u32(tmem_slot)), "n"(TMEM_COLS));
            asm volatile("tcgen05.relinquish_alloc_permit.cta_group::2.sync.aligned;");
        } else {
            asm volatile("tcgen05.alloc.cta_group::1.sync.aligned.shared::cta.b32 [%0], %1;" ::"r"(smem_u32(tmem_slot)), "n"(TMEM_COLS));
            asm volatile("tcgen05.relinquish_alloc_permit.cta_group::1.sync.aligned;");
        }
    }
    if (warp >= 2 && warp < 2 + p.epi_warps) {
        for (int l = 0; l < p.n_layers; ++l)
            for (int i = threadIdx.x - 64; i < p.layer[l].n_total; i += epi_threads) bias_s[p.layer[l].bias_off + i] = __ldg(p.layer[l].bias + i);
    }
    tcgen05_fence_before();
    __syncthreads();
    if constexpr (PAIR) cluster_sync_all();
    tcgen05_fence_after();
    const uint32_t tmem_base = *tmem_slot;
    const int L = p.n_layers, G = p.n_groups;
    auto at_leader = [&](uint64_t* bar) -> uint32_t { return PAIR ? mapa_rank(smem_u32(bar), 0) : smem_u32(bar); };
    const int unit0 = PAIR ? (int)(blockIdx.x >> 1) : (int)blockIdx.x;
    const int unit_stride = PAIR ? (int)(gridDim.x >> 1) : (int)gridDim.x;
    const int n_units = (PAIR ? (p.n_tiles + 1) / 2 : p.n_tiles) * G;
    const int nt = unit0 < n_units ? (n_units - unit0 + unit_stride - 1) / unit_stride : 0;
    auto tile_of = [&](int j) { const int u = (unit0 + j * unit_stride) / G; return PAIR ? 2 * u + (int)rank : u; };
    auto group_of = [&](int j) { return (unit0 + j * unit_stride) % G; };
    constexpr int SKIP_UNITS = 1024;
    uint32_t* skip_bits = reinterpret_cast<uint32_t*>(tail + 384);
    const bool skipping = p.done != nullptr && nt <= SKIP_UNITS;
    if (skipping) {
        for (int base = 32 * warp; base < nt; base += (int)blockDim.x) {
            const int j = base + lane;
            bool all = false;
            if (j < nt) {
                const int u = (unit0 + j * unit_stride) / G;
                const int r0 = (PAIR ? 2 * u : u) * BLOCK_M;
                int r1 = r0 + (PAIR ? 2 * BLOCK_M : BLOCK_M);
                r1 = (r1 < p.rows ? r1 : p.rows) - 1;
                const int g0 = (r0 / p.rows_per_chain) / p.chains_per_group, g1 = (r1 / p.rows_per_chain) / p.chains_per_group;
                all = true;
                for (int g = g0; g <= g1 && all; ++g) all = __ldg(p.done + g) != 0;
            }
            const uint32_t bits = __ballot_sync(0xffffffffu, all);
            if (lane == 0) skip_bits[base >> 5] = bits;
        }
        __syncthreads();
    }
    auto unit_done = [&](int j) -> bool { return skipping && ((skip_bits[j >> 5] >> (j & 31)) & 1u) != 0; };

    if (warp == 0) {
        if (lane == 0) {
            int as = 0, ws = 0; uint32_t aph = 0, wph = 0;
            for (int j = 0; j < nt; ++j) {
                if (unit_done(j)) continue;
                const int tile = tile_of(j), grp = group_of(j);
                for (int l = 0; l < L; ++l) {
                    const X3Layer& ly = p.layer[l];
                    const int kbs = (ly.K + BLOCK_K - 1) / BLOCK_K;
                    const int wrows = PAIR ? ly.N / 2 : ly.N;
                    for (int kb = 0; kb < kbs; ++kb) {
                        if (l == 0) {
                            for (int pl = 0; pl < 2; ++pl) {
                                mbar_wait(&a_empty[as], aph ^ 1);
                                uint8_t* dst = a_ring + (size_t)as * BLK_BYTES;
                                if constexpr (PAIR) {
                                    mbar_expect_tx_at(at_leader(&a_full[as]), (uint32_t)p.a_box_rows * (BLOCK_K * 2));
                                    tma_load_2d_cg2(dst, map_a[pl], at_leader(&a_full[as]), kb * BLOCK_K, tile * BLOCK_M);
                                } else {
                                    mbar_expect_tx(&a_full[as], (uint32_t)p.a_box_rows * (BLOCK_K * 2));
                                    tma_load_2d(dst, map_a[pl], &a_full[as], kb * BLOCK_K, tile * BLOCK_M);
                                }
                                if (++as == p.a_slots) { as = 0; aph ^= 1; }
                            }
                        }
                        for (int pl = 0; pl < 2; ++pl) {
                            mbar_wait(&w_empty[ws], wph ^ 1);
                            uint8_t* dst = w_ring + (size_t)ws * p.w_slot_bytes;
                            const int row = pl * ly.w_lo_row + grp * 256 + (int)rank * wrows;
                            if constexpr (PAIR) {
                                mbar_expect_tx_at(at_leader(&w_full[ws]), (uint32_t)wrows * (BLOCK_K * 2));
                                tma_load_2d_cg2(dst, map_w[l], at_leader(&w_full[ws]), kb * BLOCK_K, row);
                            } else {
                                mbar_expect_tx(&w_full[ws], (uint32_t)wrows * (BLOCK_K * 2));
                                tma_load_2d(dst, map_w[l], &w_full[ws], kb * BLOCK_K, row);
                            }
                            if (++ws == p.w_slots) { ws = 0; wph ^= 1; }
                        }
                    }
                }
            }
        }
    } else if (warp == 1) {
        if (leader) {
            int as = 0, ws = 0; uint32_t aph = 0, wph = 0;
            long long t_wait_acc = 0, t_wait_h = 0, t_wait_a = 0, t_wait_w = 0;
            const long long t_begin = timing ? clock64() : 0;
            auto commit = [&](uint64_t* bar) { if constexpr (PAIR) tcgen05_commit_elect_cg2(bar); else tcgen05_commit_elect(bar); };
            auto kblock = [&](uint32_t acc, uint64_t da, uint64_t db, uint32_t idesc, uint32_t accum, int ksteps, uint64_t* free_bar) {
                if (ksteps == BLOCK_K / 16) {
                    if (free_bar) {
                        if constexpr (PAIR) umma_bf16_kblock_commit_elect_cg2(acc, da, db, idesc, accum, free_bar);
                        else umma_bf16_kblock_commit_elect(acc, da, db, idesc, accum, free_bar);
                    } else {
                        if constexpr (PAIR) umma_bf16_kblock_elect_cg2(acc, da, db, idesc, accum);
                        else umma_bf16_kblock_elect(acc, da, db, idesc, accum);
                    }
                } else {
                    for (int k = 0; k < ksteps; ++k) {
                        if constexpr (PAIR) umma_bf16_elect_cg2(acc, da + (uint64_t)(2 * k), db + (uint64_t)(2 * k), idesc, (accum | (uint32_t)k) != 0);
                        else umma_bf16_elect(acc, da + (uint64_t)(2 * k), db + (uint64_t)(2 * k), idesc, (accum | (uint32_t)k) != 0);
                    }
                    if (free_bar) commit(free_bar);
                }
            };
#define X3_WAIT(acc_t, call) do { if (timing) { const long long t0__ = clock64(); call; acc_t += clock64() - t0__; } else { call; } } while (0)
            int jp = 0;
            for (int j = 0; j < nt; ++j) {
                if (unit_done(j)) continue;
                for (int l = 0; l < L; ++l) {
                    const int g = jp * L + l, buf = g & 1, use = g >> 1;
                    X3_WAIT(t_wait_acc, mbar_wait(&tmem_empty[buf], (uint32_t)((use & 1) ^ 1)));
                    if (l > 0) X3_WAIT(t_wait_h, mbar_wait(h_full, (uint32_t)((jp * (L - 1) + (l - 1)) & 1)));
                    tcgen05_fence_after();
                    const int K = p.layer[l].K, N = p.layer[l].N;
                    const int kbs = (K + BLOCK_K - 1) / BLOCK_K;
                    const uint32_t idesc = make_idesc_bf16(PAIR ? 2 * BLOCK_M : BLOCK_M, N);
                    const uint32_t acc = tmem_base + (uint32_t)(buf * 256);
                    for (int kb = 0; kb < kbs; ++kb) {
                        const int ksteps = min(BLOCK_K / 16, (K - kb * BLOCK_K + 15) / 16);
                        uint64_t da_hi, da_lo;
                        int as_hi = 0, as_lo = 0;
                        if (l == 0) {
                            as_hi = as;
                            const uint32_t ph_hi = aph;
                            if (++as == p.a_slots) { as = 0; aph ^= 1; }
                            as_lo = as;
                            const uint32_t ph_lo = aph;
                            if (++as == p.a_slots) { as = 0; aph ^= 1; }
                            X3_WAIT(t_wait_a, mbar_wait(&a_full[as_hi], ph_hi));
                            X3_WAIT(t_wait_a, mbar_wait(&a_full[as_lo], ph_lo));
                            da_hi = make_smem_desc_sw128(smem_u32(a_ring + (size_t)as_hi * BLK_BYTES));
                            da_lo = make_smem_desc_sw128(smem_u32(a_ring + (size_t)as_lo * BLK_BYTES));
                        } else {
                            da_hi = make_smem_desc_sw128(smem_u32(hid + (size_t)kb * BLK_BYTES));
                            da_lo = make_smem_desc_sw128(smem_u32(hid + (size_t)h_plane_bytes + (size_t)kb * BLK_BYTES));
                        }
                        X3_WAIT(t_wait_w, mbar_wait(&w_full[ws], wph));
                        uint64_t db = make_smem_desc_sw128(smem_u32(w_ring + (size_t)ws * p.w_slot_bytes));
                        kblock(acc, da_hi, db, idesc, kb != 0, ksteps, nullptr);
                        kblock(acc, da_lo, db, idesc, 1u, ksteps, &w_empty[ws]);
                        if (++ws == p.w_slots) { ws = 0; wph ^= 1; }
                        X3_WAIT(t_wait_w, mbar_wait(&w_full[ws], wph));
                        db = make_smem_desc_sw128(smem_u32(w_ring + (size_t)ws * p.w_slot_bytes));
                        kblock(acc, da_hi, db, idesc, 1u, ksteps, &w_empty[ws]);
                        if (++ws == p.w_slots) { ws = 0; wph ^= 1; }
                        if (l == 0) { commit(&a_empty[as_hi]); commit(&a_empty[as_lo]); }
                    }
                    commit(&tmem_full[buf]);
                }
                ++jp;
            }
#undef X3_WAIT
            if (timing && lane == 0) {
                p.prof[0] = clock64() - t_begin; p.prof[1] = t_wait_acc; p.prof[2] = t_wait_h; p.prof[3] = t_wait_a; p.prof[4] = t_wait_w;
            }
        }
    } else if (warp < 2 + p.epi_warps) {
        const int quad = warp & 3;
        Epi e;
        e.r = quad * 32 + lane;
        e.lane = lane;
        e.cpar = (warp - 2) >> 2;
        e.cstep = 32 * (p.epi_warps >> 2);
        e.qmaps = p.qmaps;
        e.out0 = p.out0; e.out1 = p.out1; e.ld_out = p.ld_out; e.out_mode = p.out_mode;
        e.h_plane_bytes = h_plane_bytes;
        e.h_addr = smem_u32(hid);
        const uint32_t bias_addr0 = smem_u32(bias_s);
        e.stage_addr = (p.stage_in_h ? smem_u32(hid) : smem_u32(stage_all)) + (uint32_t)(warp - 2) * (32 * STAGE_ROW);
        long long t_wait_full = 0, t_hidden = 0, t_final = 0;
        int jp = -1;
        for (int j = 0; j < nt; ++j) {
            if (unit_done(j)) continue;
            ++jp;
            const int tile = tile_of(j), grp = group_of(j);
            DSAT_CHECK(tile >= 0 && (tile < p.n_tiles || (PAIR && tile == p.n_tiles)) && grp >= 0 && grp < G);
            e.row_first = (size_t)tile * BLOCK_M + quad * 32;
            e.rows_left = p.rows - (int)e.row_first;
            e.col0 = grp * 256;
            for (int l = 0; l < L; ++l) {
                const int g = jp * L + l, buf = g & 1, use = g >> 1;
                e.N = p.layer[l].N; e.epi = p.layer[l].epi;
                e.bl_addr = bias_addr0 + 4u * (uint32_t)(p.layer[l].bias_off + grp * 256);
                e.lane_addr = tmem_base + ((uint32_t)(quad * 32) << 16) + (uint32_t)(buf * 256);
                const long long t0 = timing ? clock64() : 0;
                mbar_wait(&tmem_full[buf], (uint32_t)(use & 1));
                tcgen05_fence_after();
                const long long t1 = timing ? clock64() : 0;
                const uint32_t empty_addr = at_leader(&tmem_empty[buf]);
                if (l + 1 < L) {
                    int c = 32 * e.cpar;
                    if (c < e.N) {
                        uint32_t ra[32], rb[32];
                        fm::tmem_ld_32cols_async(e.lane_addr + (uint32_t)c, ra);
#pragma unroll 1
                        while (true) {
                            fm::tmem_ld_wait(ra);
                            const int c1 = c + e.cstep;
                            if (c1 < e.N) fm::tmem_ld_32cols_async(e.lane_addr + (uint32_t)c1, rb);
                            epi_hidden(e, ra, c);
                            if (c1 >= e.N) break;
                            fm::tmem_ld_wait(rb);
                            c = c1 + e.cstep;
                            if (c < e.N) fm::tmem_ld_32cols_async(e.lane_addr + (uint32_t)c, ra);
                            epi_hidden(e, rb, c1);
                            if (c >= e.N) break;
                        }
                    }
                    tcgen05_fence_before();
                    asm volatile("fence.proxy.async.shared::cta;" ::: "memory");
                    __syncwarp();
                    if (lane == 0) { fm::arrive_addr<PAIR>(empty_addr); fm::arrive_addr<PAIR>(at_leader(h_full)); }
                    if (timing) t_hidden += clock64() - t1;
                } else {
                    bool released = false;
#pragma unroll 1
                    for (int c = 32 * e.cpar; c < e.N; c += e.cstep) {
                        uint32_t ra[32];
                        fm::tmem_ld_32cols_async(e.lane_addr + (uint32_t)c, ra);
                        fm::tmem_ld_wait(ra);
                        if (c + e.cstep >= e.N) {
                            tcgen05_fence_before();
                            fm::warp_arrive<PAIR>(empty_addr, lane);
                            released = true;
                        }
                        epi_final(e, ra, c);
                    }
                    if (!released) { tcgen05_fence_before(); fm::warp_arrive<PAIR>(empty_addr, lane); }
                    if (p.stage_in_h) asm volatile("bar.sync 1, %0;" ::"r"(epi_threads) : "memory");
                    if (timing) t_final += clock64() - t1;
                }
                if (timing) t_wait_full += t1 - t0;
            }
        }
        if (timing && warp == 2 && lane == 0) { p.prof[5] = t_wait_full; p.prof[6] = t_hidden; p.prof[7] = t_final; }
    }
    tcgen05_fence_before();
    __syncthreads();
    if constexpr (PAIR) cluster_sync_all();
    if (warp == 1) {
        tcgen05_fence_after();
        if constexpr (PAIR) asm volatile("tcgen05.dealloc.cta_group::2.sync.aligned.b32 %0, %1;" ::"r"(tmem_base), "n"(TMEM_COLS));
        else asm volatile("tcgen05.dealloc.cta_group::1.sync.aligned.b32 %0, %1;" ::"r"(tmem_base), "n"(TMEM_COLS));
    }
}

struct X3Mlp {
    CUtensorMap map_a_hi, map_a_lo;
    CUtensorMap map_w[MAX_LAYERS];
    X3Params p;
    int smem_bytes = 0;
    bool pair_mode = false;
    bool four_epilogue_warps = false;
    bool ready = false;
};

inline int env_int(const char* name, int dflt) { const char* e = getenv(name); return e ? atoi(e) : dflt; }

inline bool plan_x3(X3Mlp& f) {
    X3Params& p = f.p;
    const int pad = fm::dyn_smem_pad();
    p.smem_pad = pad;
    int bias_total = 0, max_n = 0, h_blocks = 0;
    bool pair = f.pair_mode && p.rows > BLOCK_M;
    for (int l = 0; l < p.n_layers; ++l) {
        X3Layer& ly = p.layer[l];
        if (ly.N > 256 || ly.N % 16 || ly.K % 16) return false;
        if (l + 1 < p.n_layers) h_blocks = max(h_blocks, (ly.N + 63) / 64);
        ly.bias_off = bias_total;
        bias_total += (ly.n_total + 31) / 32 * 32;
        max_n = max(max_n, ly.N);
    }
    if (p.n_groups > 1 && p.n_layers != 1) return false;
    p.pair = pair ? 1 : 0;
    p.h_blocks = h_blocks;
    p.bias_total = bias_total;
    p.n_tiles = ceil_div(p.rows, BLOCK_M);
    p.w_slot_bytes = ((pair ? max_n / 2 : max_n) * BLOCK_K * 2 + 1023) / 1024 * 1024;
    for (int ew : {8, 4}) {
        if (ew == 8 && f.four_epilogue_warps) continue;
        const int stage_bytes = ew * 32 * STAGE_ROW;
        const int in_h = 2 * h_blocks * BLK_BYTES >= stage_bytes;
        const int fixed = pad + 2 * h_blocks * BLK_BYTES + (in_h ? 0 : stage_bytes) + BAR_BYTES + bias_total * 4;
        int avail = SMEM_LIMIT - fixed;
        int a = 2, w = 2;
        if (avail < a * BLK_BYTES + w * p.w_slot_bytes) continue;
        avail -= a * BLK_BYTES + w * p.w_slot_bytes;
        if (p.n_layers > 1) {
            const int a_want = min(MAX_RING, 2 * ((p.layer[0].K + BLOCK_K - 1) / BLOCK_K));
            while (a < a_want && avail >= BLK_BYTES) { ++a; avail -= BLK_BYTES; }
            while (w < MAX_RING && avail >= p.w_slot_bytes) { ++w; avail -= p.w_slot_bytes; }
        } else {
            while (true) {
                bool grew = false;
                if (a <= w && a < MAX_RING && avail >= BLK_BYTES) { ++a; avail -= BLK_BYTES; grew = true; }
                else if (w < MAX_RING && avail >= p.w_slot_bytes) { ++w; avail -= p.w_slot_bytes; grew = true; }
                else if (a < MAX_RING && avail >= BLK_BYTES) { ++a; avail -= BLK_BYTES; grew = true; }
                if (!grew) break;
            }
        }
        const int ea = env_int("DSAT_X3_A_SLOTS", 0), ewn = env_int("DSAT_X3_W_SLOTS", 0);
        if (ea >= 2 && ewn >= 2 && ea <= MAX_RING && ewn <= MAX_RING &&
            fixed + ea * BLK_BYTES + ewn * p.w_slot_bytes <= SMEM_LIMIT) { a = ea; w = ewn; }
        p.a_slots = a; p.w_slots = w; p.epi_warps = ew; p.stage_in_h = in_h;
        f.smem_bytes = fixed + a * BLK_BYTES + w * p.w_slot_bytes;
        f.ready = true;
        return true;
    }
    return false;
}

inline cudaError_t configure_x3_device(int) {
    static PerDeviceOnce configured;
    if (configured.done()) return cudaSuccess;
    cudaError_t e = cudaFuncSetAttribute(x3_mlp_kernel<false>, cudaFuncAttributeMaxDynamicSharedMemorySize, SMEM_LIMIT);
    if (e == cudaSuccess) e = cudaFuncSetAttribute(x3_mlp_kernel<true>, cudaFuncAttributeMaxDynamicSharedMemorySize, SMEM_LIMIT);
    if (e == cudaSuccess) configured.mark();
    return e;
}

inline cudaError_t launch_x3(const X3Mlp& f, int device, int sm_count, cudaStream_t stream) {
    if (f.p.rows <= 0) return cudaSuccess;
    cudaError_t e = configure_x3_device(device);
    if (e != cudaSuccess) return e;
    const unsigned threads = 64 + 32 * f.p.epi_warps;
    if (f.p.pair) {
        const int n_units = (f.p.n_tiles + 1) / 2 * f.p.n_groups;
        const int pairs = n_units < sm_count / 2 ? n_units : sm_count / 2;
        cudaLaunchConfig_t cfg = {};
        cfg.gridDim = dim3(2 * pairs); cfg.blockDim = dim3(threads); cfg.dynamicSmemBytes = (size_t)f.smem_bytes; cfg.stream = stream;
        cudaLaunchAttribute attr[1];
        attr[0].id = cudaLaunchAttributeClusterDimension;
        attr[0].val.clusterDim.x = 2; attr[0].val.clusterDim.y = 1; attr[0].val.clusterDim.z = 1;
        cfg.attrs = attr; cfg.numAttrs = 1;
        return cudaLaunchKernelEx(&cfg, x3_mlp_kernel<true>, f.map_a_hi, f.map_a_lo, f.map_w[0], f.map_w[1], f.map_w[2], f.p);
    }
    const int n_units = f.p.n_tiles * f.p.n_groups;
    const unsigned grid = (unsigned)(n_units < sm_count ? n_units : sm_count);
    x3_mlp_kernel<false><<<grid, threads, f.smem_bytes, stream>>>(f.map_a_hi, f.map_a_lo, f.map_w[0], f.map_w[1], f.map_w[2], f.p);
    return cudaGetLastError();
}

}
}
```

Before: 682.2.

## Keep fused-MLP hidden activations in TMEM and feed next layer via TS MMA

Hidden-layer activations of the fused x3 MLP kernel are now written back into tensor memory (split hi/lo bf16) instead of swizzled shared memory. The next layer's MMA reads its A operand directly from TMEM (tcgen05.mma with a TMEM A operand), with two half-release barriers so the MMA warp can start on the low half early. This frees the shared memory used for hidden blocks, allowing larger input/weight rings (MAX_RING raised to 12). The split-per-layer launch path for clause and update MLPs is removed. The risks are TMEM column pressure and stricter ordering between epilogue TMEM stores and MMA reads.

```diff
diff --git a/diffusionsat_b200/csrc/dsat_api.cu b/diffusionsat_b200/csrc/dsat_api.cu
--- a/diffusionsat_b200/csrc/dsat_api.cu
+++ b/diffusionsat_b200/csrc/dsat_api.cu
@@ -135,9 +135,6 @@
     bool use_fused = true;
     bool use_smem_gather = true;
     DevBuf<__nv_bfloat16> VROWp, CROWp, SPREp, H1p, H2p;
-    DevBuf<__nv_bfloat16> CHp, U1p, U2p;
-    x3::X3Mlp x3s[5];
-    bool split_clause = false, split_update = false;
     DevBuf<__nv_bfloat16> wx[12];
     int wx_k64[12] = {0}, wx_n[12] = {0};
     x3::X3Mlp x3[7];
@@ -459,7 +456,6 @@
     c->O1b.drop();
     c->has_tc_buffers = false;
     c->VROWp.drop(); c->CROWp.drop(); c->SPREp.drop(); c->H1p.drop(); c->H2p.drop();
-    c->CHp.drop(); c->U1p.drop(); c->U2p.drop();
     c->has_x3_buffers = false;
 #endif
     c->has_buffers = false;
@@ -482,7 +478,6 @@
     c->O1b.release();
     c->has_tc_buffers = false;
     c->VROWp.release(); c->CROWp.release(); c->SPREp.release(); c->H1p.release(); c->H2p.release();
-    c->CHp.release(); c->U1p.release(); c->U2p.release();
     c->has_x3_buffers = false;
 #endif
     c->has_buffers = false;
@@ -587,9 +582,8 @@
         }
         for (; i < x3::MAX_LAYERS; ++i) f.map_w[i] = f.map_w[0];
         if (getenv("DSAT_PLAN_LOG"))
-            fprintf(stderr, "[dsat] x3 mlp %d: smem %d B, hidden blocks 2 x %d, input ring %d, weight ring %d x %d B, epilogue warps %d, "
-                    "staging in hidden %d, cta pair %d, groups %d\n", which, f.smem_bytes, p.h_blocks, p.a_slots, p.w_slots, p.w_slot_bytes,
-                    p.epi_warps, p.stage_in_h, p.pair, p.n_groups);
+            fprintf(stderr, "[dsat] x3 mlp %d: smem %d B, input ring %d, weight ring %d x %d B, epilogue warps %d, cta pair %d, groups %d\n",
+                    which, f.smem_bytes, p.a_slots, p.w_slots, p.w_slot_bytes, p.epi_warps, p.pair, p.n_groups);
         return true;
     };
     const size_t vplane = Nt * c->ldv(), cplane = Mt * c->ldc(), splane = Nt * F, hplane = Nt * c->HL;
@@ -616,40 +610,6 @@
     else ok = false;
     ok = ok && build(XO, c->SPREp.p, splane, c->Nt, F, F,
                      {{10, OP_O1, 0, tc::TC_LRELU}, {11, OP_O2, 0, tc::TC_LINEAR}}, 1, x3::OUT_F32, c->LOGITS.p, nullptr, DSAT_LOGIT_PAD);
-    {
-        static const int split_mask = getenv("DSAT_X3_SPLIT") ? atoi(getenv("DSAT_X3_SPLIT")) : 1;
-        c->split_clause = c->split_update = false;
-        if (ok && (split_mask & 1)) {
-            const size_t chplane = Mt * c->HC;
-            CK_CUDA(c, c->CHp.alloc(2 * chplane));
-            x3::X3Mlp keep_c = c->x3[XC];
-            bool k = build(XC, c->CROWp.p, cplane, c->Mt, F + 2 * Q, c->ldc(), {{5, OP_C1, 0, tc::TC_LRELU}}, 1, x3::OUT_SPLIT,
-                           c->CHp.p, c->CHp.p + chplane, c->HC);
-            c->x3s[0] = c->x3[XC];
-            k = k && build(XC, c->CHp.p, chplane, c->Mt, c->HC, c->HC, {{6, OP_C2, 0, tc::TC_LINEAR}}, 1, x3::OUT_F32,
-                           c->COUT.p, nullptr, Q + F);
-            c->x3s[1] = c->x3[XC];
-            c->x3[XC] = keep_c;
-            c->split_clause = k;
-        }
-        if (ok && (split_mask & 2)) {
-            const size_t uplane = Nt * c->HU;
-            CK_CUDA(c, c->U1p.alloc(2 * uplane));
-            CK_CUDA(c, c->U2p.alloc(2 * uplane));
-            x3::X3Mlp keep_u = c->x3[XU];
-            bool k = build(XU, c->VROWp.p, vplane, c->Nt, F + DSAT_AUX_PAD + 3 * Q, c->ldv(), {{7, OP_U1, 0, tc::TC_LRELU}}, 1,
-                           x3::OUT_SPLIT, c->U1p.p, c->U1p.p + uplane, c->HU);
-            c->x3s[2] = c->x3[XU];
-            k = k && build(XU, c->U1p.p, uplane, c->Nt, c->HU, c->HU, {{8, OP_U2, 0, tc::TC_LRELU}}, 1, x3::OUT_SPLIT,
-                           c->U2p.p, c->U2p.p + uplane, c->HU);
-            c->x3s[3] = c->x3[XU];
-            k = k && build(XU, c->U2p.p, uplane, c->Nt, c->HU, c->HU, {{9, OP_U3, 0, tc::TC_LINEAR}}, 1, x3::OUT_F32,
-                           c->UOUT.p, nullptr, F);
-            c->x3s[4] = c->x3[XU];
-            c->x3[XU] = keep_u;
-            c->split_update = k;
-        }
-    }
     c->x3_ready = ok;
     if (!ok) { c->err = "the fp32-accurate tensor-core path supports feature_maps = query_maps <= 128 (hidden widths <= 256 or 512)"; return DSAT_ERR_UNSUPPORTED; }
     c->has_x3_buffers = true;
@@ -1005,13 +965,7 @@
     LAUNCHED(c);
     if (x3p) {
 #ifdef DSAT_WITH_TCGEN05
-        if (c->split_clause) {
-            for (int k = 0; k < 2; ++k) {
-                prof_mark(c, k == 0 ? OP_C1 : OP_C2);
-                CK_CUDA(c, x3::launch_x3(c->x3s[k], c->device, c->sm_count, c->stream));
-                c->launches++;
-            }
-        } else if ((rc = run_x3(c, XC, OP_C2))) return rc;
+        if ((rc = run_x3(c, XC, OP_C2))) return rc;
 #endif
     } else if (!tcp) {
         if ((rc = run_linear(c, OP_C1, c->CROW.p, ldc, c->CH.p, c->HC, Mt, EPI_LRELU))) return rc;
@@ -1087,13 +1041,7 @@
     LAUNCHED(c);
     if (x3p) {
 #ifdef DSAT_WITH_TCGEN05
-        if (c->split_update) {
-            for (int k = 0; k < 3; ++k) {
-                prof_mark(c, k == 0 ? OP_U1 : k == 1 ? OP_U2 : OP_U3);
-                CK_CUDA(c, x3::launch_x3(c->x3s[2 + k], c->device, c->sm_count, c->stream));
-                c->launches++;
-            }
-        } else if ((rc = run_x3(c, XU, OP_U3))) return rc;
+        if ((rc = run_x3(c, XU, OP_U3))) return rc;
 #endif
     } else if (!tcp) {
         if ((rc = run_linear(c, OP_U1, c->VROW.p, ldv, c->U1.p, c->HU, Nt, EPI_LRELU))) return rc;
@@ -2259,22 +2207,8 @@
         switch (which) {
             case 0: rc = run_x3(c, XQ, OP_Q2); break;
             case 1: rc = run_x3(c, XL1, OP_V1); if (!rc) rc = run_x3(c, XL2, OP_L2); if (!rc) rc = run_x3(c, XL3, OP_L3); break;
-            case 2:
-                if (c->split_clause) {
-                    for (int k = 0; k < 2 && !rc; ++k) {
-                        CK_CUDA(c, x3::launch_x3(c->x3s[k], c->device, c->sm_count, c->stream));
-                        c->launches++;
-                    }
-                } else rc = run_x3(c, XC, OP_C2);
-                break;
-            case 3:
-                if (c->split_update) {
-                    for (int k = 0; k < 3 && !rc; ++k) {
-                        CK_CUDA(c, x3::launch_x3(c->x3s[2 + k], c->device, c->sm_count, c->stream));
-                        c->launches++;
-                    }
-                } else rc = run_x3(c, XU, OP_U3);
-                break;
+            case 2: rc = run_x3(c, XC, OP_C2); break;
+            case 3: rc = run_x3(c, XU, OP_U3); break;
             default: rc = run_x3(c, XO, OP_O2); break;
         }
     } else if (use_tc(c) && c->precision == DSAT_BF16 && c->fused_ready && c->use_fused) {
diff --git a/diffusionsat_b200/csrc/dsat_gemm_tc.cuh b/diffusionsat_b200/csrc/dsat_gemm_tc.cuh
--- a/diffusionsat_b200/csrc/dsat_gemm_tc.cuh
+++ b/diffusionsat_b200/csrc/dsat_gemm_tc.cuh
@@ -196,6 +196,51 @@
         "@q tcgen05.mma.cta_group::2.kind::f16 [%0], a2, b2, %3, t;\n"
         "@q tcgen05.mma.cta_group::2.kind::f16 [%0], a3, b3, %3, t;\n"
         "}\n" ::"r"(tmem_d), "l"(desc_a), "l"(desc_b), "r"(idesc), "r"(accumulate_first) : "memory");
+}
+__device__ __forceinline__ uint32_t tmem_a_kstep(int k) { return (uint32_t)(32 * (k >> 1) + 8 * (k & 1)); }
+template <bool PAIR>
+__device__ __forceinline__ void umma_bf16_ts_elect(uint32_t tmem_d, uint32_t tmem_a, uint64_t desc_b, uint32_t idesc, uint32_t accumulate) {
+    if constexpr (PAIR) {
+        asm volatile(
+            "{\n"
+            ".reg .pred p, q;\n"
+            "setp.ne.b32 p, %4, 0;\n"
+            "elect.sync _|q, 0xffffffff;\n"
+            "@q tcgen05.mma.cta_group::2.kind::f16 [%0], [%1], %2, %3, p;\n"
+            "}\n" ::"r"(tmem_d), "r"(tmem_a), "l"(desc_b), "r"(idesc), "r"(accumulate) : "memory");
+    } else {
+        asm volatile(
+            "{\n"
+            ".reg .pred p, q;\n"
+            "setp.ne.b32 p, %4, 0;\n"
+            "elect.sync _|q, 0xffffffff;\n"
+            "@q tcgen05.mma.cta_group::1.kind::f16 [%0], [%1], %2, %3, p;\n"
+            "}\n" ::"r"(tmem_d), "r"(tmem_a), "l"(desc_b), "r"(idesc), "r"(accumulate) : "memory");
+    }
+}
+template <bool PAIR>
+__device__ __forceinline__ void umma_bf16_ts_kblock_elect(uint32_t tmem_d, uint32_t tmem_a, uint64_t desc_b, uint32_t idesc,
+                                                          uint32_t accumulate_first) {
+#define DSAT_UMMA_TS_KBLOCK(CG)                                                              \
+    "{\n"                                                                                    \
+    ".reg .pred p, q, t;\n"                                                                  \
+    ".reg .b32 a1, a2, a3;\n"                                                                \
+    ".reg .b64 b1, b2, b3;\n"                                                                \
+    "setp.ne.b32 p, %4, 0;\n"                                                                \
+    "setp.eq.b32 t, 0, 0;\n"                                                                 \
+    "add.u32 a1, %1, 8;\n add.u32 a2, %1, 32;\n add.u32 a3, %1, 40;\n"                       \
+    "add.s64 b1, %2, 2;\n add.s64 b2, %2, 4;\n add.s64 b3, %2, 6;\n"                         \
+    "elect.sync _|q, 0xffffffff;\n"                                                          \
+    "@q tcgen05.mma.cta_group::" CG ".kind::f16 [%0], [%1], %2, %3, p;\n"                    \
+    "@q tcgen05.mma.cta_group::" CG ".kind::f16 [%0], [a1], b1, %3, t;\n"                    \
+    "@q tcgen05.mma.cta_group::" CG ".kind::f16 [%0], [a2], b2, %3, t;\n"                    \
+    "@q tcgen05.mma.cta_group::" CG ".kind::f16 [%0], [a3], b3, %3, t;\n"                    \
+    "}\n"
+    if constexpr (PAIR)
+        asm volatile(DSAT_UMMA_TS_KBLOCK("2") ::"r"(tmem_d), "r"(tmem_a), "l"(desc_b), "r"(idesc), "r"(accumulate_first) : "memory");
+    else
+        asm volatile(DSAT_UMMA_TS_KBLOCK("1") ::"r"(tmem_d), "r"(tmem_a), "l"(desc_b), "r"(idesc), "r"(accumulate_first) : "memory");
+#undef DSAT_UMMA_TS_KBLOCK
 }
 __device__ __forceinline__ void tcgen05_commit_elect(uint64_t* bar) {
     asm volatile(
diff --git a/diffusionsat_b200/csrc/dsat_mlp_fused.cuh b/diffusionsat_b200/csrc/dsat_mlp_fused.cuh
--- a/diffusionsat_b200/csrc/dsat_mlp_fused.cuh
+++ b/diffusionsat_b200/csrc/dsat_mlp_fused.cuh
@@ -100,6 +100,19 @@
                    "+r"(r[16]), "+r"(r[17]), "+r"(r[18]), "+r"(r[19]), "+r"(r[20]), "+r"(r[21]), "+r"(r[22]), "+r"(r[23]),
                    "+r"(r[24]), "+r"(r[25]), "+r"(r[26]), "+r"(r[27]), "+r"(r[28]), "+r"(r[29]), "+r"(r[30]), "+r"(r[31]));
 }
+
+__device__ __forceinline__ void tmem_st_32cols(uint32_t taddr, const uint32_t (&r)[32]) {
+    asm volatile(
+        "tcgen05.st.sync.aligned.32x32b.x32.b32 [%0], "
+        "{%1, %2, %3, %4, %5, %6, %7, %8, %9, %10, %11, %12, %13, %14, %15, %16, "
+        "%17, %18, %19, %20, %21, %22, %23, %24, %25, %26, %27, %28, %29, %30, %31, %32};"
+        ::"r"(taddr), "r"(r[0]), "r"(r[1]), "r"(r[2]), "r"(r[3]), "r"(r[4]), "r"(r[5]), "r"(r[6]), "r"(r[7]),
+          "r"(r[8]), "r"(r[9]), "r"(r[10]), "r"(r[11]), "r"(r[12]), "r"(r[13]), "r"(r[14]), "r"(r[15]),
+          "r"(r[16]), "r"(r[17]), "r"(r[18]), "r"(r[19]), "r"(r[20]), "r"(r[21]), "r"(r[22]), "r"(r[23]),
+          "r"(r[24]), "r"(r[25]), "r"(r[26]), "r"(r[27]), "r"(r[28]), "r"(r[29]), "r"(r[30]), "r"(r[31])
+        : "memory");
+}
+__device__ __forceinline__ void tmem_st_wait() { asm volatile("tcgen05.wait::st.sync.aligned;" ::: "memory"); }
 
 __device__ __forceinline__ uint4 pack8_bf16(const float* v) {
     __nv_bfloat162 p0 = __floats2bfloat162_rn(v[0], v[1]), p1 = __floats2bfloat162_rn(v[2], v[3]);
diff --git a/diffusionsat_b200/csrc/dsat_mlp_x3.cuh b/diffusionsat_b200/csrc/dsat_mlp_x3.cuh
--- a/diffusionsat_b200/csrc/dsat_mlp_x3.cuh
+++ b/diffusionsat_b200/csrc/dsat_mlp_x3.cuh
@@ -8,10 +8,13 @@
 constexpr int BLOCK_K = 64;
 constexpr int BLK_BYTES = BLOCK_M * BLOCK_K * 2;
 constexpr int MAX_LAYERS = 3;
-constexpr int MAX_RING = 8;
+constexpr int MAX_RING = 12;
 constexpr int TMEM_COLS = 512;
 constexpr int STAGE_ROW = 128 + 16;
-constexpr int BAR_BYTES = 512;
+constexpr int SKIP_UNITS = 1024;
+constexpr int SKIP_OFF = 512;
+constexpr int BAR_BYTES = SKIP_OFF + SKIP_UNITS / 8;
+static_assert((4 * MAX_RING + 6) * 8 + 4 <= SKIP_OFF, "x3 barriers overlap the early-exit bits");
 constexpr int SMEM_LIMIT = 227 * 1024;
 
 enum OutMode : int { OUT_F32 = 0, OUT_SPLIT = 1 };
@@ -29,9 +32,8 @@
     int n_layers;
     X3Layer layer[MAX_LAYERS];
     int rows, n_tiles, n_groups, a_box_rows;
-    int h_blocks;
     int a_slots, w_slots, w_slot_bytes;
-    int epi_warps, stage_in_h, smem_pad, bias_total, qmaps, pair;
+    int epi_warps, smem_pad, bias_total, qmaps, pair;
     int out_mode;
     void* out0; void* out1; int ld_out;
     long long* prof;
@@ -41,8 +43,8 @@
 __device__ __forceinline__ void split2(float v0, float v1, uint32_t& hi, uint32_t& lo) { split_bf16x2(v0, v1, hi, lo); }
 
 struct Epi {
-    uint32_t lane_addr, h_addr, bl_addr, stage_addr;
-    int N, epi, cpar, cstep, r, lane, qmaps, col0, h_plane_bytes;
+    uint32_t lane_addr, bl_addr, stage_addr;
+    int N, epi, cpar, cstep, lane, qmaps, col0;
     size_t row_first; int rows_left;
     void* out0; void* out1; int ld_out, out_mode;
 };
@@ -50,21 +52,10 @@
 __device__ __forceinline__ void epi_hidden(const Epi& e, const uint32_t (&raw)[32], int c) {
     float v[32];
     fm::bias_act_chunk(raw, e.bl_addr + 4u * (uint32_t)c, e.epi == tc::TC_LRELU, v);
-    const uint32_t blk = e.h_addr + (uint32_t)(c >> 6) * BLK_BYTES + (uint32_t)e.r * 128;
-    const int j0 = (c & 63) >> 3;
+    uint32_t w[32];
 #pragma unroll
-    for (int q = 0; q < 4; ++q) {
-        uint4 hi, lo;
-        split2(v[8 * q], v[8 * q + 1], hi.x, lo.x);
-        split2(v[8 * q + 2], v[8 * q + 3], hi.y, lo.y);
-        split2(v[8 * q + 4], v[8 * q + 5], hi.z, lo.z);
-        split2(v[8 * q + 6], v[8 * q + 7], hi.w, lo.w);
-        if (c + 8 * q < e.N) {
-            const uint32_t at = blk + (uint32_t)(((j0 + q) ^ (e.r & 7)) << 4);
-            fm::sts128(at, hi);
-            fm::sts128(at + (uint32_t)e.h_plane_bytes, lo);
-        }
-    }
+    for (int i = 0; i < 16; ++i) split2(v[2 * i], v[2 * i + 1], w[i], w[16 + i]);
+    fm::tmem_st_32cols(e.lane_addr + (uint32_t)c, w);
 }
 
 __device__ __forceinline__ void epi_final(const Epi& e, const uint32_t (&raw)[32], int c) {
@@ -111,12 +102,10 @@
     extern __shared__ __align__(1024) uint8_t smem_raw[];
     uint8_t* smem = reinterpret_cast<uint8_t*>((reinterpret_cast<uintptr_t>(smem_raw) + 1023) & ~(uintptr_t)1023);
     if ((int)(smem - smem_raw) > p.smem_pad) __trap();
-    const int h_plane_bytes = p.h_blocks * BLK_BYTES;
-    uint8_t* hid = smem;
-    uint8_t* a_ring = smem + 2 * (size_t)h_plane_bytes;
+    uint8_t* a_ring = smem;
     uint8_t* w_ring = a_ring + (size_t)p.a_slots * BLK_BYTES;
     uint8_t* stage_all = w_ring + (size_t)p.w_slots * p.w_slot_bytes;
-    uint8_t* tail = stage_all + (p.stage_in_h ? 0 : (size_t)p.epi_warps * 32 * STAGE_ROW);
+    uint8_t* tail = stage_all + (size_t)p.epi_warps * 32 * STAGE_ROW;
     uint64_t* a_full = reinterpret_cast<uint64_t*>(tail);
     uint64_t* a_empty = a_full + MAX_RING;
     uint64_t* w_full = a_empty + MAX_RING;
@@ -124,7 +113,7 @@
     uint64_t* tmem_full = w_empty + MAX_RING;
     uint64_t* tmem_empty = tmem_full + 2;
     uint64_t* h_full = tmem_empty + 2;
-    uint32_t* tmem_slot = reinterpret_cast<uint32_t*>(h_full + 1);
+    uint32_t* tmem_slot = reinterpret_cast<uint32_t*>(h_full + 2);
     float* bias_s = reinterpret_cast<float*>(tail + BAR_BYTES);
 
     const int warp = threadIdx.x >> 5, lane = threadIdx.x & 31;
@@ -142,7 +131,7 @@
             mbar_init(&w_full[s], NC); mbar_init(&w_empty[s], 1);
         }
         for (int b = 0; b < 2; ++b) { mbar_init(&tmem_full[b], 1); mbar_init(&tmem_empty[b], NC * p.epi_warps); }
-        mbar_init(h_full, NC * p.epi_warps);
+        for (int h = 0; h < 2; ++h) mbar_init(&h_full[h], NC * p.epi_warps);
         asm volatile("fence.mbarrier_init.release.cluster;" ::: "memory");
         asm volatile("prefetch.tensormap [%0];" ::"l"(&map_a_hi) : "memory");
         asm volatile("prefetch.tensormap [%0];" ::"l"(&map_a_lo) : "memory");
@@ -176,8 +165,7 @@
     const int nt = unit0 < n_units ? (n_units - unit0 + unit_stride - 1) / unit_stride : 0;
     auto tile_of = [&](int j) { const int u = (unit0 + j * unit_stride) / G; return PAIR ? 2 * u + (int)rank : u; };
     auto group_of = [&](int j) { return (unit0 + j * unit_stride) % G; };
-    constexpr int SKIP_UNITS = 1024;
-    uint32_t* skip_bits = reinterpret_cast<uint32_t*>(tail + 384);
+    uint32_t* skip_bits = reinterpret_cast<uint32_t*>(tail + SKIP_OFF);
     const bool skipping = p.done != nullptr && nt <= SKIP_UNITS;
     if (skipping) {
         for (int base = 32 * warp; base < nt; base += (int)blockDim.x) {
@@ -244,9 +232,18 @@
     } else if (warp == 1) {
         if (leader) {
             int as = 0, ws = 0; uint32_t aph = 0, wph = 0;
-            long long t_wait_acc = 0, t_wait_h = 0, t_wait_a = 0, t_wait_w = 0;
+            long long t_wait_acc = 0, t_wait_h = 0, t_wait_a = 0, t_wait_w = 0, t_wait_read = 0;
             const long long t_begin = timing ? clock64() : 0;
             auto commit = [&](uint64_t* bar) { if constexpr (PAIR) tcgen05_commit_elect_cg2(bar); else tcgen05_commit_elect(bar); };
+            auto kblock_ts = [&](uint32_t acc, uint32_t ta, uint64_t db, uint32_t idesc, uint32_t accum, int ksteps, uint64_t* free_bar) {
+                if (ksteps == BLOCK_K / 16) {
+                    umma_bf16_ts_kblock_elect<PAIR>(acc, ta, db, idesc, accum);
+                } else {
+                    for (int k = 0; k < ksteps; ++k)
+                        umma_bf16_ts_elect<PAIR>(acc, ta + tmem_a_kstep(k), db + (uint64_t)(2 * k), idesc, (accum | (uint32_t)k) != 0);
+                }
+                if (free_bar) commit(free_bar);
+            };
             auto kblock = [&](uint32_t acc, uint64_t da, uint64_t db, uint32_t idesc, uint32_t accum, int ksteps, uint64_t* free_bar) {
                 if (ksteps == BLOCK_K / 16) {
                     if (free_bar) {
@@ -271,41 +268,54 @@
                 for (int l = 0; l < L; ++l) {
                     const int g = jp * L + l, buf = g & 1, use = g >> 1;
                     X3_WAIT(t_wait_acc, mbar_wait(&tmem_empty[buf], (uint32_t)((use & 1) ^ 1)));
-                    if (l > 0) X3_WAIT(t_wait_h, mbar_wait(h_full, (uint32_t)((jp * (L - 1) + (l - 1)) & 1)));
+                    if (g > 0 && (l > 0 ? l - 1 : L - 1) > 0)
+                        X3_WAIT(t_wait_read, mbar_wait(&tmem_full[buf ^ 1], (uint32_t)(((g - 1) >> 1) & 1)));
+                    const uint32_t h_par = (uint32_t)((jp * (L - 1) + (l - 1)) & 1);
                     tcgen05_fence_after();
                     const int K = p.layer[l].K, N = p.layer[l].N;
                     const int kbs = (K + BLOCK_K - 1) / BLOCK_K;
                     const uint32_t idesc = make_idesc_bf16(PAIR ? 2 * BLOCK_M : BLOCK_M, N);
                     const uint32_t acc = tmem_base + (uint32_t)(buf * 256);
+                    const uint32_t hid = tmem_base + (uint32_t)((buf ^ 1) * 256);
                     for (int kb = 0; kb < kbs; ++kb) {
                         const int ksteps = min(BLOCK_K / 16, (K - kb * BLOCK_K + 15) / 16);
-                        uint64_t da_hi, da_lo;
-                        int as_hi = 0, as_lo = 0;
                         if (l == 0) {
-                            as_hi = as;
+                            const int as_hi = as;
                             const uint32_t ph_hi = aph;
                             if (++as == p.a_slots) { as = 0; aph ^= 1; }
-                            as_lo = as;
+                            const int as_lo = as;
                             const uint32_t ph_lo = aph;
                             if (++as == p.a_slots) { as = 0; aph ^= 1; }
                             X3_WAIT(t_wait_a, mbar_wait(&a_full[as_hi], ph_hi));
                             X3_WAIT(t_wait_a, mbar_wait(&a_full[as_lo], ph_lo));
-                            da_hi = make_smem_desc_sw128(smem_u32(a_ring + (size_t)as_hi * BLK_BYTES));
-                            da_lo = make_smem_desc_sw128(smem_u32(a_ring + (size_t)as_lo * BLK_BYTES));
+                            const uint64_t da_hi = make_smem_desc_sw128(smem_u32(a_ring + (size_t)as_hi * BLK_BYTES));
+                            const uint64_t da_lo = make_smem_desc_sw128(smem_u32(a_ring + (size_t)as_lo * BLK_BYTES));
+                            X3_WAIT(t_wait_w, mbar_wait(&w_full[ws], wph));
+                            uint64_t db = make_smem_desc_sw128(smem_u32(w_ring + (size_t)ws * p.w_slot_bytes));
+                            kblock(acc, da_hi, db, idesc, kb != 0, ksteps, nullptr);
+                            kblock(acc, da_lo, db, idesc, 1u, ksteps, &w_empty[ws]);
+                            if (++ws == p.w_slots) { ws = 0; wph ^= 1; }
+                            X3_WAIT(t_wait_w, mbar_wait(&w_full[ws], wph));
+                            db = make_smem_desc_sw128(smem_u32(w_ring + (size_t)ws * p.w_slot_bytes));
+                            kblock(acc, da_hi, db, idesc, 1u, ksteps, &w_empty[ws]);
+                            if (++ws == p.w_slots) { ws = 0; wph ^= 1; }
+                            commit(&a_empty[as_hi]); commit(&a_empty[as_lo]);
                         } else {
-                            da_hi = make_smem_desc_sw128(smem_u32(hid + (size_t)kb * BLK_BYTES));
-                            da_lo = make_smem_desc_sw128(smem_u32(hid + (size_t)h_plane_bytes + (size_t)kb * BLK_BYTES));
+                            const uint32_t ta_hi = hid + (uint32_t)(kb * BLOCK_K), ta_lo = ta_hi + 16;
+                            if ((kb & 1) == 0 && kb < 4) {
+                                X3_WAIT(t_wait_h, mbar_wait(&h_full[kb >> 1], h_par));
+                                tcgen05_fence_after();
+                            }
+                            X3_WAIT(t_wait_w, mbar_wait(&w_full[ws], wph));
+                            uint64_t db = make_smem_desc_sw128(smem_u32(w_ring + (size_t)ws * p.w_slot_bytes));
+                            kblock_ts(acc, ta_hi, db, idesc, kb != 0, ksteps, nullptr);
+                            kblock_ts(acc, ta_lo, db, idesc, 1u, ksteps, &w_empty[ws]);
+                            if (++ws == p.w_slots) { ws = 0; wph ^= 1; }
+                            X3_WAIT(t_wait_w, mbar_wait(&w_full[ws], wph));
+                            db = make_smem_desc_sw128(smem_u32(w_ring + (size_t)ws * p.w_slot_bytes));
+                            kblock_ts(acc, ta_hi, db, idesc, 1u, ksteps, &w_empty[ws]);
+                            if (++ws == p.w_slots) { ws = 0; wph ^= 1; }
                         }
-                        X3_WAIT(t_wait_w, mbar_wait(&w_full[ws], wph));
-                        uint64_t db = make_smem_desc_sw128(smem_u32(w_ring + (size_t)ws * p.w_slot_bytes));
-                        kblock(acc, da_hi, db, idesc, kb != 0, ksteps, nullptr);
-                        kblock(acc, da_lo, db, idesc, 1u, ksteps, &w_empty[ws]);
-                        if (++ws == p.w_slots) { ws = 0; wph ^= 1; }
-                        X3_WAIT(t_wait_w, mbar_wait(&w_full[ws], wph));
-                        db = make_smem_desc_sw128(smem_u32(w_ring + (size_t)ws * p.w_slot_bytes));
-                        kblock(acc, da_hi, db, idesc, 1u, ksteps, &w_empty[ws]);
-                        if (++ws == p.w_slots) { ws = 0; wph ^= 1; }
-                        if (l == 0) { commit(&a_empty[as_hi]); commit(&a_empty[as_lo]); }
                     }
                     commit(&tmem_full[buf]);
                 }
@@ -314,21 +324,19 @@
 #undef X3_WAIT
             if (timing && lane == 0) {
                 p.prof[0] = clock64() - t_begin; p.prof[1] = t_wait_acc; p.prof[2] = t_wait_h; p.prof[3] = t_wait_a; p.prof[4] = t_wait_w;
+                p.prof[8] = t_wait_read;
             }
         }
     } else if (warp < 2 + p.epi_warps) {
         const int quad = warp & 3;
         Epi e;
-        e.r = quad * 32 + lane;
         e.lane = lane;
         e.cpar = (warp - 2) >> 2;
         e.cstep = 32 * (p.epi_warps >> 2);
         e.qmaps = p.qmaps;
         e.out0 = p.out0; e.out1 = p.out1; e.ld_out = p.ld_out; e.out_mode = p.out_mode;
-        e.h_plane_bytes = h_plane_bytes;
-        e.h_addr = smem_u32(hid);
         const uint32_t bias_addr0 = smem_u32(bias_s);
-        e.stage_addr = (p.stage_in_h ? smem_u32(hid) : smem_u32(stage_all)) + (uint32_t)(warp - 2) * (32 * STAGE_ROW);
+        e.stage_addr = smem_u32(stage_all) + (uint32_t)(warp - 2) * (32 * STAGE_ROW);
         long long t_wait_full = 0, t_hidden = 0, t_final = 0;
         int jp = -1;
         for (int j = 0; j < nt; ++j) {
@@ -350,6 +358,16 @@
                 const long long t1 = timing ? clock64() : 0;
                 const uint32_t empty_addr = at_leader(&tmem_empty[buf]);
                 if (l + 1 < L) {
+                    bool low_done = false;
+                    auto release = [&](int h) {
+                        fm::tmem_st_wait();
+                        tcgen05_fence_before();
+                        __syncwarp();
+                        if (lane == 0) {
+                            if (h == 1) fm::arrive_addr<PAIR>(empty_addr);
+                            fm::arrive_addr<PAIR>(at_leader(&h_full[h]));
+                        }
+                    };
                     int c = 32 * e.cpar;
                     if (c < e.N) {
                         uint32_t ra[32], rb[32];
@@ -360,18 +378,18 @@
                             const int c1 = c + e.cstep;
                             if (c1 < e.N) fm::tmem_ld_32cols_async(e.lane_addr + (uint32_t)c1, rb);
                             epi_hidden(e, ra, c);
+                            if (!low_done && c1 >= 128) { release(0); low_done = true; }
                             if (c1 >= e.N) break;
                             fm::tmem_ld_wait(rb);
                             c = c1 + e.cstep;
                             if (c < e.N) fm::tmem_ld_32cols_async(e.lane_addr + (uint32_t)c, ra);
                             epi_hidden(e, rb, c1);
+                            if (!low_done && c >= 128) { release(0); low_done = true; }
                             if (c >= e.N) break;
                         }
                     }
-                    tcgen05_fence_before();
-                    asm volatile("fence.proxy.async.shared::cta;" ::: "memory");
-                    __syncwarp();
-                    if (lane == 0) { fm::arrive_addr<PAIR>(empty_addr); fm::arrive_addr<PAIR>(at_leader(h_full)); }
+                    if (!low_done) release(0);
+                    release(1);
                     if (timing) t_hidden += clock64() - t1;
                 } else {
                     bool released = false;
@@ -388,7 +406,6 @@
                         epi_final(e, ra, c);
                     }
                     if (!released) { tcgen05_fence_before(); fm::warp_arrive<PAIR>(empty_addr, lane); }
-                    if (p.stage_in_h) asm volatile("bar.sync 1, %0;" ::"r"(epi_threads) : "memory");
                     if (timing) t_final += clock64() - t1;
                 }
                 if (timing) t_wait_full += t1 - t0;
@@ -422,48 +439,39 @@
     X3Params& p = f.p;
     const int pad = fm::dyn_smem_pad();
     p.smem_pad = pad;
-    int bias_total = 0, max_n = 0, h_blocks = 0;
+    int bias_total = 0, max_n = 0;
     bool pair = f.pair_mode && p.rows > BLOCK_M;
     for (int l = 0; l < p.n_layers; ++l) {
         X3Layer& ly = p.layer[l];
         if (ly.N > 256 || ly.N % 16 || ly.K % 16) return false;
-        if (l + 1 < p.n_layers) h_blocks = max(h_blocks, (ly.N + 63) / 64);
+        if (l > 0 && ly.K > p.layer[l - 1].N) return false;
         ly.bias_off = bias_total;
         bias_total += (ly.n_total + 31) / 32 * 32;
         max_n = max(max_n, ly.N);
     }
     if (p.n_groups > 1 && p.n_layers != 1) return false;
     p.pair = pair ? 1 : 0;
-    p.h_blocks = h_blocks;
     p.bias_total = bias_total;
     p.n_tiles = ceil_div(p.rows, BLOCK_M);
     p.w_slot_bytes = ((pair ? max_n / 2 : max_n) * BLOCK_K * 2 + 1023) / 1024 * 1024;
     for (int ew : {8, 4}) {
         if (ew == 8 && f.four_epilogue_warps) continue;
-        const int stage_bytes = ew * 32 * STAGE_ROW;
-        const int in_h = 2 * h_blocks * BLK_BYTES >= stage_bytes;
-        const int fixed = pad + 2 * h_blocks * BLK_BYTES + (in_h ? 0 : stage_bytes) + BAR_BYTES + bias_total * 4;
+        const int fixed = pad + ew * 32 * STAGE_ROW + BAR_BYTES + bias_total * 4;
         int avail = SMEM_LIMIT - fixed;
         int a = 2, w = 2;
         if (avail < a * BLK_BYTES + w * p.w_slot_bytes) continue;
         avail -= a * BLK_BYTES + w * p.w_slot_bytes;
-        if (p.n_layers > 1) {
-            const int a_want = min(MAX_RING, 2 * ((p.layer[0].K + BLOCK_K - 1) / BLOCK_K));
-            while (a < a_want && avail >= BLK_BYTES) { ++a; avail -= BLK_BYTES; }
-            while (w < MAX_RING && avail >= p.w_slot_bytes) { ++w; avail -= p.w_slot_bytes; }
-        } else {
-            while (true) {
-                bool grew = false;
-                if (a <= w && a < MAX_RING && avail >= BLK_BYTES) { ++a; avail -= BLK_BYTES; grew = true; }
-                else if (w < MAX_RING && avail >= p.w_slot_bytes) { ++w; avail -= p.w_slot_bytes; grew = true; }
-                else if (a < MAX_RING && avail >= BLK_BYTES) { ++a; avail -= BLK_BYTES; grew = true; }
-                if (!grew) break;
-            }
+        while (true) {
+            bool grew = false;
+            if (a <= w && a < MAX_RING && avail >= BLK_BYTES) { ++a; avail -= BLK_BYTES; grew = true; }
+            else if (w < MAX_RING && avail >= p.w_slot_bytes) { ++w; avail -= p.w_slot_bytes; grew = true; }
+            else if (a < MAX_RING && avail >= BLK_BYTES) { ++a; avail -= BLK_BYTES; grew = true; }
+            if (!grew) break;
         }
         const int ea = env_int("DSAT_X3_A_SLOTS", 0), ewn = env_int("DSAT_X3_W_SLOTS", 0);
         if (ea >= 2 && ewn >= 2 && ea <= MAX_RING && ewn <= MAX_RING &&
             fixed + ea * BLK_BYTES + ewn * p.w_slot_bytes <= SMEM_LIMIT) { a = ea; w = ewn; }
-        p.a_slots = a; p.w_slots = w; p.epi_warps = ew; p.stage_in_h = in_h;
+        p.a_slots = a; p.w_slots = w; p.epi_warps = ew;
         f.smem_bytes = fixed + a * BLK_BYTES + w * p.w_slot_bytes;
         f.ready = true;
         return true;
```

After: 728.1, median of 6. 1.07x the previous value.
